# ChicyChen/LOCO-Edit

Hardware: AMD Instinct MI355X
Metric: edit-directions/sec (top-5 PMP-Jacobian SVD @256^2) + vT cos-sim vs ref (higher is better)
Workload: dtype bf16x3 (split-bf16 MFMA operands, fp32 accumulate + fp32 storage); 1 GPU; CelebA-HQ DDPM 256x256 top-5 local basis (l_eye-sized mask, L=2400), t=0.6T, 12 power iterations, one GPU; multi_gpu_form=single, probes_total=5, probes_per_gpu=5, kept=5, n_iter=12, mask_L=2400, weights=synthetic seed 0, streams=2

## Files before the change

### include/loco_hip_diag.h

```cpp
#ifndef LOCO_HIP_DIAG_H
#define LOCO_HIP_DIAG_H
#include "loco_hip.h"
#ifdef __cplusplus
extern "C" {
#endif

int  loco_bench_conv(loco_ctx* ctx, int32_t cin, int32_t cout, int32_t H, int32_t W, int32_t B, int32_t mode,
                     int32_t taps, int32_t tile, int32_t iters, float* ms_avg, void* stream);

typedef struct loco_conv_desc {
    int32_t struct_size;
    int32_t Cin, Cout, Hin, Win, B, taps;
    int32_t stride, upsample, zins, mode, cpg;
    int32_t transposed, accumulate, in_arena, pad;
    int32_t Cin2, cot_cpg;
    float   res_scale;
    int32_t reserved;
    const float *weight, *bias;
    const float *in, *bias2, *res;
    const float *prim, *sc, *sh, *mr, *gamma, *tst, *tc;
    const float *in2, *w2, *bias2nd;
    const float *cot_d, *cot_prim, *cot_sc, *cot_sh, *cot_mr, *cot_tc;
    float* out;
} loco_conv_desc;
int  loco_debug_conv(loco_ctx* ctx, const loco_conv_desc* desc, char* plan, int64_t cap, void* stream);

int64_t loco_debug_tensor(loco_ctx* ctx, const char* name, float* dst, int64_t cap, void* stream);

#ifdef __cplusplus
}
#endif
#endif
```

### loco-edit_amd/csrc/conv_bf16.hip

```cpp
#include "kernels.h"
#include <cstdio>
#include <cstdlib>

namespace loco {

enum : int { PR_BF16X3 = 0, PR_F16 = 1 };
template <int PR, int TAPS, int MODE> void launch_tile_b(const ConvArgs& a, hipStream_t st);
template <int PR, int MODE> void launch_kcat_b(const ConvArgs& a, hipStream_t st);
template <int PR, int MODE> void launch_pair_b(const ConvArgs& a, hipStream_t st);
template <int PR, int MODE> void launch_dual_b(const ConvArgs& a, hipStream_t st);
void launch_conv_gemm(const ConvArgs& a, hipStream_t st);

template <int PR>
static void launch_lowp(const ConvArgs& a, int taps, hipStream_t st) {
#ifdef LOCO_DIAG
    if (a.cot_d && (taps != 1 || a.gemm || a.nsplit > 1 || a.Cin2 > 0 || (a.Cout % conv_bf16_tile_couts(a)) != 0 || a.st_kind == ST_TAN || a.st_kind == ST_COT)) {
        fprintf(stderr, "loco: ConvArgs::cot_d on a launch whose epilogue has no norm-cotangent term (taps %d, gemm %d, nsplit %d, Cout %d, st_kind %d)\n",
                taps, a.gemm, a.nsplit, a.Cout, a.st_kind);
        abort();
    }
#endif
    if constexpr (PR == PR_BF16X3) {
        if (taps == 1 && a.gemm) { launch_conv_gemm(a, st); return; }
    }
    if (taps == 9 && a.Cin2 > 0) {
        if (a.mode == CM_GN_SILU) launch_kcat_b<PR, CM_GN_SILU>(a, st);
        else if (a.mode == CM_GN_GELU) launch_kcat_b<PR, CM_GN_GELU>(a, st);
        else launch_kcat_b<PR, CM_TAN_SILU>(a, st);
        return;
    }
#ifdef LOCO_DIAG
    if constexpr (PR == PR_BF16X3) {
        if (taps == 9 && a.dual) {
            switch (a.mode) {
                case CM_NONE: launch_dual_b<PR, CM_NONE>(a, st); break;
                case CM_GN_SILU: launch_dual_b<PR, CM_GN_SILU>(a, st); break;
                case CM_TAN_SILU: launch_dual_b<PR, CM_TAN_SILU>(a, st); break;
                default: launch_dual_b<PR, CM_COT_SILU>(a, st); break;
            }
            return;
        }
    }
#endif
    if constexpr (PR == PR_BF16X3) {
        if (taps == 9 && a.pair) {
            switch (a.mode) {
                case CM_NONE: launch_pair_b<PR, CM_NONE>(a, st); break;
                case CM_GN_SILU: launch_pair_b<PR, CM_GN_SILU>(a, st); break;
                case CM_TAN_SILU: launch_pair_b<PR, CM_TAN_SILU>(a, st); break;
                default: launch_pair_b<PR, CM_COT_SILU>(a, st); break;
            }
            return;
        }
    }
    if (taps == 9) {
        switch (a.mode) {
            case CM_NONE: launch_tile_b<PR, 9, CM_NONE>(a, st); break;
            case CM_GN_SILU: launch_tile_b<PR, 9, CM_GN_SILU>(a, st); break;
            case CM_GN_GELU: launch_tile_b<PR, 9, CM_GN_GELU>(a, st); break;
            case CM_TAN_SILU: launch_tile_b<PR, 9, CM_TAN_SILU>(a, st); break;
            case CM_COT_SILU: launch_tile_b<PR, 9, CM_COT_SILU>(a, st); break;
            default: launch_tile_b<PR, 9, CM_GN>(a, st); break;
        }
    } else {
        switch (a.mode) {
            case CM_NONE: launch_tile_b<PR, 1, CM_NONE>(a, st); break;
            default: launch_tile_b<PR, 1, CM_GN>(a, st); break;
        }
    }
}
void launch_conv_bf16x3(const ConvArgs& a, int taps, hipStream_t st) { launch_lowp<PR_BF16X3>(a, taps, st); }
void launch_conv_f16(const ConvArgs& a, int taps, hipStream_t st) { launch_lowp<PR_F16>(a, taps, st); }

}
```

### loco-edit_amd/csrc/conv_plan.hip

```cpp
#include "kernels.h"
#include <cstdio>
#include <cstdlib>

namespace loco {

constexpr int BKC = 16;
constexpr int BKF = 8;

static const int kMT[7] = {128, 128, 32, 64, 128, 128, 128}, kNT[7] = {128, 64, 128, 64, 256, 256, 128};

static int env_int(const char* name, int dflt) {
    const char* e = getenv(name);
    return e ? atoi(e) : dflt;
}
static int diag_switch(const char* name) {
#ifdef LOCO_DIAG
    return env_int(name, 0);
#else
    (void)name;
    return 0;
#endif
}

static int pick_tile(int Cout, int HW) {
    if (HW >= 128) return Cout > 32 ? 0 : 2;
    return Cout > 64 ? 1 : 3;
}

static int conv_pick_nsplit(int Cin, int Cout, int Hout, int Wout, int B) {
    const int t = pick_tile(Cout, Hout * Wout);
    long blocks = (long)((Hout * Wout) / kNT[t]) * ((Cout + kMT[t] - 1) / kMT[t]) * B;
    int nchunks = (Cin + BKF - 1) / BKF;
    if (blocks >= 384 || nchunks < 8) return 1;
    int want = (int)((512 + blocks - 1) / blocks);
    int maxs = nchunks / 4;
    if (want > maxs) want = maxs;
    if (want > 32) want = 32;
    return want < 1 ? 1 : want;
}

static int conv_bf16_pick_tile(int Cout, int HW, int B, int tile_override) {
    if (B <= 1 && HW <= 1024 && HW >= 64 && (Cout % 64) == 0) return 3;
    int t = pick_tile(Cout, HW);
    if (t == 0 && HW >= 256) {
        if (tile_override >= 0) return tile_override;
        return 5;
    }
    return t;
}

constexpr int kTile0MaxHW = 65536;

static int bf16_tile_of(const ConvArgs& a, int tile_override = -1) {
    static const bool two_per_cu = diag_switch("LOCO_CONV_2WG") != 0;
    int tile = conv_bf16_pick_tile(a.Cout, a.Hout * a.Wout, a.B, tile_override);
    if (tile == 4) tile = 5;
    if (tile == 5 && a.taps == 1 && !a.gemm && a.B >= 2 && a.Hout * a.Wout <= kTile0MaxHW) return 0;
    if (tile == 5 && two_per_cu && a.taps == 9 && a.stride == 1 && !a.upsample && !a.zins && (a.Cin % BKC) == 0 &&
        a.in_padded && a.pad == 1 && a.Wout >= 32) return 6;
    if (a.stride == 2 && tile == 5) tile = 0;
    return tile;
}
static int tile_for(const ConvArgs& a, int prec, int tile_override) {
    return prec ? bf16_tile_of(a, tile_override) : pick_tile(a.Cout, a.Hout * a.Wout);
}
static int conv_bf16_tile_pixels(const ConvArgs& a) { return a.gemm ? 256 : kNT[a.tile]; }
int conv_bf16_tile_couts(const ConvArgs& a) { return a.gemm ? 64 * a.gemm_tm : kMT[a.tile]; }

static int conv_bf16_pick_nsplit(int Cin, int Cout, int Hout, int Wout, int B, int chip_share, int taps, int lanes) {
    const int HW = Hout * Wout;
    int t = conv_bf16_pick_tile(Cout, HW, B, -1);
    if (t == 4) t = 5;
    if (taps == 1 && t == 5 && B >= 2 && HW <= kTile0MaxHW) t = 0;
    long blocks = (long)(HW / kNT[t]) * ((Cout + kMT[t] - 1) / kMT[t]) * B;
    int nchunks = (Cin + BKC - 1) / BKC;
    int target = chip_share > 1 ? 256 / chip_share : (lanes == 2 ? 240 : 256);
    if (target < 32) target = 32;
    if (blocks >= target / 2 || nchunks < 8) return 1;
    int want = (int)(target / blocks);
    int maxs = nchunks / 4;
    if (want > maxs) want = maxs;
    if (want > 32) want = 32;
    return want < 1 ? 1 : want;
}

static bool conv_lowp_can_kcat(const ConvArgs& a) {
    static const bool on = env_int("LOCO_KCAT", 1) != 0;
    return on && a.Cin2 > 0 && a.nsplit == 1 && bf16_tile_of(a) == 5 && a.stride == 1 && !a.upsample && !a.zins && a.pad == 1 &&
           (a.Cin % BKC) == 0 && (a.Cin2 % BKC) == 0 && a.in_padded &&
           (a.mode == CM_GN_SILU || a.mode == CM_GN_GELU || a.mode == CM_TAN_SILU);
}
static bool conv_lowp_can_fuse_stats(const ConvArgs& a) {
    return a.nsplit <= 1 && !a.gemm && (a.Cout % conv_bf16_tile_couts(a)) == 0;
}

static bool conv_pair_ok(const ConvArgs& a) {
    static const bool on = env_int("LOCO_CONV_PAIR", 1) != 0;
    if (!on || a.Hout * a.Wout < 16384 || a.taps != 9 || a.Cin2 > 0 || a.nsplit != 1 || a.stride != 1 || a.upsample || a.zins ||
        a.pad != 1 || !a.in_padded || (a.Cin % (2 * BKC)) != 0 || (a.Cout % 128) != 0 || (a.Wout % 32) != 0 || (a.Hout % 8) != 0 ||
        a.pers_groups || a.dual)
        return false;
    if (!(a.mode == CM_NONE || a.mode == CM_GN_SILU || a.mode == CM_TAN_SILU || a.mode == CM_COT_SILU)) return false;
    return a.tile == 5;
}

static bool conv_dual_ok(const ConvArgs& a) {
    static const bool on = diag_switch("LOCO_CONV_DUAL") != 0;
    if (!on || a.taps != 9 || a.Cin2 > 0 || a.nsplit != 1 || a.stride != 1 || a.upsample || a.zins || a.pad != 1 || (a.Cin % BKC) != 0 ||
        !a.in_padded || a.Wout < 32 || (a.Wout % 32) != 0 || (a.Hout % 8) != 0 || (a.Cout % 128) != 0 || a.B < 2 || a.cot_d)
        return false;
    if (!(a.mode == CM_NONE || a.mode == CM_GN_SILU || a.mode == CM_TAN_SILU || a.mode == CM_COT_SILU)) return false;
    if (a.tile != 5) return false;
    const long units = (long)((a.Hout * a.Wout) / 256) * (a.Cout / 128) * (a.B / 2);
    return units >= 192;
}

static ConvArgs conv_shift_batch(const ConvArgs& a, int nb) {
    ConvArgs t = a;
    t.B = a.B - nb;
    t.in += (long)nb * a.in_bs; t.out += (long)nb * a.out_bs;
    if (t.prim) t.prim += (long)nb * a.prim_bs;
    if (t.bias2) t.bias2 += (long)nb * a.bias2_bs;
    if (t.res) t.res += (long)nb * a.res_bs;
    if (t.sc) { t.sc += (long)nb * a.scsh_bs; t.sh += (long)nb * a.scsh_bs; }
    if (t.mr) t.mr += (long)nb * a.mr_bs;
    if (t.tst) t.tst += (long)nb * a.tst_bs;
    if (t.tc) t.tc += (long)nb * a.tc_bs;
    if (t.in2) t.in2 += (long)nb * a.in2_bs;
    if (t.cot_d) { t.cot_d += (long)nb * a.cot_d_bs; t.cot_tc += (long)nb * a.cot_tc_bs; }
    if (t.st_part) t.st_part += (long)nb * a.Cout * ((a.Hout * a.Wout) / conv_bf16_tile_pixels(a)) * 2;
    return t;
}

static void conv_pers_plan(ConvArgs& a) {
    a.pers_groups = 0;
    static const int on = diag_switch("LOCO_CONV_PERS");
    if (!on || a.taps != 9 || a.Cin2 > 0 || a.nsplit != 1 || a.stride != 1 || a.upsample || a.zins || a.pad != 1 || !a.in_padded ||
        (a.Cin % (2 * BKC)) != 0 || (a.Cout % 128) != 0 || a.B < 2 || a.cot_d || bf16_tile_of(a) != 5)
        return;
    if (!(a.mode == CM_NONE || a.mode == CM_GN_SILU || a.mode == CM_GN_GELU ||
          (on == 2 && (a.mode == CM_TAN_SILU || a.mode == CM_COT_SILU)))) return;
    const long wg0 = (long)((a.Hout * a.Wout) / 256) * (a.Cout / 128);
    int G = wg0 >= 256 ? 1 : (int)(256 / wg0);
    if (G > a.B) G = a.B;
    const int per = (a.B + G - 1) / G;
    if (per < 2 || a.B * 10 < G * per * 8 || wg0 * G < 192) return;
    a.pers_groups = G;
}

static void conv_gemm_plan(ConvArgs& a) {
    static const bool on = env_int("LOCO_CONV_GEMM", 1) != 0;
    a.gemm = 0;
    const long HW = (long)a.Hout * a.Wout;
    if (!on || a.stride != 1 || a.upsample || a.zins || (a.Cin % BKC) != 0 || a.Cin < 320 || (HW % 256) != 0 || (a.Wout % 16) != 0 ||
        a.Cout < 128 || !a.partial || a.Cin2 > 0 || !(a.mode == CM_NONE || a.mode == CM_GN) || a.cot_d)
        return;
    {
        const int TW = a.Wout < 32 ? a.Wout : 32;
        if ((256 % TW) != 0 || (a.Wout % TW) != 0 || (a.Hout % (256 / TW)) != 0) return;
    }
    static const int all_shapes = env_int("LOCO_GEMM_ALL", 0);
    if (!all_shapes && !(a.Cout >= 640 && (a.Cout >= 4 * a.Cin || a.Cin >= 2560))) return;
    const int pad256 = (a.Cout + 255) / 256 * 256;
    const int tm = (pad256 * 10 <= a.Cout * 11) ? 4 : 2;
    const int mt = 64 * tm;
    const long tiles = (HW / 256) * ((a.Cout + mt - 1) / mt) * a.B;
    const size_t rec_floats = (size_t)a.B * a.Cin * HW;
    int ns = 1;
    if (tiles < 192) {
        const int nchunks = a.Cin / BKC;
        ns = (int)((256 + tiles - 1) / tiles);
        if (ns > 8) ns = 8;
        while (ns > 1 && nchunks / ns < 8) --ns;
        while (ns > 1 && (size_t)ns * a.B * a.Cout * HW + rec_floats > a.partial_floats) --ns;
    }
    if ((ns > 1 ? (size_t)ns * a.B * a.Cout * HW : 0) + rec_floats > a.partial_floats) return;
    a.gemm = 1; a.gemm_tm = tm; a.nsplit = ns;
}

void conv_plan_family(ConvArgs& a, int prec) {
    if (prec == 1 && a.taps == 1) conv_gemm_plan(a);
    if (prec == 1 && a.taps == 9) conv_pers_plan(a);
}

int conv_plan_parts(ConvArgs& a, int prec, int tile_override, ConvArgs parts[2]) {
    a.dual = 0;
    a.tile = tile_for(a, prec, tile_override);
    a.pair = 0;
    parts[0] = a;
    int n = 1;
    if (prec == 1 && a.taps == 9 && conv_dual_ok(a)) {
        parts[0].B = a.B & ~1;
        parts[0].dual = 1;
        if (a.B & 1) {
            parts[1] = conv_shift_batch(a, a.B - 1);
            parts[1].pers_groups = 0;
            n = 2;
        }
    }
    for (int i = 0; i < n; ++i) {
        ConvArgs& p = parts[i];
        p.tile = tile_for(p, prec, tile_override);
        p.pair = prec == 1 && conv_pair_ok(p);
    }
    return n;
}

static bool short_tail(long per_probe, int B) {
    const long total = per_probe * B, r = total % 256;
    return total > 256 && r > 0 && r <= 160;
}

static int tail_split(const ConvArgs& a, size_t partial_floats, int* split) {
    const long per_probe = (long)((a.Hout * a.Wout) / conv_bf16_tile_pixels(a)) * ((a.Cout + 127) / 128);
    const long r = per_probe * a.B % 256;
    if (!short_tail(per_probe, a.B) || per_probe <= 0 || r % per_probe != 0 || r / per_probe >= a.B) return 0;
    int s = (int)(256 / r);
    if (s > 4) s = 4;
    const int nchunks = (a.Cin + 15) / 16;
    while (s > 1 && nchunks / s < 4) --s;
    const size_t one = (size_t)(r / per_probe) * a.Cout * a.Hout * a.Wout;
    while (s > 1 && (size_t)s * one > partial_floats) --s;
    *split = s;
    return s > 1 ? (int)(r / per_probe) : 0;
}

static int stats_route(const ConvEnv& e, const StatAsk* q, bool want, ConvArgs& x, int s0, int B, int* keep_ntile) {
    if (!q || q->kind == ST_NONE) return SR_NONE;
    const int alone = q->norm ? SR_ALONE : SR_NONE;
    if (!want) return alone;
    if (x.nsplit > 1) return !q->norm ? SR_NONE : ((x.Hout * x.Wout) % 4 == 0 ? SR_SPLITK : SR_ALONE);
    const int ntile = (x.Hout * x.Wout) / conv_bf16_tile_pixels(x);
    const size_t need = (size_t)x.B * x.Cout * ntile * 2;
    const int epi = q->norm ? SR_EPI : SR_KEEP;
    const bool kept = q->keep && s0 == 0 && x.B == B && need <= q->keep_floats;
    if (q->kind == ST_FWD && conv_lowp_can_fuse_stats(x) && (kept || (q->norm && need <= e.stpart_floats))) {
        x.st_part = kept ? q->keep : e.stpart; x.st_kind = ST_FWD;
        if (kept) *keep_ntile = ntile;
        return epi;
    }
    const bool cot_cache = q->kind == ST_COT && q->norm && q->sx;
    if ((q->kind == ST_TAN || cot_cache) && e.fuse_lin && !x.cot_d && conv_lowp_can_fuse_stats(x) && !x.pers_groups &&
        !conv_dual_ok(x)) {
        const size_t lane_off = (size_t)e.lane_s0 * (q->keep_floats / e.max_batch);
        const bool keptl = q->kind == ST_TAN && q->keep && s0 == 0 && x.B == B && lane_off + need <= q->keep_floats;
        if (keptl || (q->norm && need <= e.stpart_floats)) {
            x.st_part = keptl ? q->keep + lane_off : e.stpart; x.st_kind = q->kind; x.st_x = q->prim;
            if (q->kind == ST_COT) x.st_sx = q->sx;
            if (keptl) *keep_ntile = ntile;
            return epi;
        }
    }
    return alone;
}

static ConvLaunch plan_launch(const ConvEnv& e, const StatAsk* q, bool want, const ConvArgs& x, int s0, int B, int* keep_ntile) {
    ConvLaunch l;
    l.args = x;
    l.s0 = s0;
    l.args.tile = tile_for(x, e.prec, -1);
    l.stats = stats_route(e, q, want, l.args, s0, B, keep_ntile);
    if (l.stats == SR_EPI || l.stats == SR_KEEP) l.ntile = (x.Hout * x.Wout) / conv_bf16_tile_pixels(l.args);
    l.nparts = conv_plan_parts(l.args, e.prec, -1, l.parts);
    return l;
}

ConvPlan plan_conv(const ConvEnv& e, const ConvArgs& a0, int taps, const StatAsk* q, const ConvArgs* sc) {
    ConvPlan p;
    ConvArgs a = a0;
    a.taps = taps;
    a.dual = 0; a.pers_groups = 0; a.gemm = 0;
    if (sc) {
        ConvArgs t = a;
        t.nsplit = e.prec >= 1 ? conv_bf16_pick_nsplit(a.Cin, a.Cout, a.Hout, a.Wout, a.B, e.chip_share, 9, e.lanes) : 2;
        t.in2 = sc->in; t.in2_bs = sc->in_bs; t.Cin2 = sc->Cin;
        const long per_probe = (long)((a.Hout * a.Wout) / 256) * ((a.Cout + 127) / 128);
        if (e.prec >= 1 && taps == 9 && !short_tail(per_probe, a.B) && !a.bias2 && conv_lowp_can_kcat(t)) {
            a.in2 = sc->in; a.in2_bs = sc->in_bs; a.Cin2 = sc->Cin; a.in2_padded = sc->in_padded;
            a.wb2 = e.prec == 2 ? sc->wh : sc->wb;
            a.bias2 = sc->bias; a.bias2_bs = 0;
            a.res = nullptr;
        } else {
            p.sc_first = true;
            a.res = sc->out; a.res_bs = sc->out_bs;
        }
    }
    if (e.prec == 2) a.wb = a.wh;
    a.no_deep = e.deep1 ? 0 : 1;
    a.nsplit = e.prec >= 1 ? conv_bf16_pick_nsplit(a.Cin, a.Cout, a.Hout, a.Wout, a.B, e.chip_share, taps, e.lanes)
                           : conv_pick_nsplit(a.Cin, a.Cout, a.Hout, a.Wout, a.B);
    if (a.cot_d) {
        ConvArgs t = a;
        t.tile = bf16_tile_of(t);
        const long per_probe = (long)((a.Hout * a.Wout) / conv_bf16_tile_pixels(t)) * ((a.Cout + 127) / 128);
        p.cot = e.prec >= 1 && taps == 1 && a.nsplit == 1 && !short_tail(per_probe, a.B) && conv_lowp_can_fuse_stats(t);
        if (!p.cot) { a.cot_d = nullptr; a.cot_d_bs = 0; a.cot_sx = nullptr; a.cot_tc = nullptr; a.cot_tc_bs = 0; }
    }
    while (a.nsplit > 1 && (size_t)a.nsplit * a.B * a.Cout * a.Hout * a.Wout > e.partial_floats) a.nsplit >>= 1;
    if (a.nsplit < 1) a.nsplit = 1;
    a.partial = e.partial;
    a.partial_floats = e.partial_floats;
    conv_plan_family(a, e.prec);
    a.tile = tile_for(a, e.prec, -1);
    int split = 1;
    const int tail = e.prec >= 1 && a.nsplit == 1 && a.B >= 2 && !a.gemm && !a.pers_groups ? tail_split(a, e.partial_floats, &split) : 0;
    const bool want = q && q->kind != ST_NONE && e.prec >= 1 && e.fuse_stats;
    if (!tail) {
        p.l[0] = plan_launch(e, q, want, a, 0, a.B, &p.keep_ntile);
        return p;
    }
    const bool per_part = want && q->norm && (q->kind == ST_FWD || (e.fuse_lin && (a.Hout * a.Wout) % 4 == 0));
    p.stats_all = !per_part && q && q->kind != ST_NONE && q->norm;
    const StatAsk* ql = per_part ? q : nullptr;
    const int nb = a.B - tail;
    ConvArgs m = a, t = conv_shift_batch(a, nb);
    m.B = nb;
    t.nsplit = split;
    p.nl = 2;
    p.l[0] = plan_launch(e, ql, want, m, 0, a.B, &p.keep_ntile);
    p.l[1] = plan_launch(e, ql, want, t, nb, a.B, &p.keep_ntile);
    return p;
}

const char* conv_variant_name(const ConvArgs& a, int taps, int prec) {
    static const char* tiles[6] = {"2,2,2,2", "4,1,1,2", "1,4,1,1", "2,2,1,1", "2,2,2,4", "2,4,2,2"};
    static char names[3][2][6][6][56];
    static char others[5][3][6][40];
    const int mode = (a.mode < 0 || a.mode > 5) ? 2 : a.mode;
    const char* other = nullptr;
    int k = 0, v = mode;
    if (prec && taps == 9 && a.Cin2 > 0) other = prec == 1 ? "conv_kcat_bf16x3<2,4,2,2,%d>" : "conv_kcat_f16<2,4,2,2,%d>";
    else if (prec == 1 && taps == 1 && a.gemm) { k = 1; other = "conv_gemm_bf16x3<%d>"; v = a.gemm_tm; }
    else if (prec == 1 && taps == 9 && a.pers_groups > 0 && !a.dual) { k = 2; other = "conv_pers_bf16x3<9,2,4,2,2,%d>"; }
    else if (prec == 1 && taps == 9 && a.pair) { k = 3; other = "conv_pair_bf16x3<%d>"; }
    else if (prec == 1 && taps == 9 && a.dual) { k = 4; other = "conv_dual_bf16x3<%d>"; }
    if (other) {
        char* n = others[k][prec][v];
        if (!n[0]) snprintf(n, 40, other, v);
        return n;
    }
    int t = a.tile == 6 ? 0 : a.tile;
    if (t < 0 || t > 5) t = 0;
    int m = mode;
    if (taps != 9 && m != CM_NONE) m = CM_GN;
    if (!prec && m == CM_GN_GELU) m = CM_GN_SILU;
    char* n = names[prec][taps == 9 ? 0 : 1][t][m];
    static const char* kn[3] = {"conv_mfma_f32", "conv_mfma_bf16x3", "conv_mfma_f16"};
    if (!n[0]) snprintf(n, 56, "%s<%d,%s,%d>", kn[prec], taps, tiles[t], m);
    return n;
}

}
```

### loco-edit_amd/csrc/conv_plan_text.h

```cpp
#pragma once
#include "kernels.h"
#include <cstdio>
#include <string>

namespace loco {

inline void conv_plan_text(const ConvPlan& p, int taps, int prec, std::string& out) {
    char line[320];
    for (int li = 0; li < p.nl; ++li) {
        const ConvLaunch& l = p.l[li];
        for (int pi = 0; pi < l.nparts; ++pi) {
            const ConvArgs& y = l.parts[pi];
            snprintf(line, sizeof(line),
                     "launch=%d part=%d kernel=%s tile=%d nsplit=%d B=%d s0=%d gemm=%d gemm_tm=%d pair=%d Cin2=%d sc_first=%d cot=%d\n",
                     li, pi, conv_variant_name(y, taps, prec), y.tile, l.args.nsplit, y.B, l.s0 + (pi ? l.args.B - y.B : 0), y.gemm,
                     y.gemm ? y.gemm_tm : 0, y.pair, y.Cin2, p.sc_first ? 1 : 0, p.cot ? 1 : 0);
            out += line;
        }
    }
}

}
```

### loco-edit_amd/csrc/engine.hip

```cpp
#include <hip/hip_runtime.h>

#include <algorithm>
#include <array>
#include <cmath>
#include <cstdio>
#include <cstdlib>
#include <cstring>
#include <map>
#include <memory>
#include <thread>
#include <atomic>
#include <string>
#include <vector>

#include "../../include/loco_hip.h"
#ifdef LOCO_DIAG
#include "../../include/loco_hip_diag.h"
#endif
#include "kernels.h"
#include "program.h"
#ifdef LOCO_DIAG
#include "conv_plan_text.h"
#endif

// ... 35 lines not shown
};
struct Weights {
    std::vector<OpWeights> op;
    float *freq = nullptr, *td0w = nullptr, *td0b = nullptr, *td1w = nullptr, *td1b = nullptr;
    float* tcw = nullptr;
    float *tp_w = nullptr, *tp_b = nullptr;
    long tproj_total = 0;
    double flops = 0.0;
};

struct Tens : TensPlan {
    float* keep = nullptr; size_t keep_floats = 0; int keep_ntile = 0;
};
struct NormP : NormPlan, NormW {
    bool ready = false;
};
struct Op : OpPlan, OpWeights {
    NormP n1, n2, nx;
    float *xK = nullptr, *xV = nullptr;
};

struct HostParam { std::vector<float> data; std::vector<int64_t> shape; bool loaded = false; };

}


struct loco_ctx {
    loco_unet_cfg cfg;
    std::string err;
    std::map<std::string, HostParam> params;
    bool finalized = false;

    std::shared_ptr<const Program> prog;
    std::shared_ptr<Weights> wts;
    std::vector<Tens> tens;
    std::vector<Op> ops;


    float *arenaP = nullptr, *arenaT = nullptr;
    float *statsP = nullptr, *statsT = nullptr;
    double* red = nullptr;
    bool fuse_cot = true;
    float *stpart = nullptr, *stpart2 = nullptr;
    size_t stpart_floats = 0;
    bool fuse_stats = true;
    bool fuse_xattn = true;
    bool deep1 = true;
    bool flash_attn = true;
    float* attn_delta = nullptr;
    float* partial = nullptr;
    size_t partial_floats = 0;
    const float* bench_out = nullptr; int64_t bench_out_count = 0;
#ifdef LOCO_DIAG
    std::string* plan_log = nullptr;
#endif
    float *tact = nullptr, *tproj = nullptr;
    float* eps_buf = nullptr;
    float* gx0 = nullptr;
    float* ge = nullptr;
    float* tmpA = nullptr;
    double *G = nullptr, *Q = nullptr, *W = nullptr, *gscratch = nullptr;
    float* alphas = nullptr;
    float* ctx_colbias = nullptr;
    bool has_ctx = false;
    float* cond_add = nullptr;
    float* ctx_norm = nullptr;
    bool has_cond = false;
    float* cond_in = nullptr;
    bool has_tcond = false;
    float2* sxcache = nullptr;
    int prec = 0;
    std::vector<float*> owned;
    size_t bytes = 0;

    bool primal_ok = false;
    float p_cv = 0.f, p_ce = 0.f;
    uint8_t* mask = nullptr;
    bool has_mask = false;
    uint8_t* mask2 = nullptr;
    bool has_mask2 = false;
    int mask2_from = 0;
    int* mask_idx = nullptr;
    int* mask_L_dev = nullptr;
    long mask_L = 0;
    hipStream_t mask_stream = nullptr;
    int primal_B = 0;
    hipEvent_t ev0 = nullptr, ev1 = nullptr;
    int n_streams = 1;
    hipStream_t st2 = nullptr;
    hipStream_t st2_user = nullptr;
    hipEvent_t ev_fork = nullptr, ev_join = nullptr;
    double* red2 = nullptr;
    struct FwdGraph { hipGraph_t graph = nullptr; hipGraphExec_t exec = nullptr; int calls = 0; };
    std::map<int, FwdGraph> fwd_graphs;
    bool graph_on = false;
    bool gemm_lowp = true;
    unsigned char* gemm_ws[2] = {nullptr, nullptr}; size_t gemm_ws_bytes[2] = {0, 0}; int lane = 0;
    loco_ctx* weights_of = nullptr;
    int forks = 0;
    bool zombie = false;
    bool fuse_lin = true;
    int lanes_active = 1;
    int lane_s0 = 0;
    int chip_share = 1;
    hipStream_t cap_st = nullptr;
    float* xin_buf = nullptr;
    float* t_dev = nullptr;
    bool prof_on = false;
    struct ProfRec { const char* name; double flops; hipEvent_t e0, e1; int cin, cout, h, b, ns, mode, taps; };
    bool prof_shapes = false;
    std::vector<ProfRec> prof;
    std::vector<hipEvent_t> ev_pool;
    size_t ev_used = 0;
    hipEvent_t next_event() {
        if (ev_used == ev_pool.size()) {
            hipEvent_t e; (void)hipEventCreate(&e); ev_pool.push_back(e);
        }
        return ev_pool[ev_used++];
    }
};

namespace {

template <typename T>
int dalloc(loco_ctx* c, T** p, size_t count) {
    void* q = nullptr;
    HIPCHK(c, hipMalloc(&q, count * sizeof(T)));
    *p = reinterpret_cast<T*>(q);
    c->owned.push_back(reinterpret_cast<float*>(q));
    c->bytes += count * sizeof(T);
    return 0;
}

inline float eps_of(const loco_ctx* c, const NormP& n) { return n.eps > 0.f ? n.eps : c->cfg.gn_eps; }


int upload(loco_ctx* c, float** dst, const std::vector<float>& h) {
    if (dalloc(c, dst, h.size() ? h.size() : 1)) return -1;
    HIPCHK(c, hipMemcpy(*dst, h.data(), h.size() * sizeof(float), hipMemcpyHostToDevice));
    return 0;
}

static inline uint16_t f2bf(float f) {
    uint32_t u; std::memcpy(&u, &f, 4);
    u += 0x7FFFu + ((u >> 16) & 1u);
    return (uint16_t)(u >> 16);
}
static inline float bf2f(uint16_t h) {
    uint32_t u = (uint32_t)h << 16; float f; std::memcpy(&f, &u, 4); return f;
}
template <typename F>
static void parallel_for(int n, size_t work, F fn) {
    unsigned nt = std::thread::hardware_concurrency();
    if (nt > 16) nt = 16;
    if ((int)nt > n) nt = (unsigned)n;
    if (nt <= 1 || work < ((size_t)1 << 18)) { for (int i = 0; i < n; ++i) fn(i); return; }
    std::atomic<int> next{0};
    std::vector<std::thread> th;
    for (unsigned t = 0; t < nt; ++t)
        th.emplace_back([&]() { int i; while ((i = next.fetch_add(1)) < n) fn(i); });
    for (auto& t : th) t.join();
}

template <typename F>
static std::vector<float> build_records(int nin, int nout, int taps, F get) {
    int nch = (nin + 15) / 16, noutP = (nout + 31) & ~31;
// ... 895 lines not shown
                const long PSb = p.bs();
                auto X = [&](int i) { return p.T(op.xt[i]); };
                if (!op.n1.ready) gn_forward_stats(p, op.n1, p.T(op.in), PSb, HW);
                op.n1.ready = false;
                NS s = nstats(c, stats, op.n1);
                {
                    ConvArgs a; conv_defaults(a);
                    a.in = p.T(op.in); a.in_bs = PSb; a.Cin = C; a.Hin = H; a.Win = W;
                    setw(a, op.pj_in, false); a.bias = op.pj_in.bias; a.pad = 0;
                    a.mode = CM_GN; a.sc = s.sc; a.sh = s.sh; a.scsh_bs = SB;
                    a.out = X(X_H0); a.out_bs = PSb; a.Cout = C; a.Hout = H; a.Wout = W; a.B = B;
                    run_conv(c, a, 1, st);
                }
                const SA sa{c, &op, B, T, NH, C / NH, st};
                const XA xa = xa_of(c, op, B, st);
                launch_ln_fwd(X(X_H0), PSb, B, C, T, op.lng[0], op.lnb[0], 1e-5f, X(X_A1), PSb, X(X_LN1), PSb, st);
                lin1x1(c, op.qkvc, false, X(X_A1), PSb, C, X(X_QKV), PSb, 3 * C, H, W, B, nullptr, 0, false, st);
                sa_forward(sa, arena);
                lin1x1(c, op.to_out1, false, X(X_O), PSb, C, X(X_H1), PSb, C, H, W, B, X(X_H0), PSb, true, st);
                launch_ln_fwd(X(X_H1), PSb, B, C, T, op.lng[1], op.lnb[1], 1e-5f, X(X_A2), PSb, X(X_LN2), PSb, st);
                lin1x1(c, op.xqc, false, X(X_A2), PSb, C, X(X_XQ), PSb, C, H, W, B, nullptr, 0, false, st);
                if (!xa_fused(xa, 0, X(X_XQ), PSb, op.xK, op.xV, X(X_XS), PSb, X(X_XO), PSb)) {
                    xa_scores(xa, X(X_XQ), PSb, op.xK, X(X_XS), PSb, xa.scale, true);
                    launch_softmax_rows(X(X_XS), (long)NH * T, xa.Lp, st, B, PSb);
                    xa_values(xa, op.xV, X(X_XS), PSb, X(X_XO), PSb);
                }
                lin1x1(c, op.to_out2, false, X(X_XO), PSb, C, X(X_H2), PSb, C, H, W, B, X(X_H1), PSb, true, st);
                launch_ln_fwd(X(X_H2), PSb, B, C, T, op.lng[2], op.lnb[2], 1e-5f, X(X_A3), PSb, X(X_LN3), PSb, st);
                lin1x1(c, op.ff1, false, X(X_A3), PSb, C, X(X_F), PSb, 8 * C, H, W, B, nullptr, 0, true, st);
                launch_geglu(0, X(X_F), PSb, nullptr, B, 4L * C * T, X(X_GG), PSb, st);
                lin1x1(c, op.ff2, false, X(X_GG), PSb, 4 * C, X(X_H3), PSb, C, H, W, B, X(X_H2), PSb, true, st);
                const StatReq rq = next_fwd(op.out);
                lin1x1(c, op.pj_out, false, X(X_H3), PSb, C, p.T(op.out), PSb, C, H, W, B, p.T(op.in), PSb, true, st, &rq);
                break;
            }
            case OP_DOWN: case OP_UP: {
                const Tens& ti = c->tens[op.in];
                ConvArgs a; conv_defaults(a);
                a.in = p.T(op.in); a.in_bs = p.bs(); a.Cin = ti.C; a.Hin = ti.H; a.Win = ti.W;
                setw(a, op.conv, false); a.bias = op.conv.bias;
                if (op.kind == OP_DOWN) { a.stride = 2; a.pad = op.sym_down ? 1 : 0; } else { a.upsample = 1; }
                a.out = p.T(op.out); a.out_bs = p.bs(); a.Cout = to.C; a.Hout = to.H; a.Wout = to.W; a.B = B;
                const StatReq rq = next_fwd(op.out);
                run_conv(c, a, 9, st, &rq);
                break;
            }
            case OP_OUT: {
                const Tens& ti = c->tens[op.in];
                if (!op.n1.ready) gn_forward_stats(p, op.n1, p.T(op.in), p.bs(), ti.H * ti.W);
                op.n1.ready = false;
                NS s = nstats(c, stats, op.n1);
                ConvArgs a; conv_defaults(a);
                a.in = p.T(op.in); a.in_bs = p.bs(); a.Cin = ti.C; a.Hin = ti.H; a.Win = ti.W;
                setw(a, op.conv, false); a.bias = op.conv.bias;
                a.mode = CM_GN_SILU; a.sc = s.sc; a.sh = s.sh; a.scsh_bs = SB;
                a.out = p.T(op.out); a.out_bs = p.bs(); a.Cout = to.C; a.Hout = to.H; a.Wout = to.W; a.B = B;
                run_conv(c, a, 9, st);
                break;
            }
        }
    }
    return 0;
}

void tangent_stats(loco_ctx* c, const NormP& n, const float* d, long dbs, const float* x, int HW, int B,
                   hipStream_t st) {
    NS sp = nstats(c, c->statsP, n);
    NS stt = nstats(c, c->statsT, n);
    launch_gn_tstats(d, dbs, x, 0, B, n.C, HW, c->cfg.gn_groups, sp.sc, sp.sh, sp.mr, 0, 0, 0, stt.tst,
                     stt.tc, c->prog->stats_per_sample, c->red, st);
}
void set_tan(loco_ctx* c, ConvArgs& a, const NormP& n, const float* prim) {
    NS sp = nstats(c, c->statsP, n);
    NS stt = nstats(c, c->statsT, n);
    a.mode = CM_TAN_SILU; a.prim = prim; a.prim_bs = 0;
    a.sc = sp.sc; a.sh = sp.sh; a.scsh_bs = 0; a.mr = sp.mr; a.mr_bs = 0; a.gamma_ = n.gamma;
    a.tst = stt.tst; a.tst_bs = c->prog->stats_per_sample; a.cpg = n.C / c->cfg.gn_groups;
    a.tc = stt.tc; a.tc_bs = c->prog->stats_per_sample;
    a.sx = (n.sx_off >= 0 && c->sxcache) ? c->sxcache + n.sx_off : nullptr;
}

constexpr size_t RED_BYTES = (size_t)4 << 20;

int tangent_pass(loco_ctx* c, const float* V, int B, hipStream_t st) {
    const loco_unet_cfg& cfg = c->cfg;
    const long PS = c->prog->per_sample;
    auto TP = [&](int id) { return c->arenaP + c->tens[id].off; };
    auto TT = [&](int id) { return c->arenaT + c->tens[id].off; };
    clear_ready(c);
    auto next_tan = [&](int tid) {
        StatReq r = req_lin(c, ST_TAN, consumer_norm(c, tid), TP(tid));
        Tens& t = c->tens[tid];
        if (t.cat_of >= 0 && t.keep && c->fuse_lin) {
            r.kind = ST_TAN; r.stats = c->statsT; r.prim = TP(tid);
            r.keep = t.keep; r.keep_floats = t.keep_floats; r.keep_ntile = &t.keep_ntile;
        }
        return r;
    };
    for (auto& op : c->ops) {
        const Tens& to = c->tens[op.out];
        const int HW = to.H * to.W;
        switch (op.kind) {
            case OP_CONV_IN: {
                ConvArgs a; conv_defaults(a);
                a.in = V; a.in_bs = c->prog->n_in; a.Cin = cfg.in_channels; a.Hin = cfg.resolution; a.Win = cfg.resolution;
                setw(a, op.conv, false);
                a.out = TT(op.out); a.out_bs = PS; a.Cout = to.C; a.Hout = to.H; a.Wout = to.W; a.B = B;
                if (op.ksize == 1) a.pad = 0;
                const StatReq rq = next_tan(op.out);
                run_conv(c, a, op.ksize == 1 ? 1 : 9, st, &rq);
                break;
            }
            case OP_CONV: {
                const Tens& ti = c->tens[op.in];
                ConvArgs a; conv_defaults(a);
                a.in = TT(op.in); a.in_bs = PS; a.Cin = ti.C; a.Hin = ti.H; a.Win = ti.W;
                setw(a, op.conv, false);
                a.out = TT(op.out); a.out_bs = PS; a.Cout = to.C; a.Hout = to.H; a.Wout = to.W; a.B = B;
                if (op.ksize == 1) a.pad = 0;
                const StatReq rq = next_tan(op.out);
                run_conv(c, a, op.ksize == 1 ? 1 : 9, st, &rq);
                break;
            }
            case OP_RES: {
                const Tens& ti = c->tens[op.in];
                const int HWi = ti.H * ti.W;
                if (!op.n1.ready && !cat_fused_tstats(c, op.n1, op.in, B, st)) tangent_stats(c, op.n1, TT(op.in), PS, TP(op.in), HWi, B, st);
                op.n1.ready = false;
                ConvArgs a; conv_defaults(a);
                a.Cin = ti.C;
                setw(a, op.c1, false);
                if (op.updown == 1) {
                    NS sp = nstats(c, c->statsP, op.n1);
                    NS stt = nstats(c, c->statsT, op.n1);
                    launch_gn_apply(5, TT(op.in), PS, TP(op.in), 0, nullptr, 0, TT(op.a1), PS, 0, B, ti.C, HWi,
                                    cfg.gn_groups, sp.sc, sp.sh, sp.mr, 0, 0, stt.tst, c->prog->stats_per_sample, st, cfg.act);
                    launch_pool2x2_sum(TT(op.a1), PS, TT(op.ap), PS, 0, B, ti.C, to.H, to.W, st, 0.25f);
                    launch_pool2x2_sum(TT(op.in), PS, TT(op.xu), PS, 0, B, ti.C, to.H, to.W, st, 0.25f);
                    a.in = TT(op.ap); a.in_bs = PS; a.Hin = to.H; a.Win = to.W;
                } else {
                    a.in = TT(op.in); a.in_bs = PS; a.Hin = ti.H; a.Win = ti.W;
                    set_tan(c, a, op.n1, TP(op.in));
                    if (op.updown == 2) {
                        a.upsample = 1;
                        launch_upsample2x(TT(op.in), PS, TT(op.xu), PS, 0, 1.0f, B, ti.C, ti.H, ti.W, st);
                    }
                }
                a.out = TT(op.h1); a.out_bs = PS; a.Cout = to.C; a.Hout = to.H; a.Wout = to.W; a.B = B;
                {
                    const StatReq rq2 = req_lin(c, ST_TAN, &op.n2, TP(op.h1));
                    run_conv(c, a, 9, st, &rq2);
                    op.n2.ready = false;
                }
                const float* xin = op.updown ? TT(op.xu) : TT(op.in);
                ConvArgs n; conv_defaults(n);
                if (op.has_nin) {
                    n.in = xin; n.in_bs = PS; n.Cin = ti.C; n.Hin = to.H; n.Win = to.W;
                    setw(n, op.nin, false); n.pad = 0;
                    n.out = TT(op.out); n.out_bs = PS; n.Cout = to.C; n.Hout = to.H; n.Wout = to.W; n.B = B;
                }
                ConvArgs b; conv_defaults(b);
                b.in = TT(op.h1); b.in_bs = PS; b.Cin = to.C; b.Hin = to.H; b.Win = to.W;
                setw(b, op.c2, false); b.res = xin; b.res_bs = PS;
                b.res_scale = op.has_nin ? 1.f : c->prog->res_scale;
                set_tan(c, b, op.n2, TP(op.h1));
                b.out = TT(op.out); b.out_bs = PS; b.Cout = to.C; b.Hout = to.H; b.Wout = to.W; b.B = B;
                const StatReq rq = next_tan(op.out);
// ... 49 lines not shown
                attn_gemm(c, h, st);
                if (!kcat) { h.A = v; h.sab = 0; h.Bm = TT(op.S); h.sbb = PS; h.beta = 1.f; attn_gemm(c, h, st); }
                }
                ConvArgs pr; conv_defaults(pr);
                pr.in = TT(op.o); pr.in_bs = PS; pr.Cin = C; pr.Hin = to.H; pr.Win = to.W;
                setw(pr, op.proj, false); pr.pad = 0; pr.res = TT(op.in); pr.res_bs = PS;
                pr.out = TT(op.has_x ? op.xmid : op.out); pr.out_bs = PS; pr.Cout = C; pr.Hout = to.H; pr.Wout = to.W; pr.B = B;
                {
                    const StatReq rq = next_tan(op.has_x ? op.xmid : op.out);
                    run_conv(c, pr, 1, st, &rq);
                }
                if (op.has_x) {
                    const XA x = xa_of(c, op, B, st);
                    if (!op.nx.ready) tangent_stats(c, op.nx, TT(op.xmid), PS, TP(op.xmid), HW, B, st);
                    op.nx.ready = false;
                    NS spx = nstats(c, c->statsP, op.nx);
                    NS stx = nstats(c, c->statsT, op.nx);
                    launch_gn_apply(1, TT(op.xmid), PS, TP(op.xmid), 0, nullptr, 0, TT(op.xhn), PS, 0, B, C, HW,
                                    cfg.gn_groups, spx.sc, spx.sh, spx.mr, 0, 0, stx.tst, c->prog->stats_per_sample, st);
                    xa_conv1x1(c, op.xqc, false, TT(op.xhn), PS, TT(op.xq), PS, C, to.H, to.W, B, nullptr, 0, false, st);
                    if (!xa_fused(x, 1, TT(op.xq), PS, op.xK, op.xV, TP(op.xS), 0, TT(op.xo), PS)) {
                        xa_scores(x, TT(op.xq), PS, op.xK, TT(op.xS), PS, 1.f, false);
                        launch_softmax_jac(TT(op.xS), TP(op.xS), (long)NH * T, x.Lp, (long)NH * T, x.scale, st, B, PS);
                        xa_values(x, op.xV, TT(op.xS), PS, TT(op.xo), PS);
                    }
                    const StatReq rqx = next_tan(op.out);
                    xa_conv1x1(c, op.xproj, false, TT(op.xo), PS, TT(op.out), PS, C, to.H, to.W, B, TT(op.xmid), PS, false, st, &rqx);
                }
                break;
            }
            case OP_XFMR: {
                const int C = to.C, T = HW, NH = op.heads, H = to.H, W = to.W;
                auto XP = [&](int i) { return TP(op.xt[i]); };
                auto XT_ = [&](int i) { return TT(op.xt[i]); };
                if (!op.n1.ready) tangent_stats(c, op.n1, TT(op.in), PS, TP(op.in), HW, B, st);
                op.n1.ready = false;
                NS sp = nstats(c, c->statsP, op.n1);
                NS stt = nstats(c, c->statsT, op.n1);
                launch_gn_apply(1, TT(op.in), PS, TP(op.in), 0, nullptr, 0, XT_(X_G0), PS, 0, B, C, HW,
                                cfg.gn_groups, sp.sc, sp.sh, sp.mr, 0, 0, stt.tst, c->prog->stats_per_sample, st);
                lin1x1(c, op.pj_in, false, XT_(X_G0), PS, C, XT_(X_H0), PS, C, H, W, B, nullptr, 0, false, st);
                const SA sa{c, &op, B, T, NH, C / NH, st};
                const XA xa = xa_of(c, op, B, st);
                launch_ln_tan(XT_(X_H0), PS, XP(X_H0), XP(X_LN1), B, C, T, op.lng[0], XT_(X_A1), PS, st);
                lin1x1(c, op.qkvc, false, XT_(X_A1), PS, C, XT_(X_QKV), PS, 3 * C, H, W, B, nullptr, 0, false, st);
                sa_tangent(sa);
                lin1x1(c, op.to_out1, false, XT_(X_O), PS, C, XT_(X_H1), PS, C, H, W, B, XT_(X_H0), PS, false, st);
                launch_ln_tan(XT_(X_H1), PS, XP(X_H1), XP(X_LN2), B, C, T, op.lng[1], XT_(X_A2), PS, st);
                lin1x1(c, op.xqc, false, XT_(X_A2), PS, C, XT_(X_XQ), PS, C, H, W, B, nullptr, 0, false, st);
                if (!xa_fused(xa, 1, XT_(X_XQ), PS, op.xK, op.xV, XP(X_XS), 0, XT_(X_XO), PS)) {
                    xa_scores(xa, XT_(X_XQ), PS, op.xK, XT_(X_XS), PS, 1.f, false);
                    launch_softmax_jac(XT_(X_XS), XP(X_XS), (long)NH * T, xa.Lp, (long)NH * T, xa.scale, st, B, PS);
                    xa_values(xa, op.xV, XT_(X_XS), PS, XT_(X_XO), PS);
                }
                lin1x1(c, op.to_out2, false, XT_(X_XO), PS, C, XT_(X_H2), PS, C, H, W, B, XT_(X_H1), PS, false, st);
                launch_ln_tan(XT_(X_H2), PS, XP(X_H2), XP(X_LN3), B, C, T, op.lng[2], XT_(X_A3), PS, st);
                lin1x1(c, op.ff1, false, XT_(X_A3), PS, C, XT_(X_F), PS, 8 * C, H, W, B, nullptr, 0, false, st);
                launch_geglu(1, XT_(X_F), PS, XP(X_F), B, 4L * C * T, XT_(X_GG), PS, st);
                lin1x1(c, op.ff2, false, XT_(X_GG), PS, 4 * C, XT_(X_H3), PS, C, H, W, B, XT_(X_H2), PS, false, st);
                const StatReq rq = next_tan(op.out);
                lin1x1(c, op.pj_out, false, XT_(X_H3), PS, C, TT(op.out), PS, C, H, W, B, TT(op.in), PS, false, st, &rq);
                break;
            }
            case OP_DOWN: case OP_UP: {
                const Tens& ti = c->tens[op.in];
                ConvArgs a; conv_defaults(a);
                a.in = TT(op.in); a.in_bs = PS; a.Cin = ti.C; a.Hin = ti.H; a.Win = ti.W;
                setw(a, op.conv, false);
                if (op.kind == OP_DOWN) { a.stride = 2; a.pad = op.sym_down ? 1 : 0; } else { a.upsample = 1; }
                a.out = TT(op.out); a.out_bs = PS; a.Cout = to.C; a.Hout = to.H; a.Wout = to.W; a.B = B;
                const StatReq rq = next_tan(op.out);
                run_conv(c, a, 9, st, &rq);
                break;
            }
            case OP_OUT: {
                const Tens& ti = c->tens[op.in];
                if (!op.n1.ready) tangent_stats(c, op.n1, TT(op.in), PS, TP(op.in), ti.H * ti.W, B, st);
                op.n1.ready = false;
                ConvArgs a; conv_defaults(a);
                a.in = TT(op.in); a.in_bs = PS; a.Cin = ti.C; a.Hin = ti.H; a.Win = ti.W;
                setw(a, op.conv, false);
                set_tan(c, a, op.n1, TP(op.in));
                a.out = TT(op.out); a.out_bs = PS; a.Cout = to.C; a.Hout = to.H; a.Wout = to.W; a.B = B;
                run_conv(c, a, 9, st);
                break;
            }
        }
    }
    return 0;
}

void cot_stats(loco_ctx* c, const NormP& n, const float* d, long dbs, const float* x, int HW, int B, int kind,
               hipStream_t st) {
    NS sp = nstats(c, c->statsP, n);
    NS stt = nstats(c, c->statsT, n);
    launch_gn_tstats(d, dbs, x, 0, B, n.C, HW, c->cfg.gn_groups, sp.sc, sp.sh, sp.mr, 0, 0, kind, stt.tst,
                     stt.tc, c->prog->stats_per_sample, c->red, st, c->cfg.act);
}

int cotangent_pass(loco_ctx* c, const float* ge, const float* gx0, float* Aout, int B, hipStream_t st) {
    const loco_unet_cfg& cfg = c->cfg;
    const long PS = c->prog->per_sample;
    const int G = cfg.gn_groups;
    auto TP = [&](int id) { return c->arenaP + c->tens[id].off; };
    auto TG = [&](int id) { return c->arenaT + c->tens[id].off; };
    auto GO = [&](const Op& o) -> const float* { return o.out == c->prog->eps_t ? ge : TG(o.out); };
    auto GOS = [&](const Op& o) -> long { return o.out == c->prog->eps_t ? (long)c->prog->n_out : PS; };
    clear_ready(c);
    for (int oi = (int)c->ops.size() - 1; oi >= 0; --oi) {
        Op& op = c->ops[oi];
        const Tens& to = c->tens[op.out];
        const int HW = to.H * to.W;
        switch (op.kind) {
            case OP_OUT: {
                const Tens& ti = c->tens[op.in];
                ConvArgs a; conv_defaults(a);
                a.in = GO(op); a.in_bs = GOS(op); a.Cin = to.C; a.Hin = to.H; a.Win = to.W;
                setw(a, op.conv, true);
                a.out = TG(op.a1); a.out_bs = PS; a.Cout = ti.C; a.Hout = ti.H; a.Wout = ti.W; a.B = B;
                {
                    const StatReq rq = req_lin(c, ST_COT, &op.n1, TP(op.in));
                    run_conv(c, a, 9, st, &rq);
                    op.n1.ready = false;
                }
                NS sp = nstats(c, c->statsP, op.n1);
                NS stt = nstats(c, c->statsT, op.n1);
                launch_gn_apply(2, TG(op.a1), PS, TP(op.in), 0, nullptr, 0, TG(op.in), PS, 0, B, ti.C, ti.H * ti.W, G,
                                sp.sc, sp.sh, sp.mr, 0, 0, stt.tst, c->prog->stats_per_sample, st, cfg.act);
                break;
            }
            case OP_UP: {
                const Tens& ti = c->tens[op.in];
                ConvArgs a; conv_defaults(a);
                a.in = TG(op.out); a.in_bs = PS; a.Cin = to.C; a.Hin = to.H; a.Win = to.W;
                setw(a, op.conv, true);
                a.out = TG(op.up); a.out_bs = PS; a.Cout = ti.C; a.Hout = to.H; a.Wout = to.W; a.B = B;
                run_conv(c, a, 9, st);
                launch_pool2x2_sum(TG(op.up), PS, TG(op.in), PS, 0, B, ti.C, ti.H, ti.W, st);
                break;
            }
            case OP_DOWN: {
                const Tens& ti = c->tens[op.in];
                ConvArgs a; conv_defaults(a);
                a.in = TG(op.out); a.in_bs = PS; a.Cin = to.C; a.Hin = to.H; a.Win = to.W;
                setw(a, op.conv, true); a.zins = 1; a.pad = op.sym_down ? 1 : 2; a.accumulate = op.in_is_skip ? 1 : 0;
                a.out = TG(op.in); a.out_bs = PS; a.Cout = ti.C; a.Hout = ti.H; a.Wout = ti.W; a.B = B;
                run_conv(c, a, 9, st);
                break;
            }
            case OP_RES: {
                const Tens& ti = c->tens[op.in];
                const int HWi = ti.H * ti.W;
                ConvArgs a; conv_defaults(a);
                a.in = TG(op.out); a.in_bs = PS; a.Cin = to.C; a.Hin = to.H; a.Win = to.W;
                setw(a, op.c2, true);
                a.out = TG(op.h1); a.out_bs = PS; a.Cout = to.C; a.Hout = to.H; a.Wout = to.W; a.B = B;
                {
                    const StatReq rq2 = req_lin(c, ST_COT, &op.n2, TP(op.h1));
                    run_conv(c, a, 9, st, &rq2);
                    op.n2.ready = false;
                }
                ConvArgs b; conv_defaults(b);
                b.in = TG(op.h1); b.in_bs = PS; b.Cin = to.C; b.Hin = to.H; b.Win = to.W;
                setw(b, op.c1, true);
                set_tan(c, b, op.n2, TP(op.h1));
                b.mode = CM_COT_SILU;
                b.out_bs = PS; b.Cout = ti.C; b.Hout = to.H; b.Wout = to.W; b.B = B;
                if (op.updown == 0) {
                    b.out = TG(op.a1);
                    const StatReq rq1 = req_lin(c, ST_COT, &op.n1, TP(op.in));
                    run_conv(c, b, 9, st, &rq1);
                } else if (op.updown == 1) {
                    b.out = TG(op.ap);
                    run_conv(c, b, 9, st);
                    launch_upsample2x(TG(op.ap), PS, TG(op.a1), PS, 0, 0.25f, B, ti.C, to.H, to.W, st);
                } else {
                    b.out = TG(op.xu);
                    run_conv(c, b, 9, st);
                    launch_pool2x2_sum(TG(op.xu), PS, TG(op.a1), PS, 0, B, ti.C, ti.H, ti.W, st);
                }
                if (!op.n1.ready) cot_stats(c, op.n1, TG(op.a1), PS, TP(op.in), HWi, B, 1, st);
                op.n1.ready = false;
                NS sp = nstats(c, c->statsP, op.n1);
                NS stt = nstats(c, c->statsT, op.n1);
                int acc = op.in_is_skip ? 1 : 0;
                const float* gsk = TG(op.out);
                bool cot_in_epilogue = false;
                if (op.has_nin) {
                    ConvArgs n; conv_defaults(n);
                    n.in = TG(op.out); n.in_bs = PS; n.Cin = to.C; n.Hin = to.H; n.Win = to.W;
                    setw(n, op.nin, true); n.pad = 0;
                    n.Cout = ti.C; n.Hout = to.H; n.Wout = to.W; n.B = B; n.out_bs = PS;
                    n.out = TG(op.in); n.accumulate = acc;
                    if (op.updown == 0 && c->prec >= 1 && c->fuse_cot && op.n1.sx_off >= 0 && c->sxcache) {
                        n.cot_d = TG(op.a1); n.cot_d_bs = PS; n.cot_sx = c->sxcache + op.n1.sx_off;
                        n.cot_tc = stt.tc; n.cot_tc_bs = c->prog->stats_per_sample;
                    }
                    cot_in_epilogue = run_conv(c, n, 1, st);
                    gsk = nullptr;
                }
                if (op.updown == 0) {
                    if (cot_in_epilogue) {  }
                    else if (op.has_nin)
                        launch_gn_apply(2, TG(op.a1), PS, TP(op.in), 0, nullptr, 0, TG(op.in), PS, 1, B, ti.C, HWi, G,
                                        sp.sc, sp.sh, sp.mr, 0, 0, stt.tst, c->prog->stats_per_sample, st, cfg.act);
                    else
                        launch_gn_apply(2, TG(op.a1), PS, TP(op.in), 0, gsk, PS, TG(op.in), PS, acc, B, ti.C, HWi, G,
                                        sp.sc, sp.sh, sp.mr, 0, 0, stt.tst, c->prog->stats_per_sample, st, cfg.act, c->prog->res_scale);
                } else {
                    launch_gn_apply(2, TG(op.a1), PS, TP(op.in), 0, nullptr, 0, TG(op.in), PS, acc, B, ti.C, HWi, G,
                                    sp.sc, sp.sh, sp.mr, 0, 0, stt.tst, c->prog->stats_per_sample, st, cfg.act);
// ... 171 lines not shown
    c->lanes_active = 1;
    if (rc) return rc;
    HIPCHK(c, hipEventRecord(c->ev_join, s2));
    HIPCHK(c, hipStreamWaitEvent(st, c->ev_join, 0));
    return 0;
}
int alloc_state(loco_ctx* c) {
    const Program& P = *c->prog;
    const size_t MB = (size_t)c->cfg.max_batch;
    c->tens.resize(P.tens.size());
    c->ops.resize(P.ops.size());
    for (size_t i = 0; i < P.tens.size(); ++i) {
        Tens& t = c->tens[i];
        static_cast<TensPlan&>(t) = P.tens[i];
        if (t.cat_of < 0) continue;
        t.keep_floats = MB * (size_t)t.C * ((size_t)t.H * t.W / 64 + 1) * 2;
        if (dalloc(c, &t.keep, t.keep_floats)) return -1;
    }
    for (size_t i = 0; i < P.ops.size(); ++i) {
        const OpPlan& plan = P.ops[i];
        Op& v = c->ops[i];
        static_cast<OpPlan&>(v) = plan;
        static_cast<NormPlan&>(v.n1) = plan.n1; static_cast<NormPlan&>(v.n2) = plan.n2; static_cast<NormPlan&>(v.nx) = plan.nx;
        if (!plan.has_ctx_kv()) continue;
        const size_t kv = (size_t)P.tens[plan.in].C * P.ctx_Lp;
        if (dalloc(c, &v.xK, kv) || dalloc(c, &v.xV, kv)) return -1;
    }
    return 0;
}

int create_ctx(loco_ctx* c, const loco_unet_cfg* cfg, std::shared_ptr<const Program> prog) {
    c->cfg = *cfg;
    c->prog = std::move(prog);
    const size_t MB = (size_t)cfg->max_batch;
    {
        float *p0 = nullptr, *p1 = nullptr;
        if (dalloc(c, &p0, MB * c->prog->per_sample + 128) || dalloc(c, &p1, MB * c->prog->per_sample + 128)) return -1;
        c->arenaP = p0 + 64; c->arenaT = p1 + 64;
    }
    if (dalloc(c, &c->statsP, MB * c->prog->stats_per_sample) || dalloc(c, &c->statsT, MB * c->prog->stats_per_sample)) return -1;
    if (dalloc(c, &c->red, RED_BYTES) || dalloc(c, &c->red2, RED_BYTES)) return -1;
    if (alloc_state(c)) return -1;
    {
        c->stpart_floats = MB * (size_t)(c->prog->max_tensor / 64 + 1) * 2;
        if (dalloc(c, &c->stpart, c->stpart_floats) || dalloc(c, &c->stpart2, c->stpart_floats)) return -1;
        const char* e = getenv("LOCO_FUSE_STATS");
        c->fuse_stats = !(e && atoi(e) == 0);
        e = getenv("LOCO_FUSE_LIN");
        c->fuse_lin = !(e && atoi(e) == 0);
        e = getenv("LOCO_FUSE_COT");
        c->fuse_cot = !(e && atoi(e) == 0) && cfg->act == ACT_SILU;
        e = getenv("LOCO_DEEP1");
        c->deep1 = !(e && atoi(e) == 0);
        e = getenv("LOCO_FUSE_XATTN");
        c->fuse_xattn = !(e && atoi(e) == 0);
        const char* fa = getenv("LOCO_FLASH_ATTN");
        c->flash_attn = !(fa && atoi(fa) == 0);
        if (dalloc(c, &c->attn_delta, MB * (size_t)c->prog->attn_dmax)) return -1;
    }
    c->partial_floats = (size_t)64 << 20;
    if (dalloc(c, &c->partial, c->partial_floats)) return -1;
    if (dalloc(c, &c->xin_buf, MB * c->prog->n_in) || dalloc(c, &c->t_dev, 4)) return -1;
    if (dalloc(c, &c->eps_buf, MB * c->prog->n_out) || dalloc(c, &c->gx0, MB * c->prog->n_in) || dalloc(c, &c->ge, MB * c->prog->n_out))
        return -1;
    if (dalloc(c, &c->tmpA, (size_t)64 * c->prog->n_in)) return -1;
    if (dalloc(c, &c->G, 64 * 64) || dalloc(c, &c->Q, 64 * 64) || dalloc(c, &c->W, SOLVER_W_GATE + 1)) return -1;
    {
        size_t nblk = ((size_t)c->prog->n_in + 255) / 256;
        if (dalloc(c, &c->gscratch, nblk * 64 * 64 + 4096)) return -1;
    }
    if (dalloc(c, &c->alphas, 256) || dalloc(c, &c->cond_add, (size_t)cfg->ch * 4)) return -1;
    if (dalloc(c, &c->cond_in, (size_t)cfg->ch)) return -1;
    {
        float2* sx0 = nullptr;
        if (dalloc(c, &sx0, (size_t)c->prog->sx_total + 64)) return -1;
        c->sxcache = sx0 + 32;
    }
    {
        const char* e = getenv("LOCO_PRECISION");
        c->prec = (e && std::string(e) == "f32") ? 0 : (e && std::string(e) == "f16") ? 2 : 1;
    }
    if (dalloc(c, &c->mask2, (size_t)c->prog->n_out)) return -1;
    if (dalloc(c, &c->mask, (size_t)c->prog->n_out) || dalloc(c, &c->mask_idx, (size_t)c->prog->n_out) ||
        dalloc(c, &c->mask_L_dev, 4)) return -1;
    HIPCHK(c, hipEventCreate(&c->ev0));
    HIPCHK(c, hipEventCreate(&c->ev1));
    {
        const char* e = getenv("LOCO_STREAMS");
        c->n_streams = (e && atoi(e) == 2) ? 2 : 1;
        HIPCHK(c, hipStreamCreateWithFlags(&c->st2, hipStreamNonBlocking));
        HIPCHK(c, hipStreamCreateWithFlags(&c->cap_st, hipStreamNonBlocking));
        const char* gl = getenv("LOCO_GEMM_LOWP");
        if (gl) c->gemm_lowp = atoi(gl) != 0;
        const char* gr = getenv("LOCO_GRAPH");
        c->graph_on = gr && atoi(gr) == 1;
        HIPCHK(c, hipEventCreateWithFlags(&c->ev_fork, hipEventDisableTiming));
        HIPCHK(c, hipEventCreateWithFlags(&c->ev_join, hipEventDisableTiming));
    }
    return 0;
}

}

extern "C" {

const char* loco_version(void) { return "loco_hip 0.2 (gfx950; conv arithmetic: f32 MFMA | bf16x3 split-bf16 MFMA | f16 MFMA)"; }

int loco_device_count(void) {
    int n = 0;
    if (hipGetDeviceCount(&n) != hipSuccess) return 0;
    return n;
}

int loco_create(const loco_unet_cfg* cfg, loco_ctx** out) {
    if (!cfg || !out) return -2;
    loco_ctx* c = new loco_ctx();
    *out = c;
    if (cfg->struct_size != (int32_t)sizeof(loco_unet_cfg)) {
        c->err = "loco_unet_cfg.struct_size = " + std::to_string(cfg->struct_size) + ", this library expects " +
                 std::to_string(sizeof(loco_unet_cfg)) + " (binding and library built from different headers)";
        return -2;
    }
    auto prog = std::make_shared<Program>();
    if (const int rc = build_program(*cfg, prog.get(), &c->err)) return rc;
    for (const ParamDecl& d : prog->params) c->params[d.name].shape = d.shape;
    c->wts = std::make_shared<Weights>();
    c->wts->op.resize(prog->ops.size());
    return create_ctx(c, cfg, std::move(prog));
}

int loco_fork(loco_ctx* parent, int32_t max_batch, loco_ctx** out) {
    if (!parent || !out) return -2;
    *out = nullptr;
    if (finalize_params(parent)) return -3;
    loco_ctx* root = parent->weights_of ? parent->weights_of : parent;
    loco_unet_cfg cfg = parent->cfg;
    if (max_batch > 0) cfg.max_batch = max_batch;
    loco_ctx* c = new loco_ctx();
    *out = c;
    if (const int rc = create_ctx(c, &cfg, root->prog)) return rc;
    c->wts = root->wts;
    if (bind_weights(c)) return -1;
    c->prec = parent->prec;
    c->weights_of = root;
    ++root->forks;
    return 0;
}

static void destroy_now(loco_ctx* c);
void loco_destroy(loco_ctx* c) {
    if (!c) return;
    if (c->forks > 0) { c->zombie = true; return; }
    loco_ctx* root = c->weights_of;
    destroy_now(c);
    if (root && --root->forks == 0 && root->zombie) destroy_now(root);
}
static void destroy_now(loco_ctx* c) {
    for (float* p : c->owned) (void)hipFree(p);
    for (unsigned char* p : c->gemm_ws) if (p) (void)hipFree(p);
    if (c->ev0) (void)hipEventDestroy(c->ev0);
    if (c->ev1) (void)hipEventDestroy(c->ev1);
    if (c->ev_fork) (void)hipEventDestroy(c->ev_fork);
    if (c->ev_join) (void)hipEventDestroy(c->ev_join);
    if (c->st2) (void)hipStreamDestroy(c->st2);
    drop_graphs(c);
    if (c->cap_st) (void)hipStreamDestroy(c->cap_st);
    for (hipEvent_t e : c->ev_pool) (void)hipEventDestroy(e);
// ... 57 lines not shown
            c->primal_B = B;
            launch_copy(c->arenaP + c->tens[c->prog->eps_t].off, c->prog->per_sample, eps, c->prog->n_out, 0, B, c->prog->n_out, st);
            HIPCHK(c, hipGetLastError());
            return 0;
        }
    }
    if (forward_pass(c, x, t, B, c->arenaP, c->statsP, st)) return -1;
    c->primal_B = B;
    launch_copy(c->arenaP + c->tens[c->prog->eps_t].off, c->prog->per_sample, eps, c->prog->n_out, 0, B, c->prog->n_out, st);
    HIPCHK(c, hipGetLastError());
    return 0;
}

static void sched_coeffs(float at, float at_next, float eta, float* s1, float* s2, float* s3, float* ce, float* cn) {
    *s1 = std::sqrt(1.0f - at); *s2 = std::sqrt(at); *s3 = std::sqrt(at_next);
    *cn = 0.f;
    if (eta == 0.f) {
        *ce = std::sqrt(1.0f - at_next);
    } else {
        float sigma = std::sqrt((1.0f - at / at_next) * (1.0f - at_next) / (1.0f - at));
        *ce = std::sqrt(1.0f - at_next - eta * (sigma * sigma));
        *cn = eta * sigma;
    }
}

int loco_sched_step(loco_ctx* c, const float* x, const float* et, float at, float at_next, float eta,
                    const float* noise, int64_t count, float* x_next, float* x0_out, void* stream) {
    if (!c) return -2;
    if (eta != 0.f && !noise) { c->err = "eta != 0 needs a noise tensor"; return -2; }
    float s1, s2, s3, ce, cn;
    sched_coeffs(at, at_next, eta, &s1, &s2, &s3, &ce, &cn);
    launch_ddim_step(x, et, eta == 0.f ? nullptr : noise, x_next, x0_out, (long)count, s2, s1, s3, ce, cn,
                     (hipStream_t)stream);
    HIPCHK(c, hipGetLastError());
    return 0;
}

int loco_ddim_step(loco_ctx* c, const float* x, float t, float at, float at_next, float eta, const float* noise,
                   int32_t B, float* x_next, void* stream) {
    if (!c) return -2;
    if (eta != 0.f && !noise) { c->err = "eta != 0 needs a noise tensor"; return -2; }
    if (c->prog->n_out != c->prog->n_in) { c->err = "loco_ddim_step: this network is not a denoiser (output and input sizes differ)"; return -2; }
    int rc = loco_unet_forward(c, x, t, B, c->eps_buf, stream);
    if (rc) return rc;
    return loco_sched_step(c, x, c->eps_buf, at, at_next, eta, noise, (int64_t)B * c->prog->n_in, x_next, nullptr, stream);
}

int loco_pmp_primal(loco_ctx* c, const float* x, float t, float at, const uint8_t* mask, int32_t use_et,
                    void* stream) {
    if (!c) return -2;
    if (finalize_params(c)) return -3;
    if (c->prog->n_out != c->prog->n_in && !use_et) {
        c->err = "loco_pmp_primal: a network whose output size differs from its input has no x0 combination; use_et = 1 "
                 "(raw network Jacobian)";
        return -2;
    }
    hipStream_t st = (hipStream_t)stream;
    if (forward_pass(c, x, t, 1, c->arenaP, c->statsP, st)) return -1;
    c->primal_B = 1;
    if (c->prec >= 1) {
        for (auto& op : c->ops) {
            if (op.kind != OP_RES && op.kind != OP_OUT) continue;
            const Tens& ti = c->tens[op.in];
            const int HW = ti.H * ti.W, G = c->cfg.gn_groups;
            NS s1 = nstats(c, c->statsP, op.n1);
            launch_gn_cache(c->arenaP + ti.off, op.n1.C, HW, op.n1.C / G, s1.sc, s1.sh, s1.mr,
                            c->sxcache + op.n1.sx_off, st, c->cfg.act);
            if (op.kind == OP_RES) {
                const Tens& th = c->tens[op.h1];
                NS s2 = nstats(c, c->statsP, op.n2);
                launch_gn_cache(c->arenaP + th.off, op.n2.C, th.H * th.W, op.n2.C / G, s2.sc, s2.sh, s2.mr,
                                c->sxcache + op.n2.sx_off, st, c->cfg.act);
            }
        }
    }
    if (use_et) { c->p_cv = 0.f; c->p_ce = 1.f; }
    else { c->p_cv = 1.0f / std::sqrt(at); c->p_ce = -std::sqrt(1.0f - at) / std::sqrt(at); }
    c->has_mask = (mask != nullptr);
    c->has_mask2 = false;
    c->mask_L = c->prog->n_out;
    if (mask) {
        HIPCHK(c, hipMemcpyAsync(c->mask, mask, (size_t)c->prog->n_out, hipMemcpyDeviceToDevice, st));
        launch_mask_compact(c->mask, c->prog->n_out, c->mask_idx, c->mask_L_dev, st);
        c->mask_L = -1;
        c->mask_stream = st;
    }
    HIPCHK(c, hipGetLastError());
    c->primal_ok = true;
    return 0;
}

int loco_pmp_set_second_mask(loco_ctx* c, const uint8_t* mask2, int32_t from_row, void* stream) {
    if (!c) return -2;
    if (!c->primal_ok) { c->err = "loco_pmp_primal has not been called"; return -2; }
    if (!mask2) { c->has_mask2 = false; return 0; }
    if (!c->has_mask) { c->err = "a second mask needs a first one (loco_pmp_primal with mask)"; return -2; }
    if (from_row < 0) { c->err = "from_row must be >= 0"; return -2; }
    HIPCHK(c, hipMemcpyAsync(c->mask2, mask2, (size_t)c->prog->n_out, hipMemcpyDeviceToDevice, (hipStream_t)stream));
    c->has_mask2 = true;
    c->mask2_from = from_row;
    return 0;
}

int loco_pmp_jvp(loco_ctx* c, const float* V, int32_t k, float* U, void* stream) {
    if (!c) return -2;
    if (!c->primal_ok) { c->err = "loco_pmp_primal has not been called"; return -2; }
    hipStream_t st = (hipStream_t)stream;
    const int MB = c->cfg.max_batch;
    for (int b0 = 0; b0 < k; b0 += MB) {
        int B = (k - b0 < MB) ? k - b0 : MB;
        int rc = run_lanes(c, B, st, [&](int s0, int nb, hipStream_t ls) -> int {
            const float* Vc = V + (long)(b0 + s0) * c->prog->n_in;
            if (tangent_pass(c, Vc, nb, ls)) return -1;
            launch_copy(c->arenaT + c->tens[c->prog->eps_t].off, c->prog->per_sample, c->eps_buf, c->prog->n_out, 0, nb, c->prog->n_out, ls);
            launch_masked_axpby(c->prog->n_out == c->prog->n_in ? Vc : nullptr, c->eps_buf, c->has_mask ? c->mask : nullptr, c->p_cv,
                                c->p_ce, U + (long)(b0 + s0) * c->prog->n_out, nb, c->prog->n_out, ls,
                                c->has_mask2 ? c->mask2 : nullptr, (long)c->mask2_from - (b0 + s0));
            return 0;
        });
        if (rc) return rc;
    }
    HIPCHK(c, hipGetLastError());
    return 0;
}

int loco_pmp_vjp(loco_ctx* c, const float* U, int32_t k, float* A, void* stream) {
    if (!c) return -2;
    if (!c->primal_ok) { c->err = "loco_pmp_primal has not been called"; return -2; }
    hipStream_t st = (hipStream_t)stream;
    const int MB = c->cfg.max_batch;
    for (int b0 = 0; b0 < k; b0 += MB) {
        int B = (k - b0 < MB) ? k - b0 : MB;
        int rc = run_lanes(c, B, st, [&](int s0, int nb, hipStream_t ls) -> int {
            const bool same = c->prog->n_out == c->prog->n_in;
            launch_cot_seed(U + (long)(b0 + s0) * c->prog->n_out, c->has_mask ? c->mask : nullptr, c->p_cv, c->p_ce, c->ge,
                            same ? c->gx0 : nullptr, nb, c->prog->n_out, ls, c->has_mask2 ? c->mask2 : nullptr,
                            (long)c->mask2_from - (b0 + s0));
            return cotangent_pass(c, c->ge, same ? c->gx0 : nullptr, A + (long)(b0 + s0) * c->prog->n_in, nb, ls);
        });
        if (rc) return rc;
    }
    HIPCHK(c, hipGetLastError());
    return 0;
}

int loco_orthonormalize(loco_ctx* c, float* A, int32_t k, int64_t n, float* s, void* stream) {
    if (!c) return -2;
    if (k < 1 || k > 64 || n > c->prog->n_in) { c->err = "orthonormalize: need k <= 64 and n <= C*H*W"; return -2; }
    hipStream_t st = (hipStream_t)stream;
    launch_gram(A, k, n, c->G, c->gscratch, st);
    launch_jacobi_eig(c->G, k, c->W, c->Q, st);
    launch_rotate_rows(A, c->tmpA, k, n, c->Q, c->W, 0, st);
    const double* gate = c->W + SOLVER_W_GATE;
    launch_gram(c->tmpA, k, n, c->G, c->gscratch, st, gate);
    launch_cholesky(c->G, k, st, 0.25, c->W, gate);
    launch_trsm_rows(c->tmpA, A, k, n, c->G, st, gate);
    launch_sign_fix(A, k, n, s, c->W, reinterpret_cast<float*>(c->red), st);
    HIPCHK(c, hipGetLastError());
    return 0;
}

int loco_qr_rows(loco_ctx* c, float* A, int32_t k, int64_t n, void* stream) {
    if (!c) return -2;
    if (k < 1 || k > 64 || n > c->prog->n_in) { c->err = "qr_rows: need k <= 64 and n <= C*H*W"; return -2; }
    hipStream_t st = (hipStream_t)stream;
    for (int rep = 0; rep < 2; ++rep) {
        launch_gram(A, k, n, c->G, c->gscratch, st);
        launch_cholesky(c->G, k, st);
        launch_trsm_rows(A, c->tmpA, k, n, c->G, st);
        HIPCHK(c, hipMemcpyAsync(A, c->tmpA, (size_t)k * n * sizeof(float), hipMemcpyDeviceToDevice, st));
    }
    HIPCHK(c, hipGetLastError());
    return 0;
}

int loco_convergence(loco_ctx* c, const float* Vprev, const float* V, int64_t count, float atol, float* out2,
                     void* stream) {
    if (!c) return -2;
    launch_convergence(Vprev, V, count, atol, 1e-5f, out2, c->gscratch, (hipStream_t)stream);
    HIPCHK(c, hipGetLastError());
    return 0;
}

int loco_convergence_rows(loco_ctx* c, const float* Vprev, const float* V, int32_t k, int64_t n, float atol,
                          float* out2, void* stream) {
    if (!c) return -2;
    if (k < 1 || k > 64 || n < 1) { c->err = "convergence_rows: need 1 <= k <= 64"; return -2; }
    if (n > c->prog->n_in) { c->err = "convergence_rows: rows longer than the context's input"; return -2; }
    {
        const size_t nseg = (size_t)((n + 255) / 256) < 64 ? (size_t)((n + 255) / 256) : 64;
        const size_t cap = (((size_t)c->prog->n_in + 255) / 256) * 64 * 64 + 4096;
        if ((size_t)k * nseg * 4 > cap) { c->err = "convergence_rows: k rows of this length exceed the reduction workspace"; return -2; }
    }
    launch_convergence_rows(Vprev, V, k, n, atol, 1e-5f, out2, c->gscratch, (hipStream_t)stream);
    HIPCHK(c, hipGetLastError());
    return 0;
}

int loco_null_project(loco_ctx* c, const float* Vm, int32_t k, const float* Vn, int32_t k0, int64_t n, float* out,
                      void* stream) {
    if (!c) return -2;
    if (k < 1 || k > 64 || k0 > 64 || n > c->prog->n_in) { c->err = "null_project: bad sizes"; return -2; }
    hipStream_t st = (hipStream_t)stream;
    if (Vn && k0 > 0) {
        launch_cross_gram(Vn, k0, Vm, k, n, c->G, c->gscratch, st);
        launch_project_rows(Vm, k, Vn, k0, n, c->G, out, st);
    } else if (out != Vm) {
        HIPCHK(c, hipMemcpyAsync(out, Vm, (size_t)k * n * sizeof(float), hipMemcpyDeviceToDevice, st));
    }
    launch_normalize_rows(out, k, n, c->gscratch, st);
    HIPCHK(c, hipGetLastError());
    return 0;
}

int loco_edit_axpy(loco_ctx* c, const float* x, const float* v, const float* alphas, int32_t B, int64_t n, float* out,
                   void* stream) {
    if (!c) return -2;
    if (B > 256) { c->err = "edit_axpy: B > 256"; return -2; }
    hipStream_t st = (hipStream_t)stream;
    HIPCHK(c, hipMemcpyAsync(c->alphas, alphas, B * sizeof(float), hipMemcpyHostToDevice, st));
    launch_edit_axpy(x, v, c->alphas, B, n, out, st);
// ... 151 lines not shown
    HIPCHK(c, hipGetLastError());
    return 0;
}

int loco_diffedit_mask(loco_ctx* c, const float* eps_a, const float* eps_b, float scale, int32_t B, int32_t C, int64_t HW,
                       int32_t rule, float* m_out, uint8_t* mask_out, void* stream) {
    if (!c) return -2;
    if (!eps_a || !eps_b || !mask_out || B < 1 || C < 1 || HW < 1) { c->err = "diffedit_mask: bad arguments"; return -2; }
    if (rule != 0 && rule != 1) { c->err = "diffedit_mask: rule is 0 (reference) or 1 (intended)"; return -2; }
    float* ws = reinterpret_cast<float*>(c->gscratch);
    const size_t cap = 2 * ((((size_t)c->prog->n_in + 255) / 256) * 64 * 64 + 4096);
    float* m = m_out;
    if (!m) {
        if (1024 + (size_t)HW > cap) { c->err = "diffedit_mask: map larger than the reduction workspace; pass m_out"; return -2; }
        m = ws + 1024;
    }
    hipStream_t st = (hipStream_t)stream;
    launch_diffedit_mask(eps_a, eps_b, scale, B, C, (long)HW, rule, m, mask_out, ws, ws + 768, st);
    HIPCHK(c, hipGetLastError());
    float status[3] = {0.f, 0.f, 0.f};
    HIPCHK(c, hipMemcpyAsync(status, ws + 768, sizeof(status), hipMemcpyDeviceToHost, st));
    HIPCHK(c, hipStreamSynchronize(st));
    if (status[0] == 1.f) {
        c->err = "diffedit_mask: constant map (max == min = " + std::to_string(status[1]) + "): the two noise predictions do not differ";
        return -4;
    }
    if (status[0] != 0.f) { c->err = "diffedit_mask: non-finite map"; return -5; }
    return 0;
}

int loco_cfg_masked_step(loco_ctx* c, const float* x, const float* eps_for, const float* eps_edit, const float* eps_null,
                         float g, float at, float at_next, const uint8_t* mask, int32_t B, int64_t n, float* x_next,
                         void* stream) {
    if (!c) return -2;
    if (!x || !eps_for || !eps_edit || !eps_null || !mask || !x_next || B < 1 || n < 1) {
        c->err = "cfg_masked_step: bad arguments";
        return -2;
    }
    float s1, s2, s3, ce, cn;
    sched_coeffs(at, at_next, 0.f, &s1, &s2, &s3, &ce, &cn);
    launch_cfg_masked_step(x, eps_for, eps_edit, eps_null, mask, x_next, B, (long)n, g, s2, s1, s3, ce, (hipStream_t)stream);
    HIPCHK(c, hipGetLastError());
    return 0;
}

int loco_lcm_step(loco_ctx* c, const float* x, const float* eps, float at, float at_prev, float c_skip, float c_out,
                  const float* noise, int64_t count, float* x_prev, float* denoised, void* stream) {
    if (!c) return -2;
    if (!x || !eps || count < 1 || (!x_prev && !denoised)) { c->err = "lcm_step: bad arguments"; return -2; }
    if (!(at > 0.f && at <= 1.f) || !(at_prev >= 0.f && at_prev <= 1.f)) { c->err = "lcm_step: alpha-bar outside (0, 1]"; return -2; }
    launch_lcm_step(x, eps, noise, x_prev, denoised, (long)count, std::sqrt(at), std::sqrt(1.0f - at), std::sqrt(at_prev),
                    std::sqrt(1.0f - at_prev), c_skip, c_out, (hipStream_t)stream);
    HIPCHK(c, hipGetLastError());
    return 0;
}

#ifdef LOCO_DIAG
}
__global__ void diag_fill_records(unsigned char* rec, long nrec, int wpitch, unsigned seed, float scale) {
    const long r = (long)blockIdx.x * 256 + threadIdx.x;
    if (r >= nrec) return;
    const int idx = (int)(r % wpitch);
    unsigned short hi[16], lo[16];
    for (int k = 0; k < 16; ++k) {
        unsigned h = (unsigned)(r * 16 + k) * 2654435761u + seed * 40503u;
        h ^= h >> 15; h *= 2246822519u; h ^= h >> 13; h *= 3266489917u; h ^= h >> 16;
        const float v = scale * ((float)(h & 0xffffff) * (1.0f / 8388608.0f) - 1.0f);
        const __bf16 hb = (__bf16)v;
        const __bf16 lb = (__bf16)(v - (float)hb);
        hi[k] = __builtin_bit_cast(unsigned short, hb);
        lo[k] = __builtin_bit_cast(unsigned short, lb);
    }
    const int sw = (idx >> 2) & 3;
    unsigned short* base = reinterpret_cast<unsigned short*>(rec + r * 64);
    for (int k = 0; k < 8; ++k) {
        base[((0 ^ sw) << 3) + k] = hi[k];
        base[((1 ^ sw) << 3) + k] = hi[8 + k];
        base[((2 ^ sw) << 3) + k] = lo[k];
        base[((3 ^ sw) << 3) + k] = lo[8 + k];
    }
}
extern "C" {
int loco_bench_conv(loco_ctx* c, int32_t cin, int32_t cout, int32_t H, int32_t W, int32_t B, int32_t mode,
                    int32_t taps, int32_t tile, int32_t iters, float* ms_avg, void* stream) {
    if (!c) return -2;
    if (finalize_params(c)) return -3;
    hipStream_t st = (hipStream_t)stream;
    const long HW = (long)H * W;
    const long in_e = (long)cin * HW, out_e = (long)cout * HW;
    if ((in_e + out_e) * B > (long)c->cfg.max_batch * c->prog->per_sample || 2 * in_e > (long)c->prog->per_sample ||
        in_e > c->prog->sx_total) { c->err = "bench_conv: shape exceeds the arenas"; return -2; }
    float* in = c->arenaT;
    float* out = c->arenaT + in_e * B;
    const int bz = getenv("LOCO_BENCH_ZERO") ? atoi(getenv("LOCO_BENCH_ZERO")) : 0;
    const float zs = (bz & 1) ? 0.0f : 1.0f, zw = (bz & 2) ? 0.0f : 1.0f;
    launch_fill_random(in, in_e * B, 1u, zs, st);
    launch_fill_random(c->arenaP, in_e, 2u, zs, st);
    launch_fill_random(reinterpret_cast<float*>(c->sxcache), 2 * in_e, 3u, zs, st);
    launch_fill_random(c->statsP, c->prog->stats_per_sample, 4u, 1.0f, st);
    launch_fill_random(c->statsT, c->prog->stats_per_sample * B, 5u, 0.01f, st);
    size_t wfl = (size_t)((cin + 15) / 16) * 16 * taps * ((cout + 31) & ~31);
    if (wfl * 2 > c->partial_floats) { c->err = "bench_conv: weights exceed workspace"; return -2; }
    float* wf = c->partial + c->partial_floats - wfl * 2;
    launch_fill_random(wf, (long)wfl * 2, 6u, 0.05f * zw, st);
    if (c->prec == 1) {
        const long nrec = (long)((cin + 15) / 16) * taps * ((cout + 31) & ~31);
        hipLaunchKernelGGL(diag_fill_records, dim3((unsigned)((nrec + 255) / 256)), dim3(256), 0, st,
                           reinterpret_cast<unsigned char*>(wf), nrec, (cout + 31) & ~31, 7u, 0.05f * zw);
    }
    ConvArgs a; conv_defaults(a);
    a.in = in; a.in_bs = in_e; a.Cin = cin; a.Hin = H; a.Win = W;
    a.prim = c->arenaP; a.prim_bs = 0; a.sx = c->sxcache;
    a.w = wf; a.wb = wf; a.wh = wf;
    a.out = out; a.out_bs = out_e; a.Cout = cout; a.Hout = H; a.Wout = W; a.B = B;
    a.mode = mode; a.pad = taps == 9 ? 1 : 0; a.in_padded = 1; a.taps = taps;
    a.sc = c->statsP; a.sh = c->statsP + cin; a.scsh_bs = 0; a.mr = c->statsP + 2 * cin; a.mr_bs = 0;
    a.gamma_ = c->statsP; a.tst = c->statsT; a.tst_bs = c->prog->stats_per_sample; a.cpg = cin / c->cfg.gn_groups;
    a.tc = c->statsT + 64; a.tc_bs = c->prog->stats_per_sample;
    if (a.cpg < 1) a.cpg = 1;
    a.nsplit = 1; a.partial = c->partial;
    a.partial_floats = c->partial_floats - wfl * 2;
    if (getenv("LOCO_BENCH_COT") && atoi(getenv("LOCO_BENCH_COT")) && taps == 1) {
        if ((in_e + 2 * out_e) * B > (long)c->cfg.max_batch * c->prog->per_sample || out_e > c->prog->sx_total ||
            2L * cout > c->prog->stats_per_sample) { c->err = "bench_conv: cot operands exceed the arenas"; return -2; }
        launch_fill_random(out + out_e * B, out_e * B, 8u, zs, st);
        if (out_e > in_e) launch_fill_random(reinterpret_cast<float*>(c->sxcache), 2 * out_e, 3u, zs, st);
        a.cot_d = out + out_e * B; a.cot_d_bs = out_e; a.cot_sx = c->sxcache; a.cot_tc = c->statsT; a.cot_tc_bs = c->prog->stats_per_sample;
    }
    if (getenv("LOCO_BENCH_ACC") && atoi(getenv("LOCO_BENCH_ACC"))) a.accumulate = 1;
    conv_plan_family(a, c->prec);
    if (const char* e = getenv("LOCO_DUAL_WHATIF")) a.no_deep = atoi(e);
    ConvArgs parts[2];
    const int nparts = conv_plan_parts(a, c->prec, tile, parts);
    auto run = [&]() {
        for (int pi = 0; pi < nparts; ++pi) {
            if (c->prec == 1) launch_conv_bf16x3(parts[pi], taps, st);
            else if (c->prec == 2) launch_conv_f16(parts[pi], taps, st);
            else launch_conv(parts[pi], taps, st);
        }
        launch_conv_splitk_reduce(a, st);
    };
    run();
    HIPCHK(c, hipEventRecord(c->ev0, st));
    for (int i = 0; i < iters; ++i) run();
    HIPCHK(c, hipEventRecord(c->ev1, st));
    HIPCHK(c, hipEventSynchronize(c->ev1));
    c->bench_out = out; c->bench_out_count = (int64_t)out_e * B;
    float ms = 0.f;
    HIPCHK(c, hipEventElapsedTime(&ms, c->ev0, c->ev1));
    *ms_avg = ms / iters;
    HIPCHK(c, hipGetLastError());
    return 0;
}

}
__global__ void diag_scale_tc(const float* tc, const float* mr, int C, int cpg, long n, int by_rstd, float* out) {
    const long i = (long)blockIdx.x * 256 + threadIdx.x;
    if (i >= n) return;
    const float f = by_rstd ? mr[2 * (int)((i % C) / cpg) + 1] : 1.0f;
    out[2 * i] = f * tc[2 * i];
    out[2 * i + 1] = f * tc[2 * i + 1];
}
extern "C" {
int loco_debug_conv(loco_ctx* c, const loco_conv_desc* d, char* plan, int64_t cap, void* stream) {
    if (!c) return -2;
    if (!d || d->struct_size != (int32_t)sizeof(loco_conv_desc)) { c->err = "debug_conv: descriptor size mismatch"; return -2; }
    if (finalize_params(c)) return -3;
    hipStream_t st = (hipStream_t)stream;
    const int taps = d->taps, k = taps == 9 ? 3 : 1, B = d->B;
    if ((taps != 9 && taps != 1) || d->Cin < 1 || d->Cout < 1 || d->Hin < 1 || d->Win < 1 || B < 1 || (d->stride != 1 && d->stride != 2) ||
        d->mode < CM_NONE || d->mode > CM_GN_GELU || (d->upsample && d->zins) || (d->stride == 2 && (d->upsample || d->zins)) ||
        !d->weight || !d->in || !d->out) { c->err = "debug_conv: bad descriptor"; return -2; }
    if (d->stride == 2 && ((d->Hin | d->Win) & 1)) { c->err = "debug_conv: stride 2 needs an even map"; return -2; }
    const bool lin = d->mode == CM_TAN_SILU || d->mode == CM_COT_SILU;
    if (d->mode != CM_NONE && (!d->sc || !d->sh)) { c->err = "debug_conv: the prologue modes need sc / sh"; return -2; }
    if (lin && (!d->prim || !d->mr || !d->gamma || !d->tst || !d->tc || d->cpg < 1 || d->Cin % d->cpg)) {
        c->err = "debug_conv: modes 3 / 4 need prim, mr, gamma, tst, tc and cpg"; return -2;
    }
    if (d->Cin2 > 0 && (!d->in2 || !d->w2)) { c->err = "debug_conv: the second operator needs in2 and w2"; return -2; }
    if (d->Cin2 > 0 && (d->res || d->accumulate || taps != 9)) {
        c->err = "debug_conv: the second operator goes with a 3x3 conv without res / accumulate"; return -2;
    }
    if (d->cot_d && (!d->cot_prim || !d->cot_sc || !d->cot_sh || !d->cot_mr || !d->cot_tc || d->cot_cpg < 1 || d->Cout % d->cot_cpg)) {
        c->err = "debug_conv: the norm-cotangent term needs cot_prim, cot_sc, cot_sh, cot_mr, cot_tc and cot_cpg"; return -2;
    }
    const int Hout = d->stride == 2 ? d->Hin / 2 : (d->upsample || d->zins) ? 2 * d->Hin : d->Hin;
    const int Wout = d->stride == 2 ? d->Win / 2 : (d->upsample || d->zins) ? 2 * d->Win : d->Win;
    {
        auto pow2 = [](int v) { return v >= 8 && (v & (v - 1)) == 0; };
        if (!((pow2(Hout) && pow2(Wout)) || (Wout % 32 == 0 && Hout % 8 == 0 && ((long)Hout * Wout) % 256 == 0))) {
            c->err = "debug_conv: output map outside the tile geometry of the conv kernels"; return -2;
        }
    }
    const long in_e = (long)d->Cin * d->Hin * d->Win, out_e = (long)d->Cout * Hout * Wout, in2_e = (long)d->Cin2 * Hout * Wout;
    if ((in_e | out_e | in2_e) & 3) { c->err = "debug_conv: planes must be whole 16-byte units"; return -2; }
    auto up64 = [](long v) { return (v + 63) & ~63L; };
    const long offT_in2 = d->in_arena ? up64(in_e * B) : 0, offT_cot = offT_in2 + up64(in2_e * B);
    const long needT = offT_cot + (d->cot_d ? out_e * B : 0);
    const long sx_cot = lin ? up64(in_e) : 0, need_sx = sx_cot + (d->cot_d ? out_e : 0);
    if (needT > (long)c->cfg.max_batch * c->prog->per_sample || (lin && in_e > (long)c->cfg.max_batch * c->prog->per_sample) ||
        need_sx > c->prog->sx_total) { c->err = "debug_conv: shape exceeds the arenas"; return -2; }
    const int G = lin ? d->Cin / d->cpg : 0;
    const long tbs = up64(2L * G) + up64(2L * d->Cin);
    const long small_n = (lin ? (long)B * tbs : 0) + (d->cot_d ? (long)B * up64(2L * d->Cout) : 0) + 64;
    const size_t owned0 = c->owned.size();
    const size_t bytes0 = c->bytes;
    auto release = [&]() {
        (void)hipStreamSynchronize(st);
        while (c->owned.size() > owned0) { (void)hipFree(c->owned.back()); c->owned.pop_back(); }
        c->bytes = bytes0;
    };
    auto host_param = [&](const float* p, std::vector<int64_t> shape) {
        HostParam h; h.shape = shape; h.loaded = true;
        size_t n = 1; for (int64_t s : shape) n *= (size_t)s;
        if (p) h.data.assign(p, p + n); else h.data.assign(n, 0.f);
        return h;
    };
    const int m_out = d->transposed ? d->Cin : d->Cout, m_in = d->transposed ? d->Cout : d->Cin;
    HostParam w = host_param(d->weight, {m_out, m_in, k, k}), wb0 = host_param(nullptr, {m_out});
    HostParam w2 = host_param(d->Cin2 > 0 ? d->w2 : nullptr, {d->Cout, d->Cin2 > 0 ? d->Cin2 : 1, 1, 1}), wb2 = host_param(nullptr, {d->Cout});
    ConvP cp, cp2;
    float *bias_d = nullptr, *bias2nd_d = nullptr, *small = nullptr;
    int rc = make_conv(c, {&w}, {&wb0}, &cp);
    if (!rc && d->Cin2 > 0) rc = make_conv(c, {&w2}, {&wb2}, &cp2);
    if (!rc && d->bias) rc = upload(c, &bias_d, std::vector<float>(d->bias, d->bias + d->Cout));
    if (!rc && d->Cin2 > 0 && d->bias2nd) rc = upload(c, &bias2nd_d, std::vector<float>(d->bias2nd, d->bias2nd + d->Cout));
    if (!rc) rc = dalloc(c, &small, (size_t)small_n);
    if (rc) { release(); return -1; }
    auto copy = [&](float* dst, const float* src, long n) {
        return hipMemcpyAsync(dst, src, (size_t)n * sizeof(float), hipMemcpyDeviceToDevice, st);
    };
    hipError_t he = hipSuccess;
    ConvArgs a; conv_defaults(a);
    if (d->in_arena) { he = copy(c->arenaT, d->in, in_e * B); a.in = c->arenaT; } else a.in = d->in;
    a.in_bs = in_e; a.Cin = d->Cin; a.Hin = d->Hin; a.Win = d->Win;
    setw(a, cp, d->transposed != 0);
    a.bias = bias_d;
    a.out = d->out; a.out_bs = out_e; a.Cout = d->Cout; a.Hout = Hout; a.Wout = Wout; a.B = B;
    a.bias2 = d->bias2; a.bias2_bs = d->Cout;
    a.res = d->res; a.res_bs = out_e; a.res_scale = d->res_scale;
    a.mode = d->mode; a.stride = d->stride; a.upsample = d->upsample; a.zins = d->zins; a.accumulate = d->accumulate;
    a.pad = d->pad >= 0 ? d->pad : taps == 1 ? 0 : d->zins ? 2 : d->stride == 2 ? 0 : 1;
    a.sc = d->sc; a.sh = d->sh; a.scsh_bs = 0; a.cpg = d->cpg;
    if (lin) {
        if (he == hipSuccess) he = copy(c->arenaP, d->prim, in_e);
        a.prim = c->arenaP; a.prim_bs = 0;
        a.mr = d->mr; a.mr_bs = 0; a.gamma_ = d->gamma;
        for (int b = 0; b < B && he == hipSuccess; ++b) he = copy(small + b * tbs, d->tst + (long)b * 2 * G, 2L * G);
        a.tst = small; a.tst_bs = tbs;
        for (int b = 0; b < B; ++b)
            hipLaunchKernelGGL(diag_scale_tc, dim3((unsigned)((d->Cin + 255) / 256)), dim3(256), 0, st, d->tc + (long)b * 2 * d->Cin, d->mr,
                               d->Cin, d->cpg, (long)d->Cin, d->mode == CM_COT_SILU ? 1 : 0, small + b * tbs + up64(2L * G));
        a.tc = small + up64(2L * G); a.tc_bs = tbs;
        launch_gn_cache(c->arenaP, d->Cin, d->Hin * d->Win, d->cpg, d->sc, d->sh, d->mr, c->sxcache, st, ACT_SILU);
        a.sx = c->sxcache;
    }
    ConvArgs n2; conv_defaults(n2);
    if (d->Cin2 > 0) {
        float* in2 = c->arenaT + offT_in2;
        if (he == hipSuccess) he = copy(in2, d->in2, in2_e * B);
        n2.in = in2; n2.in_bs = in2_e; n2.Cin = d->Cin2; n2.Hin = Hout; n2.Win = Wout;
        setw(n2, cp2, false); n2.bias = bias2nd_d; n2.pad = 0;
        n2.out = d->out; n2.out_bs = out_e; n2.Cout = d->Cout; n2.Hout = Hout; n2.Wout = Wout; n2.B = B;
        a.res = d->out; a.res_bs = out_e;
    }
    if (d->cot_d) {
        float* cd = c->arenaT + offT_cot;
        float* ctc = small + (lin ? (long)B * tbs : 0);
        const long cbs = up64(2L * d->Cout);
        if (he == hipSuccess) he = copy(cd, d->cot_d, out_e * B);
        for (int b = 0; b < B; ++b)
            hipLaunchKernelGGL(diag_scale_tc, dim3((unsigned)((d->Cout + 255) / 256)), dim3(256), 0, st, d->cot_tc + (long)b * 2 * d->Cout,
                               d->cot_mr, d->Cout, d->cot_cpg, (long)d->Cout, 1, ctc + b * cbs);
        launch_gn_cache(d->cot_prim, d->Cout, Hout * Wout, d->cot_cpg, d->cot_sc, d->cot_sh, d->cot_mr, c->sxcache + sx_cot, st, ACT_SILU);
        a.cot_d = cd; a.cot_d_bs = out_e; a.cot_sx = c->sxcache + sx_cot; a.cot_tc = ctc; a.cot_tc_bs = cbs;
    }
    if (he != hipSuccess) { c->err = std::string("debug_conv: ") + hipGetErrorString(he); release(); return -1; }
    std::string text;
    const int act0 = c->cfg.act;
    if (d->mode == CM_GN_GELU) c->cfg.act = ACT_GELU;
    c->plan_log = &text;
    const bool rode = run_conv(c, a, taps, st, nullptr, d->Cin2 > 0 ? &n2 : nullptr);
    c->plan_log = nullptr;
    c->cfg.act = act0;
    he = hipGetLastError();
    release();
    if (he == hipSuccess) he = hipGetLastError();
    if (he != hipSuccess) { c->err = std::string("debug_conv: ") + hipGetErrorString(he); return -1; }
    if (plan && cap > 0) {
        if ((int64_t)text.size() + 1 > cap) { c->err = "debug_conv: plan buffer too small"; return -4; }
        std::memcpy(plan, text.c_str(), text.size() + 1);
    }
    if (d->cot_d && !rode) { c->err = "debug_conv: norm-cotangent term declined"; return 1; }
    return 0;
}

#endif

int loco_set_streams(loco_ctx* c, int32_t n) {
    if (!c || (n != 1 && n != 2)) return -2;
    c->n_streams = n;
    return 0;
}

int loco_set_chip_share(loco_ctx* c, int32_t n) {
    if (!c || n < 1 || n > 8) return -2;
    c->chip_share = n;
    return 0;
}

int loco_set_side_stream(loco_ctx* c, void* stream) {
    if (!c) return -2;
    c->st2_user = (hipStream_t)stream;
    return 0;
}

int loco_profile_enable(loco_ctx* c, int32_t on) {
    if (!c) return -2;
    c->prof_on = on != 0;
    c->prof_shapes = on == 2;
    if (on) { c->prof.clear(); c->ev_used = 0; }
    return 0;
}

int loco_profile_report(loco_ctx* c, char* buf, int64_t cap) {
    if (!c || !buf || cap < 1) return -2;
    HIPCHK(c, hipDeviceSynchronize());
    std::map<std::string, std::array<double, 3>> agg;
    for (auto& r : c->prof) {
        float ms = 0.f;
        if (hipEventElapsedTime(&ms, r.e0, r.e1) != hipSuccess) continue;
        std::string key = r.name;
        if (c->prof_shapes) {
            char sb[96];
            snprintf(sb, sizeof(sb), "|t%d_m%d_ci%d_co%d_h%d_b%d_s%d", r.taps, r.mode, r.cin, r.cout, r.h, r.b, r.ns);
            key += sb;
        }
        auto& a = agg[key];
        a[0] += 1.0; a[1] += ms; a[2] += r.flops;
    }
    std::string out;
    char line[256];
    for (auto& kv : agg) {
        snprintf(line, sizeof(line), "%s %.0f %.6f %.6e\n", kv.first.c_str(), kv.second[0], kv.second[1], kv.second[2]);
        out += line;
    }
    if ((int64_t)out.size() + 1 > cap) { c->err = "profile buffer too small"; return -4; }
    std::memcpy(buf, out.c_str(), out.size() + 1);
    return 0;
}

#ifdef LOCO_DIAG
int64_t loco_debug_tensor(loco_ctx* c, const char* name, float* dst, int64_t cap, void* stream) {
    if (!c) return -2;
    std::string nm(name);
    if (nm == "bench_out") {
        if (!c->bench_out) { c->err = "no loco_bench_conv yet"; return -3; }
        int64_t cnt = cap < c->bench_out_count ? cap : c->bench_out_count;
// ... 32 lines not shown
```

### loco-edit_amd/csrc/kernels.h

```cpp
#pragma once
#include <hip/hip_runtime.h>
#include <stdint.h>

namespace loco {

struct DeviceOnce { bool seen[64] = {}; };
inline bool first_on_device(DeviceOnce& f) {
    int d = 0;
    (void)hipGetDevice(&d);
    d &= 63;
    if (f.seen[d]) return false;
    f.seen[d] = true;
    return true;
}


enum ConvMode : int {
    CM_NONE = 0,
    CM_GN_SILU = 1,
    CM_GN = 2,
    CM_TAN_SILU = 3,
    CM_COT_SILU = 4,
    CM_GN_GELU = 5,
};
enum ActKind : int { ACT_SILU = 0, ACT_GELU = 1 };
__device__ __forceinline__ float act_fwd(float y, int act) {
    if (act == ACT_GELU) return 0.5f * y * (1.0f + erff(y * 0.70710678118654752f));
    return y * (1.0f / (1.0f + __expf(-y)));
}
__device__ __forceinline__ float act_der(float y, int act) {
    if (act == ACT_GELU) return 0.5f * (1.0f + erff(y * 0.70710678118654752f)) + y * 0.39894228040143268f * __expf(-0.5f * y * y);
    const float sg = 1.0f / (1.0f + __expf(-y));
    return sg * (1.0f + y * (1.0f - sg));
}

enum StatKind : int { ST_NONE = 0, ST_FWD = 1, ST_TAN = 2, ST_COT = 3 };

struct ConvArgs {
    const float* in; long in_bs; int Cin, Hin, Win;
    const float* prim; long prim_bs;
    const float* w;
    const void* wb;
    const void* wh;
    const float2* sx;
    float* out; long out_bs; int Cout, Hout, Wout;
    const float* bias;
    const float* bias2; long bias2_bs;
    const float* res; long res_bs;
    const float* sc; const float* sh; long scsh_bs;
    const float* mr; long mr_bs;
    const float* gamma_;
    const float* tst; long tst_bs;
    const float* tc; long tc_bs;
    int cpg;
    int mode;
    int stride;
    int pad;
    int upsample;
    int zins;
    int in_padded;
    int accumulate;
    int nsplit;
    int taps;
    int no_deep;
    float* partial;
    int B;
    float* st_part; int st_kind;
    const float* st_x; const float2* st_sx;
    const float* in2; long in2_bs; int Cin2; int in2_padded;
    const void* wb2;
    const float* cot_d; long cot_d_bs; const float2* cot_sx; const float* cot_tc; long cot_tc_bs;
    int act;
    float res_scale;
    int dual;
    int gemm, gemm_tm;
    size_t partial_floats;
    int pers_groups;
    int tile, pair;
};

void launch_conv(const ConvArgs& a, int taps, hipStream_t st);
void launch_conv_bf16x3(const ConvArgs& a, int taps, hipStream_t st);
void launch_conv_f16(const ConvArgs& a, int taps, hipStream_t st);
void launch_conv_splitk_reduce(const ConvArgs& a, hipStream_t st);

struct ConvEnv {
    int prec = 1;
    int chip_share = 1;
    int lanes = 1, lane_s0 = 0;
    float* partial = nullptr; size_t partial_floats = 0;
    float* stpart = nullptr; size_t stpart_floats = 0;
    bool fuse_stats = true, fuse_lin = true, deep1 = true;
    int max_batch = 1;
};

struct StatAsk {
    int kind = ST_NONE;
    bool norm = false;
    const float2* sx = nullptr;
    const float* prim = nullptr;
    float* keep = nullptr; size_t keep_floats = 0;
};

enum StatRoute : int {
    SR_NONE = 0,
    SR_EPI = 1,
    SR_SPLITK = 2,
    SR_ALONE = 3,
    SR_KEEP = 4,
};

struct ConvLaunch {
    ConvArgs args;
    ConvArgs parts[2]; int nparts = 1;
    int s0 = 0;
    int stats = SR_NONE;
    int ntile = 0;
};

struct ConvPlan {
    bool sc_first = false;
    int nl = 1;
    ConvLaunch l[2];
    bool stats_all = false;
    int keep_ntile = 0;
    bool cot = false;
};

ConvPlan plan_conv(const ConvEnv& env, const ConvArgs& a, int taps, const StatAsk* ask, const ConvArgs* shortcut);
void conv_plan_family(ConvArgs& a, int prec);
int conv_plan_parts(ConvArgs& a, int prec, int tile_override, ConvArgs parts[2]);

int conv_bf16_tile_couts(const ConvArgs& a);
const char* conv_variant_name(const ConvArgs& a, int taps, int prec);

void launch_fill_random(float* p, long count, unsigned seed, float scale, hipStream_t st);
void launch_gn_cache(const float* x, int C, int HW, int cpg, const float* sc, const float* sh, const float* mr,
                     float2* sx, hipStream_t st, int act = 0);

struct GemmArgs {
    const float* A; long sam, sak, sab;
    const float* Bm; long sbk, sbn, sbb;
    float* C; long scm, scn, scb;
    const float* bias;
    const float* colbias;
    const float* R; long srb;
    int M, N, K, batch;
    float alpha, beta;
    int batch2; long sah, sbh, sch;
    const float* A2; long sab2; const float* Bm2; long sbb2;
};
void launch_gemm(const GemmArgs& g, hipStream_t st);
enum GemmAct : int { GEMM_ACT_NONE = 0, GEMM_ACT_QUICK_GELU = 1, GEMM_ACT_GELU = 2 };
void launch_gemm_fixed(const GemmArgs& g, int act, hipStream_t st);
void launch_gemm_bf16x3(const GemmArgs& g, hipStream_t st);
bool gemm_prefers_bf16x3(const GemmArgs& g);
bool gemm_rec_eligible(const GemmArgs& g);
size_t gemm_rec_ws_bytes(const GemmArgs& g);
void launch_gemm_rec(const GemmArgs& g, unsigned char* ws, hipStream_t st);

struct AttnFlashArgs {
    int T, NH, B, CH; float scale;
    const float *q, *k, *v; long hs;
    const float* P;
    const float* o;
    const float *dq, *dk, *dv; long bs_d;
    float* out; long bs_out;
    const float* go; long bs_go;
    float *gq, *gk, *gv; long bs_g;
    float* delta;
    int Lt; const float *kt, *vt;
    unsigned char* ws; size_t ws_bytes;
};
size_t attn_flash_ws_bytes(const AttnFlashArgs& a);
bool attn_flash_supported(int T, int CH);
bool attn_flash_text_supported(int T, int CH, int Lt);
void launch_attn_flash_tangent(const AttnFlashArgs& a, hipStream_t st);
void launch_attn_flash_cotangent(const AttnFlashArgs& a, hipStream_t st);

void launch_ln_fwd(const float* x, long xbs, int B, int C, int T, const float* gamma, const float* beta, float eps, float* y,
                   long ybs, float* stats, long sbs, hipStream_t st);
void launch_ln_tan(const float* dx, long dbs, const float* xprim, const float* sprim, int B, int C, int T, const float* gamma,
                   float* dy, long ybs, hipStream_t st);
void launch_ln_cot(const float* gy, long gbs, const float* xprim, const float* sprim, int B, int C, int T, const float* gamma,
                   const float* base, long base_bs, float* gx, long xbs, hipStream_t st);
struct XAttnArgs {
    int T, NH, B, CH, L, Lp, fwd;
    float alpha;
    const float* X; long x_bs;
    const float* K1; const float* K2;
    float* P; long p_bs;
    float* O; long o_bs;
};
bool xattn_fused_supported(int T, int CH, int L, int Lp);
void launch_xattn_fused(const XAttnArgs& a, hipStream_t st);
void launch_geglu(int kind, const float* in, long in_bs, const float* fprim, int B, long n4, float* out, long out_bs,
                  hipStream_t st);

void launch_gn_stats(const float* x, long bs, int B, int C, int HW, int G, float eps,
                     const float* gamma, const float* beta,
                     float* mr, float* sc, float* sh, long stats_bs, double* scratch, hipStream_t st,
                     const float* ss_scale = nullptr, const float* ss_shift = nullptr);
void launch_gn_fused_finalize_cat(const float* partA, int C1, int ntA, const float* partB, int ntB, int B, int C, int HW, int G,
                                  float eps, const float* gamma, const float* beta, float* mr, float* sc, float* sh,
                                  long stats_bs, hipStream_t st);
void launch_gn_fused_finalize(const float* part, int ntile, int B, int C, int HW, int G, float eps, const float* gamma,
                              const float* beta, float* mr, float* sc, float* sh, long stats_bs, const float* ss_scale,
                              const float* ss_shift, hipStream_t st);
void launch_gn_lin_fused_finalize(int kind, const float* partA, int C1, int ntA, const float* partB, int ntB, int B, int C, int HW,
                                  int G, const float* mr, float* tst, float* tc, long tst_bs, hipStream_t st);
void launch_conv_splitk_reduce_stats(const ConvArgs& a, int kind, int G, float eps, const float* gamma, const float* beta,
                                     float* mr, float* sc, float* sh, long stats_bs, const float* ss_scale,
                                     const float* ss_shift, const float* prim, const float* sc_prim, const float* sh_prim,
                                     const float* mr_prim, float* tst, float* tc, long tst_bs, double* scratch,
                                     hipStream_t st);
void launch_gn_tstats(const float* d, long d_bs, const float* x, long x_bs, int B, int C, int HW, int G,
                      const float* sc, const float* sh, const float* mr, long pbs_c, long pbs_g,
                      int kind, float* tst, float* tc, long tst_bs, double* scratch, hipStream_t st, int act = 0);
void launch_gn_apply(int kind, const float* d, long d_bs, const float* x, long x_bs,
                     const float* base, long base_bs, float* out, long out_bs, int accumulate,
                     int B, int C, int HW, int G, const float* sc, const float* sh, const float* mr,
                     long pbs_c, long pbs_g, const float* tst, long tst_bs, hipStream_t st, int act = 0,
                     float base_scale = 1.0f);

void launch_ctx_groupnorm(const float* tok, int L, int D, int G, float eps, const float* gamma, const float* beta,
                          float* out, hipStream_t st);

void launch_softmax_rows(float* S, long rows, int T, hipStream_t st, int B = 1, long bs = 0);
void launch_softmax_jac(float* dS, const float* P, long rows, int T, long p_rows, float scale, hipStream_t st,
                        int B = 1, long bs = 0);

void launch_temb(float t, int ch, int temb_ch, const float* freq, const float* w0, const float* b0,
                 const float* w1, const float* b1, float* scratch, hipStream_t st, int cos_first = 0,
                 const float* add = nullptr,
                 const float* t_ptr = nullptr,
                 int act = 0,
                 const float* add_in = nullptr);
void launch_set_scalar(float* p, float v, hipStream_t st);
void launch_clock_stamp(unsigned long long* out2, hipStream_t st);
void launch_temb_proj(const float* tact, int temb_ch, const float* w, const float* b, int cout,
                      float* out, hipStream_t st);
void launch_pool2x2_sum(const float* in, long in_bs, float* out, long out_bs, int accumulate,
                        int B, int C, int Hout, int Wout, hipStream_t st, float scale = 1.0f);
void launch_upsample2x(const float* in, long in_bs, float* out, long out_bs, int accumulate, float scale, int B,
                       int C, int Hin, int Win, hipStream_t st);
void launch_copy(const float* in, long in_bs, float* out, long out_bs, int accumulate,
                 int B, long per_sample, hipStream_t st);

void launch_ddim_step(const float* x, const float* eps, const float* noise, float* out, float* x0_out, long count,
                      float c_x0_x, float c_x0_e, float c_next_x0, float c_next_e, float c_noise,
                      hipStream_t st);
void launch_latent_sample(const float* mom, const float* noise, float scale, float* z, int B, long zhw, hipStream_t st);
void launch_masked_axpby(const float* V, const float* dE, const uint8_t* mask, float cv, float ce,
                         float* U, int k, long n, hipStream_t st, const uint8_t* mask2 = nullptr, long split = 0);
void launch_cot_seed(const float* U, const uint8_t* mask, float cv, float ce, float* gE, float* gX0,
                     int k, long n, hipStream_t st, const uint8_t* mask2 = nullptr, long split = 0);
void launch_add(const float* a, const float* b, float* out, long count, hipStream_t st);
void launch_lincomb(const float* const* src, const float* coef, int n, float* out, long count, hipStream_t st);
void launch_diffedit_mask(const float* eps_a, const float* eps_b, float scale, int B, int C, long HW, int rule, float* m,
                          uint8_t* mask, float* part, float* status, hipStream_t st);
void launch_cfg_masked_step(const float* x, const float* ef, const float* ee, const float* en, const uint8_t* mask, float* out,
                            int B, long n, float g, float c_x0_x, float c_x0_e, float c_next_x0, float c_next_e,
                            hipStream_t st);
void launch_lcm_step(const float* x, const float* eps, const float* noise, float* prev, float* den, long count, float sat,
                     float s1mat, float satp, float s1matp, float c_skip, float c_out, hipStream_t st);

void launch_gram(const float* A, int k, long n, double* G, double* scratch, hipStream_t st, const double* gate = nullptr);
void launch_cross_gram(const float* A, int k1, const float* B, int k2, long n, double* C, double* scratch,
                       hipStream_t st, const double* gate = nullptr);
constexpr int SOLVER_W_GATE = 64;
constexpr double SOLVER_W_FLOOR = 0x1p-47;
constexpr double SOLVER_REORTHO_RATIO = 1e-7;
void launch_jacobi_eig(double* G, int k, double* w, double* Q, hipStream_t st);
void launch_rotate_rows(const float* Ain, float* Aout, int k, long n, const double* Q, const double* w,
                        int mode, hipStream_t st);
void launch_sign_fix(float* A, int k, long n, float* s_out, const double* w, float* scratch, hipStream_t st);
void launch_cholesky(double* G, int k, hipStream_t st, double drop_below = 0.0, double* w = nullptr,
                     const double* gate = nullptr);
void launch_trsm_rows(const float* Ain, float* Aout, int k, long n, const double* L, hipStream_t st,
                      const double* gate = nullptr);
void launch_convergence(const float* a, const float* b, long count, float atol, float rtol, float* out2,
                        double* scratch, hipStream_t st);
void launch_convergence_rows(const float* a, const float* b, int k, long n, float atol, float rtol, float* out2,
                             double* scratch, hipStream_t st);
void launch_project_rows(const float* Vm, int k, const float* Vn, int k0, long n, const double* C,
                         float* out, hipStream_t st);
void launch_normalize_rows(float* A, int k, long n, double* scratch, hipStream_t st);
void launch_edit_axpy(const float* x, const float* v, const float* alphas_dev, int B, long n, float* out,
                      hipStream_t st);
void launch_mask_gather(const float* U, const int* idx, long L, long n, int k, float* out, hipStream_t st);
void launch_mask_compact(const uint8_t* mask, long n, int* idx, int* count, hipStream_t st);

}
```

### loco-edit_amd/csrc/misc.hip

```cpp
#include "kernels.h"

namespace loco {

typedef float f32x4_t __attribute__((ext_vector_type(4)));

__device__ __forceinline__ double wave_sum(double v) {
#pragma unroll
    for (int o = 32; o > 0; o >>= 1) v += __shfl_down(v, o, 64);
    return v;
}
__device__ __forceinline__ float wave_sumf(float v) {
#pragma unroll
    for (int o = 32; o > 0; o >>= 1) v += __shfl_down(v, o, 64);
    return v;
}
__device__ __forceinline__ float wave_maxf(float v) {
#pragma unroll
    for (int o = 32; o > 0; o >>= 1) v = fmaxf(v, __shfl_down(v, o, 64));
    return v;
}
__device__ __forceinline__ double block_sum(double v, double* sm) {
    v = wave_sum(v);
    __syncthreads();
    if ((threadIdx.x & 63) == 0) sm[threadIdx.x >> 6] = v;
// ... 433 lines not shown
        if (threadIdx.x == 0) {
            if (KIND == ST_FWD) {
                double* o = scratch + (((long)b * G + g) * nsl + s) * 3;
                const double n = (double)(end - beg), mu = n > 0 ? t1 / n : 0.0;
                o[0] = n; o[1] = mu; o[2] = t2;
            } else {
                double* o = scratch + (((long)b * G + g) * nsl + s) * 2;
                o[0] = t1; o[1] = t2;
            }
        }
        return;
    }
    const double inv_n = 1.0 / (double)len;
    if (KIND == ST_FWD) {
        const double mean = t1 * inv_n;
        double var = t2 * inv_n;
        if (var < 0.0) var = 0.0;
        const float meanf = (float)mean, rstd = (float)(1.0 / sqrt(var + (double)eps));
        if (threadIdx.x == 0) {
            mr[(long)b * sbs + g * 2] = meanf;
            mr[(long)b * sbs + g * 2 + 1] = rstd;
        }
        if (threadIdx.x < cpg) {
            const int c = g * cpg + threadIdx.x;
            const float gm = gamma[c];
            float aa = gm * rstd, oo = beta[c] - meanf * rstd * gm;
            if (ss_scale) {
                const float f = 1.0f + ss_scale[c];
                aa *= f;
                oo = oo * f + ss_shift[c];
            }
            sc[(long)b * sbs + c] = aa;
            sh[(long)b * sbs + c] = oo;
        }
    } else {
        const float m1 = (float)(t1 * inv_n), m2 = (float)(t2 * inv_n);
        if (threadIdx.x == 0) {
            tst[(long)b * tbs + 2 * g] = m1;
            tst[(long)b * tbs + 2 * g + 1] = m2;
        }
        if (tc && threadIdx.x < cpg) {
            const float f = KIND == ST_TAN ? 1.0f : rstd_p;
            float* t = tc + (long)b * tbs + 2 * ((long)g * cpg + threadIdx.x);
            t[0] = f * m1;
            t[1] = f * m2;
        }
    }
}

void launch_conv_splitk_reduce_stats(const ConvArgs& a, int kind, int G, float eps, const float* gamma, const float* beta,
                                     float* mr, float* sc, float* sh, long stats_bs, const float* ss_scale,
                                     const float* ss_shift, const float* prim, const float* sc_prim, const float* sh_prim,
                                     const float* mr_prim, float* tst, float* tc, long tst_bs, double* scratch,
                                     hipStream_t st) {
    const int HW = a.Hout * a.Wout, cpg = a.Cout / G;
    const long len = (long)cpg * HW;
    const int ns = gn_nsplit(len, a.B * G);
    dim3 grid(ns, G, a.B);
    long pieces = (len / ns + 3) / 4;
    int nthr = (int)((pieces + 63) / 64) * 64;
    if (nthr < 64) nthr = 64;
    if (nthr > 1024) nthr = 1024;
    if (nthr < cpg) nthr = ((cpg + 63) / 64) * 64;
#define RS(K) hipLaunchKernelGGL(splitk_reduce_stats_kernel<K>, grid, dim3(nthr), 0, st, a, G, eps, gamma, beta, mr, sc, sh, \
                                 stats_bs, ss_scale, ss_shift, prim, sc_prim, sh_prim, mr_prim, tst, tc, tst_bs, scratch)
    if (kind == ST_FWD) RS(ST_FWD); else if (kind == ST_TAN) RS(ST_TAN); else RS(ST_COT);
#undef RS
    if (ns == 1) return;
    if (kind == ST_FWD) {
        hipLaunchKernelGGL(gn_finalize_kernel, dim3((G + 63) / 64, a.B), dim3(64), 0, st, scratch, ns, G, a.Cout, eps, gamma,
                           beta, mr, sc, sh, stats_bs, ss_scale, ss_shift);
    } else {
        const long BG = (long)a.B * G;
        hipLaunchKernelGGL(gn_tstats_finalize, dim3((unsigned)((BG + 255) / 256)), dim3(256), 0, st, scratch, ns, BG, G,
                           1.0 / (double)len, tst, tc, tst_bs, cpg, mr_prim, 0L, kind == ST_TAN ? 0 : 1);
    }
}

template <int KIND>
__global__ __launch_bounds__(256) void gn_apply_kernel(const float* d, long d_bs, const float* x, long x_bs,
                                                       const float* base, long base_bs, float* out, long out_bs,
                                                       int accumulate, int C, int HW, int cpg, const float* sc,
                                                       const float* sh, const float* mr, long pbs_c, long pbs_g,
                                                       const float* tst, long tbs, int act, float base_scale) {
    const int b = blockIdx.y;
    const long per = (long)C * HW;
    for (long i = ((long)blockIdx.x * 256 + threadIdx.x) * 4; i < per; i += (long)gridDim.x * 1024) {
        int c = (int)(i / HW);
        int g = c / cpg;
        float scc = sc[(long)b * pbs_c + c], shc = sh[(long)b * pbs_c + c];
        float4 xv = *reinterpret_cast<const float4*>(x + (long)b * x_bs + i);
        float xx[4] = {xv.x, xv.y, xv.z, xv.w};
        float r[4];
        if (KIND == 0) {
#pragma unroll
            for (int j = 0; j < 4; ++j) r[j] = fmaf(scc, xx[j], shc);
        } else if (KIND == 4) {
#pragma unroll
            for (int j = 0; j < 4; ++j) r[j] = act_fwd(fmaf(scc, xx[j], shc), act);
        } else {
            float mean = mr[(long)b * pbs_g + 2 * g], rstd = mr[(long)b * pbs_g + 2 * g + 1];
            float m1 = tst[(long)b * tbs + g * 2], m2 = tst[(long)b * tbs + g * 2 + 1];
            float4 dv = *reinterpret_cast<const float4*>(d + (long)b * d_bs + i);
            float dd[4] = {dv.x, dv.y, dv.z, dv.w};
            float bb[4] = {0.f, 0.f, 0.f, 0.f};
            if (KIND >= 2 && base) {
                float4 bv = *reinterpret_cast<const float4*>(base + (long)b * base_bs + i);
                bb[0] = base_scale * bv.x; bb[1] = base_scale * bv.y; bb[2] = base_scale * bv.z; bb[3] = base_scale * bv.w;
            }
            float gm = scc / rstd;
#pragma unroll
            for (int j = 0; j < 4; ++j) {
                float xh = (xx[j] - mean) * rstd;
                if (KIND == 1) r[j] = scc * (dd[j] - m1 - xh * m2);
                else if (KIND == 5) r[j] = act_der(fmaf(scc, xx[j], shc), act) * scc * (dd[j] - m1 - xh * m2);
                else if (KIND == 2) r[j] = bb[j] + rstd * (gm * act_der(fmaf(scc, xx[j], shc), act) * dd[j] - m1 - xh * m2);
                else r[j] = bb[j] + rstd * (gm * dd[j] - m1 - xh * m2);
            }
        }
        float4* o = reinterpret_cast<float4*>(out + (long)b * out_bs + i);
        if (accumulate) {
            float4 ov = *o;
            r[0] += ov.x; r[1] += ov.y; r[2] += ov.z; r[3] += ov.w;
        }
        *o = make_float4(r[0], r[1], r[2], r[3]);
    }
}

void launch_gn_apply(int kind, const float* d, long d_bs, const float* x, long x_bs, const float* base,
                     long base_bs, float* out, long out_bs, int accumulate, int B, int C, int HW, int G,
                     const float* sc, const float* sh, const float* mr, long pbs_c, long pbs_g, const float* tst,
                     long tst_bs, hipStream_t st, int act, float base_scale) {
    long per = (long)C * HW;
    int blocks = (int)((per / 4 + 255) / 256);
    if (blocks > 1024) blocks = 1024;
    dim3 grid(blocks, B);
    int cpg = C / G;
#define GA(K) hipLaunchKernelGGL(gn_apply_kernel<K>, grid, dim3(256), 0, st, d, d_bs, x, x_bs, base, base_bs, out, \
                                 out_bs, accumulate, C, HW, cpg, sc, sh, mr, pbs_c, pbs_g, tst, tst_bs, act, base_scale)
    switch (kind) {
        case 0: GA(0); break;
        case 1: GA(1); break;
        case 2: GA(2); break;
        case 4: GA(4); break;
        case 5: GA(5); break;
        default: GA(3); break;
    }
#undef GA
}

__global__ __launch_bounds__(256) void gn_cache_kernel(const float* x, int C, int HW, int cpg, const float* sc,
                                                       const float* sh, const float* mr, float2* sx, int act) {
    const long per = (long)C * HW;
    for (long i = ((long)blockIdx.x * 256 + threadIdx.x) * 4; i < per; i += (long)gridDim.x * 1024) {
        int c = (int)(i / HW);
        int g = c / cpg;
        float scc = sc[c], shc = sh[c], mean = mr[2 * g], rstd = mr[2 * g + 1];
        float4 xv = *reinterpret_cast<const float4*>(x + i);
        float xx[4] = {xv.x, xv.y, xv.z, xv.w};
        float4 o0, o1;
        float r[8];
#pragma unroll
        for (int j = 0; j < 4; ++j) {
            r[2 * j] = scc * act_der(fmaf(scc, xx[j], shc), act);
            r[2 * j + 1] = (xx[j] - mean) * rstd;
        }
        o0 = make_float4(r[0], r[1], r[2], r[3]);
        o1 = make_float4(r[4], r[5], r[6], r[7]);
        float4* o = reinterpret_cast<float4*>(sx + i);
        o[0] = o0;
        o[1] = o1;
    }
}
void launch_gn_cache(const float* x, int C, int HW, int cpg, const float* sc, const float* sh, const float* mr,
                     float2* sx, hipStream_t st, int act) {
    long per = (long)C * HW;
    int blocks = (int)((per / 4 + 255) / 256);
    if (blocks > 2048) blocks = 2048;
    hipLaunchKernelGGL(gn_cache_kernel, dim3(blocks), dim3(256), 0, st, x, C, HW, cpg, sc, sh, mr, sx, act);
}

__global__ __launch_bounds__(256) void ctx_groupnorm_kernel(const float* tok, int L, int D, int cpg, float eps,
                                                            const float* gamma, const float* beta, float* out) {
    __shared__ double sm[4];
    const int g = blockIdx.x, n = L * cpg;
    double s1 = 0.0;
    for (int i = threadIdx.x; i < n; i += 256) s1 += (double)tok[(long)(i / cpg) * D + g * cpg + (i % cpg)];
    const double mean = block_sum(s1, sm) / (double)n;
    __syncthreads();
    double s2 = 0.0;
    for (int i = threadIdx.x; i < n; i += 256) {
        const double d = (double)tok[(long)(i / cpg) * D + g * cpg + (i % cpg)] - mean;
        s2 += d * d;
    }
    const double var = block_sum(s2, sm) / (double)n;
    const float mf = (float)mean, rstd = (float)(1.0 / sqrt(var + (double)eps));
    for (int i = threadIdx.x; i < n; i += 256) {
        const int c = g * cpg + (i % cpg);
        const long o = (long)(i / cpg) * D + c;
        out[o] = (tok[o] - mf) * rstd * gamma[c] + beta[c];
    }
}
void launch_ctx_groupnorm(const float* tok, int L, int D, int G, float eps, const float* gamma, const float* beta,
                          float* out, hipStream_t st) {
    hipLaunchKernelGGL(ctx_groupnorm_kernel, dim3(G), dim3(256), 0, st, tok, L, D, D / G, eps, gamma, beta, out);
}

__global__ __launch_bounds__(256) void softmax_rows_kernel(float* S, long rows, int T, long bs) {
    long row = (long)blockIdx.x * 4 + (threadIdx.x >> 6);
    if (row >= rows) return;
    const int lane = threadIdx.x & 63;
    float* p = S + (long)blockIdx.y * bs + row * T;
    float v[16];
    const int per = T / 64;
    float mx = -INFINITY;
    if (per > 16) {
        for (int i = 0; i < per; ++i) mx = fmaxf(mx, p[lane + i * 64]);
        mx = wave_maxf(mx);
        mx = __shfl(mx, 0, 64);
        float sum = 0.f;
        for (int i = 0; i < per; ++i) sum += expf(p[lane + i * 64] - mx);
        sum = wave_sumf(sum);
// ... 316 lines not shown
```

### loco-edit_amd/hip.py

```python
from __future__ import annotations

import ctypes as C
import os
from typing import Dict, Optional

import numpy as np
import torch

from .config import UNetConfig

_LIB_PATH = os.environ.get("LOCO_HIP_LIB") or os.path.join(os.path.dirname(os.path.abspath(__file__)), "libloco_hip.so")
_lib = None

DIAG_SYMBOLS = ["loco_bench_conv", "loco_debug_conv", "loco_debug_tensor"]

SYMBOLS = [
    "loco_version", "loco_device_count", "loco_create", "loco_fork", "loco_destroy", "loco_last_error",
    "loco_load_param", "loco_params_missing", "loco_unet_forward", "loco_ddim_step", "loco_sched_step",
    "loco_pmp_primal", "loco_pmp_set_second_mask", "loco_pmp_jvp", "loco_pmp_vjp", "loco_orthonormalize", "loco_qr_rows",
    "loco_convergence", "loco_convergence_rows", "loco_null_project", "loco_edit_axpy", "loco_mask_gather", "loco_mask_count",
    "loco_unet_flops", "loco_workspace_bytes", "loco_clock_stamp", "loco_set_side_stream", "loco_timer_start", "loco_timer_stop",
    "loco_profile_enable", "loco_profile_report", "loco_set_precision", "loco_get_precision", "loco_set_streams", "loco_set_chip_share",
    "loco_set_cond", "loco_set_context", "loco_lincomb", "loco_masked_axpby", "loco_latent_sample",
    "loco_text_create", "loco_text_load_param", "loco_text_params_missing", "loco_text_encode", "loco_text_last_error",
    "loco_text_destroy", "loco_t5_create", "loco_text_encode_masked",
    "loco_diffedit_mask", "loco_cfg_masked_step", "loco_set_time_cond", "loco_lcm_step",
    "loco_sam_create", "loco_sam_load_param", "loco_sam_params_missing", "loco_sam_encode", "loco_sam_profile",
    "loco_sam_profile_read", "loco_sam_last_error", "loco_sam_destroy",
]

DIFFEDIT_RULES = {"reference": 0, "intended": 1}


class LocoCfg(C.Structure):
    _fields_ = [
        ("struct_size", C.c_int32), ("resolution", C.c_int32), ("in_channels", C.c_int32), ("out_ch", C.c_int32), ("ch", C.c_int32),
        ("num_levels", C.c_int32), ("ch_mult", C.c_int32 * 8), ("num_res_blocks", C.c_int32),
        ("num_attn_res", C.c_int32), ("attn_resolutions", C.c_int32 * 8), ("gn_groups", C.c_int32),
        ("gn_eps", C.c_float), ("max_batch", C.c_int32),
        ("arch", C.c_int32), ("num_head_channels", C.c_int32), ("learn_sigma", C.c_int32),
        ("context_dim", C.c_int32), ("context_len", C.c_int32),
        ("scale_shift_norm", C.c_int32), ("resblock_updown", C.c_int32), ("num_heads", C.c_int32),
        ("transformer_depth", C.c_int32),
        ("act", C.c_int32), ("res_scale", C.c_float), ("added_kv", C.c_int32),
        ("time_cond_proj_dim", C.c_int32),
    ]


class LocoConvDesc(C.Structure):
    _PTRS = ("weight", "bias", "in", "bias2", "res", "prim", "sc", "sh", "mr", "gamma", "tst", "tc", "in2", "w2", "bias2nd",
             "cot_d", "cot_prim", "cot_sc", "cot_sh", "cot_mr", "cot_tc", "out")
    _HOST = ("weight", "bias", "w2", "bias2nd")
    _fields_ = ([("struct_size", C.c_int32)] +
                [(k, C.c_int32) for k in ("Cin", "Cout", "Hin", "Win", "B", "taps", "stride", "upsample", "zins", "mode", "cpg",
                                          "transposed", "accumulate", "in_arena", "pad", "Cin2", "cot_cpg")] +
                [("res_scale", C.c_float), ("reserved", C.c_int32)] + [(k, C.c_void_p) for k in _PTRS])


class LocoTextCfg(C.Structure):
    _fields_ = [("vocab", C.c_int32), ("width", C.c_int32), ("layers", C.c_int32), ("heads", C.c_int32), ("ffn", C.c_int32),
                ("positions", C.c_int32), ("act", C.c_int32), ("ln_eps", C.c_float)]


class LocoT5Cfg(C.Structure):
    _fields_ = [("vocab", C.c_int32), ("d_model", C.c_int32), ("d_kv", C.c_int32), ("heads", C.c_int32), ("d_ff", C.c_int32),
                ("layers", C.c_int32), ("positions", C.c_int32), ("buckets", C.c_int32), ("max_distance", C.c_int32),
                ("act", C.c_int32), ("ln_eps", C.c_float)]


SAM_MAX_GLOBAL = 16


class LocoSamCfg(C.Structure):
    _fields_ = [("image_size", C.c_int32), ("patch_size", C.c_int32), ("width", C.c_int32), ("depth", C.c_int32),
                ("heads", C.c_int32), ("mlp_dim", C.c_int32), ("window_size", C.c_int32), ("num_global", C.c_int32),
                ("global_attn", C.c_int32 * SAM_MAX_GLOBAL), ("out_channels", C.c_int32), ("ln_eps", C.c_float)]


def library_path() -> str:
    return _LIB_PATH


def load_library():
    global _lib
    if _lib is not None:
        return _lib
    if not os.path.exists(_LIB_PATH):
        raise RuntimeError(
            f"{_LIB_PATH} not found: build it with `python -c 'import __graft_entry__ as g; g.build()'` "
            "(hipcc --offload-arch=gfx950). There is no CPU fallback.")
    lib = C.CDLL(_LIB_PATH)
    vp, i32, i64, f32 = C.c_void_p, C.c_int32, C.c_int64, C.c_float
    lib.loco_version.restype = C.c_char_p
    lib.loco_device_count.restype = C.c_int
    lib.loco_create.argtypes = [C.POINTER(LocoCfg), C.POINTER(vp)]
    if hasattr(lib, "loco_fork"):
        lib.loco_fork.argtypes = [vp, C.c_int32, C.POINTER(vp)]
    lib.loco_destroy.argtypes = [vp]
    lib.loco_destroy.restype = None
    lib.loco_last_error.argtypes = [vp]
    lib.loco_last_error.restype = C.c_char_p
    lib.loco_load_param.argtypes = [vp, C.c_char_p, vp, C.POINTER(i64), i32, i32]
    lib.loco_params_missing.argtypes = [vp]
    lib.loco_unet_forward.argtypes = [vp, vp, f32, i32, vp, vp]
    lib.loco_ddim_step.argtypes = [vp, vp, f32, f32, f32, f32, vp, i32, vp, vp]
    lib.loco_sched_step.argtypes = [vp, vp, vp, f32, f32, f32, vp, i64, vp, vp, vp]
    lib.loco_pmp_primal.argtypes = [vp, vp, f32, f32, vp, i32, vp]
    lib.loco_pmp_set_second_mask.argtypes = [vp, vp, i32, vp]
    lib.loco_pmp_jvp.argtypes = [vp, vp, i32, vp, vp]
    lib.loco_pmp_vjp.argtypes = [vp, vp, i32, vp, vp]
    lib.loco_orthonormalize.argtypes = [vp, vp, i32, i64, vp, vp]
    lib.loco_qr_rows.argtypes = [vp, vp, i32, i64, vp]
    lib.loco_convergence.argtypes = [vp, vp, vp, i64, f32, vp, vp]
    lib.loco_convergence_rows.argtypes = [vp, vp, vp, i32, i64, f32, vp, vp]
    lib.loco_null_project.argtypes = [vp, vp, i32, vp, i32, i64, vp, vp]
    lib.loco_edit_axpy.argtypes = [vp, vp, vp, C.POINTER(f32), i32, i64, vp, vp]
    lib.loco_mask_gather.argtypes = [vp, vp, i32, vp, vp]
    lib.loco_mask_count.argtypes = [vp]
    lib.loco_mask_count.restype = i64
    lib.loco_clock_stamp.argtypes = [vp, vp, vp]
    lib.loco_set_side_stream.argtypes = [vp, vp]
    lib.loco_unet_flops.argtypes = [vp]
    lib.loco_unet_flops.restype = C.c_double
    lib.loco_workspace_bytes.argtypes = [vp]
    lib.loco_workspace_bytes.restype = i64
    lib.loco_timer_start.argtypes = [vp, vp]
    lib.loco_timer_stop.argtypes = [vp, vp, C.POINTER(f32)]
    lib.loco_set_precision.argtypes = [vp, i32]
    lib.loco_get_precision.argtypes = [vp]
    lib.loco_set_streams.argtypes = [vp, i32]
    lib.loco_set_chip_share.argtypes = [vp, i32]
    lib.loco_set_cond.argtypes = [vp, vp, vp]
    lib.loco_set_context.argtypes = [vp, vp, vp]
    lib.loco_masked_axpby.argtypes = [vp, vp, vp, f32, f32, i32, vp, vp]
    lib.loco_latent_sample.argtypes = [vp, vp, vp, f32, i32, vp, vp]
    lib.loco_lincomb.argtypes = [vp, C.POINTER(vp), C.POINTER(f32), i32, vp, i64, vp]
    lib.loco_diffedit_mask.argtypes = [vp, vp, vp, f32, i32, i32, i64, i32, vp, vp, vp]
    lib.loco_cfg_masked_step.argtypes = [vp, vp, vp, vp, vp, f32, f32, f32, vp, i32, i64, vp, vp]
    lib.loco_set_time_cond.argtypes = [vp, vp, vp]
    lib.loco_lcm_step.argtypes = [vp, vp, vp, f32, f32, f32, f32, vp, i64, vp, vp, vp]
    lib.loco_profile_enable.argtypes = [vp, i32]
    lib.loco_profile_report.argtypes = [vp, C.c_char_p, i64]
    if hasattr(lib, "loco_text_create"):
        lib.loco_text_create.argtypes = [C.POINTER(LocoTextCfg), i32, i32, C.POINTER(vp)]
        lib.loco_text_load_param.argtypes = [vp, C.c_char_p, vp, C.POINTER(i64), i32]
        lib.loco_text_params_missing.argtypes = [vp]
        lib.loco_text_encode.argtypes = [vp, vp, i32, vp, vp]
        lib.loco_text_last_error.argtypes = [vp]
        lib.loco_text_last_error.restype = C.c_char_p
        lib.loco_text_destroy.argtypes = [vp]
        lib.loco_text_destroy.restype = None
    if hasattr(lib, "loco_t5_create"):
        lib.loco_t5_create.argtypes = [C.POINTER(LocoT5Cfg), i32, i32, C.POINTER(vp)]
        lib.loco_text_encode_masked.argtypes = [vp, vp, C.POINTER(i32), i32, vp, vp]
    if hasattr(lib, "loco_sam_create"):
        lib.loco_sam_create.argtypes = [C.POINTER(LocoSamCfg), i32, C.POINTER(vp)]
        lib.loco_sam_load_param.argtypes = [vp, C.c_char_p, vp, C.POINTER(i64), i32]
        lib.loco_sam_params_missing.argtypes = [vp]
        lib.loco_sam_encode.argtypes = [vp, vp, vp, vp]
        lib.loco_sam_profile.argtypes = [vp, i32]
        lib.loco_sam_profile_read.argtypes = [vp, C.POINTER(f32)]
        lib.loco_sam_last_error.argtypes = [vp]
        lib.loco_sam_last_error.restype = C.c_char_p
        lib.loco_sam_destroy.argtypes = [vp]
        lib.loco_sam_destroy.restype = None
    if hasattr(lib, "loco_bench_conv"):
        lib.loco_bench_conv.argtypes = [vp, i32, i32, i32, i32, i32, i32, i32, i32, i32, C.POINTER(f32), vp]
        lib.loco_debug_tensor.argtypes = [vp, C.c_char_p, vp, i64, vp]
        lib.loco_debug_tensor.restype = i64
    if hasattr(lib, "loco_debug_conv"):
        lib.loco_debug_conv.argtypes = [vp, C.POINTER(LocoConvDesc), C.c_char_p, i64, vp]
    _lib = lib
    return lib


def _ptr(t: Optional[torch.Tensor]):
    return None if t is None else C.c_void_p(t.data_ptr())


def _stream():
    return C.c_void_p(torch.cuda.current_stream().cuda_stream)


def _chk_dev(t: torch.Tensor, dtype=torch.float32):
    if not t.is_cuda:
        raise ValueError("loco_hip operates on device tensors only")
    if t.dtype != dtype:
        raise ValueError(f"expected {dtype}, got {t.dtype}")
    if not t.is_contiguous():
        raise ValueError("tensor must be contiguous")


def c_cfg(cfg: UNetConfig, max_batch: int) -> LocoCfg:
    c = LocoCfg()
    c.struct_size = C.sizeof(LocoCfg)
    c.resolution, c.in_channels, c.out_ch, c.ch = cfg.resolution, cfg.in_channels, cfg.out_ch, cfg.ch
    c.num_levels = len(cfg.ch_mult)
    for i, m in enumerate(cfg.ch_mult):
        c.ch_mult[i] = m
    c.num_res_blocks = cfg.num_res_blocks
    c.num_attn_res = len(cfg.attn_resolutions)
    for i, r in enumerate(cfg.attn_resolutions):
        c.attn_resolutions[i] = r
    c.gn_groups, c.gn_eps, c.max_batch = cfg.gn_groups, cfg.gn_eps, int(max_batch)
    c.arch = {"ddpm": 0, "adm": 1, "dec": 2, "enc": 3}[cfg.arch]
    c.num_head_channels, c.learn_sigma = cfg.num_head_channels, int(cfg.learn_sigma)
    c.context_dim, c.context_len = cfg.context_dim, cfg.context_len
    c.scale_shift_norm, c.resblock_updown = int(cfg.scale_shift_norm), int(cfg.resblock_updown)
    c.num_heads, c.transformer_depth = cfg.num_heads, cfg.transformer_depth
    c.act, c.res_scale, c.added_kv = {"silu": 0, "gelu": 1}[cfg.act], float(cfg.res_scale), int(cfg.added_kv)
    c.time_cond_proj_dim = int(cfg.time_cond_proj_dim)
    return c


class LocoEngine:

    def __init__(self, cfg: UNetConfig, max_batch: int = 8, device: Optional[torch.device] = None):
        self.lib = load_library()
        if not torch.cuda.is_available() or self.lib.loco_device_count() < 1:
            raise RuntimeError("loco_hip: no HIP device visible; the hot path has no CPU fallback")
        self.device = torch.device(device if device is not None else "cuda:0")
        torch.cuda.set_device(self.device)
        self.cfg = cfg
        self.max_batch = int(max_batch)
        c = c_cfg(cfg, self.max_batch)
        self._ctx = C.c_void_p()
        rc = self.lib.loco_create(C.byref(c), C.byref(self._ctx))
        if rc != 0:
            msg = self.lib.loco_last_error(self._ctx).decode() if self._ctx else "?"
            raise RuntimeError(f"loco_create failed ({rc}): {msg}")
        self.n = cfg.n
        self.n_out = cfg.n_out

    def fork(self, max_batch: Optional[int] = None) -> "LocoEngine":
        child = object.__new__(LocoEngine)
        child.lib, child.cfg, child.device = self.lib, self.cfg, self.device
        child.max_batch = int(max_batch or self.max_batch)
        child.n, child.n_out = self.n, self.n_out
        for k, v in self.__dict__.items():
            if k not in child.__dict__ and k != "_ctx":
                child.__dict__[k] = v
        child._ctx = C.c_void_p()
        torch.cuda.set_device(self.device)
        rc = self.lib.loco_fork(self._ctx, child.max_batch, C.byref(child._ctx))
        if rc != 0:
            msg = self.lib.loco_last_error(child._ctx).decode() if child._ctx else self.lib.loco_last_error(self._ctx).decode()
            raise RuntimeError(f"loco_fork failed ({rc}): {msg}")
        return child

    def __del__(self):
# ... 276 lines not shown
        if eps.shape != x.shape:
            raise ValueError(f"x and eps must share a shape, got {tuple(x.shape)} and {tuple(eps.shape)}")
        if noise is not None:
            _chk_dev(noise)
            if noise.shape != x.shape:
                raise ValueError(f"noise must be {tuple(x.shape)}, got {tuple(noise.shape)}")
        if not (want_prev or want_denoised):
            raise ValueError("lcm_step: ask for prev, denoised or both")
        prev = None
        if want_prev:
            prev = torch.empty_like(x) if out is None else out
            if out is not None:
                _chk_dev(out)
                if out.shape != x.shape:
                    raise ValueError(f"out must be {tuple(x.shape)}, got {tuple(out.shape)}")
        den = torch.empty_like(x) if want_denoised else None
        self._check(self.lib.loco_lcm_step(self._ctx, _ptr(x), _ptr(eps), float(at), float(at_prev), float(c_skip), float(c_out),
                                           _ptr(noise), x.numel(), _ptr(prev), _ptr(den), _stream()), "loco_lcm_step")
        return prev, den

    def version(self) -> str:
        return self.lib.loco_version().decode()

    def clock_stamp(self) -> torch.Tensor:
        out = torch.zeros(2, device=self.device, dtype=torch.int64)
        self._check(self.lib.loco_clock_stamp(self._ctx, _ptr(out), _stream()), "loco_clock_stamp")
        return out

    @staticmethod
    def sclk_mhz(stamp0: torch.Tensor, stamp1: torch.Tensor) -> float:
        d = (stamp1 - stamp0).tolist()
        return 100.0 * d[0] / max(d[1], 1)

    def unet_flops(self) -> float:
        return float(self.lib.loco_unet_flops(self._ctx))

    def workspace_bytes(self) -> int:
        return int(self.lib.loco_workspace_bytes(self._ctx))

    def timer_start(self):
        self._check(self.lib.loco_timer_start(self._ctx, _stream()), "loco_timer_start")

    def timer_stop(self) -> float:
        ms = C.c_float()
        self._check(self.lib.loco_timer_stop(self._ctx, _stream(), C.byref(ms)), "loco_timer_stop")
        return float(ms.value)

    PRECISIONS = {"f32": 0, "bf16x3": 1, "f16": 2}

    def set_precision(self, mode: str):
        self._check(self.lib.loco_set_precision(self._ctx, self.PRECISIONS[mode]), "loco_set_precision")

    def set_streams(self, n: int):
        self._check(self.lib.loco_set_streams(self._ctx, int(n)), "loco_set_streams")

    def set_chip_share(self, n: int):
        self._check(self.lib.loco_set_chip_share(self._ctx, int(n)), "loco_set_chip_share")

    def set_side_stream(self, stream: "Optional[torch.cuda.Stream]"):
        self._side_stream = stream
        ptr = C.c_void_p(stream.cuda_stream) if stream is not None else None
        self._check(self.lib.loco_set_side_stream(self._ctx, ptr), "loco_set_side_stream")

    def set_streams_measured(self, n: int):
        if n == 2:
            from .tloco import BranchStreams
            side = BranchStreams._pick(1, self.device)
            if not side:
                self.set_streams(1)
                return 1
            self.set_side_stream(side[0])
        self.set_streams(n)
        return n

    def get_precision(self) -> str:
        m = self.lib.loco_get_precision(self._ctx)
        return {v: k for k, v in self.PRECISIONS.items()}[m]

    def _need_diag(self, sym):
        if not hasattr(self.lib, sym):
            raise RuntimeError(f"{sym} is a diagnostic of include/loco_hip_diag.h: build `make -C loco-edit_amd/csrc diag` "
                               "and set LOCO_HIP_LIB=<repo>/loco-edit_amd/libloco_hip_diag.so")

    def bench_conv(self, cin, cout, H, W, B, mode, taps=9, tile=-1, iters=20) -> float:
        self._need_diag("loco_bench_conv")
        ms = C.c_float()
        self._check(self.lib.loco_bench_conv(self._ctx, cin, cout, H, W, B, mode, taps, tile, iters, C.byref(ms),
                                             _stream()), "loco_bench_conv")
        return float(ms.value)

    def debug_conv(self, out: torch.Tensor, **desc):
        self._need_diag("loco_debug_conv")
        d = LocoConvDesc()
        d.struct_size = C.sizeof(LocoConvDesc)
        d.stride, d.in_arena, d.pad, d.res_scale = 1, 1, -1, 1.0
        keep = []
        _chk_dev(out)
        d.out = out.data_ptr()
        for k, v in desc.items():
            if k not in LocoConvDesc._PTRS:
                if not hasattr(d, k) or k in ("struct_size", "reserved"):
                    raise TypeError(f"debug_conv: no descriptor field {k!r}")
                setattr(d, k, v)
            elif v is not None:
                if k in LocoConvDesc._HOST:
                    v = v.detach().to("cpu", torch.float32).contiguous()
                else:
                    _chk_dev(v)
                keep.append(v)
                setattr(d, k, v.data_ptr())
        buf = C.create_string_buffer(1 << 12)
        rc = self.lib.loco_debug_conv(self._ctx, C.byref(d), buf, len(buf), _stream())
        if rc not in (0, 1):
            self._check(rc, "loco_debug_conv")
        plan = []
        for line in buf.value.decode().splitlines():
            rec = dict(f.split("=", 1) for f in line.split(" "))
            plan.append({k: (v if k == "kernel" else int(v)) for k, v in rec.items()})
        return plan, rc == 0

    def profile_enable(self, on):
        self._check(self.lib.loco_profile_enable(self._ctx, int(on)), "loco_profile_enable")

    def profile_report(self):
        buf = C.create_string_buffer(1 << 18)
        self._check(self.lib.loco_profile_report(self._ctx, buf, len(buf)), "loco_profile_report")
        out = {}
        for line in buf.value.decode().splitlines():
            name, n, ms, fl = line.rsplit(" ", 3)
            out[name] = dict(launches=int(float(n)), ms=float(ms), flops=float(fl))
        return out

    def debug_tensor(self, name: str, numel: int) -> torch.Tensor:
        self._need_diag("loco_debug_tensor")
        dst = torch.empty(numel, device=self.device, dtype=torch.float32)
        got = self.lib.loco_debug_tensor(self._ctx, name.encode(), _ptr(dst), numel, _stream())
        if got < 0:
            raise RuntimeError(f"loco_debug_tensor({name}) failed: {self.lib.loco_last_error(self._ctx).decode()}")
        return dst[:got]


class _EncoderEngine:
    _prefix = ""
    _label = ""

    def _open(self, device: Optional[torch.device]):
        self.lib = load_library()
        if not torch.cuda.is_available() or self.lib.loco_device_count() < 1:
            raise RuntimeError(f"loco_hip: no HIP device visible; the {self._label} has no CPU fallback")
        self.device = torch.device(device if device is not None else "cuda:0")
        if self.device.index is None:
            self.device = torch.device("cuda", torch.cuda.current_device())
        self._t = C.c_void_p()

    def _fn(self, name):
        return getattr(self.lib, f"{self._prefix}_{name}")

    def _create(self, what, c_cfg, *args):
        rc = getattr(self.lib, what)(C.byref(c_cfg), self.device.index, *args, C.byref(self._t))
        if rc != 0:
            raise RuntimeError(f"{what} failed ({rc}): {self._fn('last_error')(None).decode()}")

    def __del__(self):
        try:
            if getattr(self, "_t", None):
                self._fn("destroy")(self._t)
                self._t = None
        except Exception:
            pass

    def _check(self, rc, what):
        if rc != 0:
            raise RuntimeError(f"{what} failed ({rc}): {self._fn('last_error')(self._t).decode()}")

    def load_params(self, sd: Dict[str, "np.ndarray | torch.Tensor"]):
        if any(isinstance(v, torch.Tensor) and v.is_cuda for v in sd.values()):
            torch.cuda.synchronize()
        for name, v in sd.items():
            t = torch.as_tensor(np.asarray(v) if not isinstance(v, torch.Tensor) else v).detach().to(torch.float32).contiguous()
            if not t.is_cuda:
                t = t.cpu()
            shape = (C.c_int64 * max(t.dim(), 1))(*t.shape)
            self._check(self._fn("load_param")(self._t, name.encode(), C.c_void_p(t.data_ptr()), shape, t.dim()),
                        f"{self._prefix}_load_param({name})")
# ... 101 lines not shown
```

Measured before the change: 19.90 edit-directions/s.

## Add specialised end-conv kernels and mask row-window skipping for stem/head convs

Adds two specialised 3x3 conv kernels for the network's ends. One targets few-output-channel convs (Cout*9<=32): it puts the taps into the MFMA M dimension and reduces the shifted partials through shared memory. The other targets few-input-channel convs (Cin*9<=32) and uses an im2col-style K of at most 32. It also computes a device-side row window from the edit mask, so tiles outside the masked rows can exit early and the GN-apply backward can skip loading rows outside it. This is meant to cut wasted MFMA padding and wasted work on unmasked rows. The cost is extra kernel paths and the correctness risk of the mask-derived windowing.

```diff
diff --git a/include/loco_hip_diag.h b/include/loco_hip_diag.h
--- a/include/loco_hip_diag.h
+++ b/include/loco_hip_diag.h
@@ -6,7 +6,7 @@
 #endif
 
 int  loco_bench_conv(loco_ctx* ctx, int32_t cin, int32_t cout, int32_t H, int32_t W, int32_t B, int32_t mode,
-                     int32_t taps, int32_t tile, int32_t iters, float* ms_avg, void* stream);
+                     int32_t taps, int32_t tile, int32_t iters, float* ms_avg, void* stream, int32_t win_y0, int32_t win_y1);
 
 typedef struct loco_conv_desc {
     int32_t struct_size;
@@ -15,13 +15,15 @@
     int32_t transposed, accumulate, in_arena, pad;
     int32_t Cin2, cot_cpg;
     float   res_scale;
-    int32_t reserved;
+    int32_t st_kind;
     const float *weight, *bias;
     const float *in, *bias2, *res;
     const float *prim, *sc, *sh, *mr, *gamma, *tst, *tc;
     const float *in2, *w2, *bias2nd;
     const float *cot_d, *cot_prim, *cot_sc, *cot_sh, *cot_mr, *cot_tc;
     float* out;
+    const int32_t* rowwin;
+    float* st_part;
 } loco_conv_desc;
 int  loco_debug_conv(loco_ctx* ctx, const loco_conv_desc* desc, char* plan, int64_t cap, void* stream);
 
diff --git a/loco-edit_amd/csrc/conv_bf16.hip b/loco-edit_amd/csrc/conv_bf16.hip
--- a/loco-edit_amd/csrc/conv_bf16.hip
+++ b/loco-edit_amd/csrc/conv_bf16.hip
@@ -43,6 +43,10 @@
     }
 #endif
     if constexpr (PR == PR_BF16X3) {
+        if (taps == 9 && a.ends == 1) { launch_conv_fewcout(a, st); return; }
+        if (taps == 9 && a.ends == 2) { launch_conv_fewcin(a, st); return; }
+    }
+    if constexpr (PR == PR_BF16X3) {
         if (taps == 9 && a.pair) {
             switch (a.mode) {
                 case CM_NONE: launch_pair_b<PR, CM_NONE>(a, st); break;
diff --git a/loco-edit_amd/csrc/conv_ends.hip b/loco-edit_amd/csrc/conv_ends.hip
--- /dev/null
+++ b/loco-edit_amd/csrc/conv_ends.hip
@@ -0,0 +1,263 @@
+#include "conv_bf16_kernel.h"
+
+namespace loco {
+
+constexpr int FC_TH = 8, FC_TW = 32;
+constexpr int FC_HW = FC_TW + 2, FC_HH = FC_TH + 2;
+constexpr int FC_HALO = FC_HW * FC_HH;
+constexpr int FC_NT = (FC_HALO + 31) / 32;
+constexpr int FC_PITCH = FC_NT * 32;
+constexpr int FC_ROWS = 27;
+constexpr int FC_NW = 4;
+constexpr int FC_PER = (FC_NT + FC_NW - 1) / FC_NW;
+
+template <int MODE>
+__global__ __launch_bounds__(FC_NW * 64) void conv_fewcout_bf16x3(ConvArgs a) {
+    static_assert(MODE == CM_NONE || MODE == CM_GN_SILU || MODE == CM_TAN_SILU, "prologues of the few-cout kernel");
+    __shared__ float P[FC_ROWS * FC_PITCH];
+    const int tid = threadIdx.x, lane = tid & 63, wave = tid >> 6, l31 = lane & 31, kh = lane >> 5;
+    const int tiles_x = a.Wout / FC_TW, ntile = tiles_x * (a.Hout / FC_TH);
+    int tile_id, b;
+    {
+        const int L = blockIdx.x;
+        if ((ntile & 7) == 0) { const int q = L >> 3, t8 = q / a.B; b = q - t8 * a.B; tile_id = t8 * 8 + (L & 7); }
+        else { tile_id = L / a.B; b = L - tile_id * a.B; }
+    }
+    const int ty0 = tile_id / tiles_x;
+    const int oy0 = ty0 * FC_TH, ox0 = (tile_id - ty0 * tiles_x) * FC_TW;
+    int y0 = 0, y1 = a.Hout - 1;
+    if (a.rowwin) { y0 = a.rowwin[0]; y1 = a.rowwin[1]; }
+    if (oy0 + FC_TH - 1 < y0 || oy0 > y1) return;
+
+    const long plane = (long)a.Hin * a.Win;
+    const float* const inb = a.in + (long)b * a.in_bs;
+    unsigned poff[FC_PER];
+    bool pval[FC_PER];
+#pragma unroll
+    for (int i = 0; i < FC_PER; ++i) {
+        const int p = (wave + FC_NW * i) * 32 + l31;
+        const int py = p / FC_HW, px = p - py * FC_HW;
+        const int iy = oy0 - 1 + py, ix = ox0 - 1 + px;
+        pval[i] = p < FC_HALO && iy >= 0 && iy < a.Hin && ix >= 0 && ix < a.Win;
+        poff[i] = pval[i] ? (unsigned)(iy * a.Win + ix) : 0u;
+    }
+    const int coutP = (a.Cout + 31) & ~31;
+    const bool rval = l31 < a.Cout * 9;
+    const int rco = l31 / 9, rtap = l31 - rco * 9;
+    const float* const wrow = a.w + (rval ? rtap * coutP + rco : 0);
+    const long wstride = 9L * coutP;
+    const float* const scb = MODE == CM_GN_SILU ? a.sc + (long)b * a.scsh_bs : nullptr;
+    const float* const shb = MODE == CM_GN_SILU ? a.sh + (long)b * a.scsh_bs : nullptr;
+    const f32x2* const tcb = MODE == CM_TAN_SILU ? reinterpret_cast<const f32x2*>(a.tc + (long)b * a.tc_bs) : nullptr;
+
+    f32x16 acc[FC_PER];
+#pragma unroll
+    for (int i = 0; i < FC_PER; ++i)
+#pragma unroll
+        for (int r = 0; r < 16; ++r) acc[i][r] = 0.f;
+
+    for (int c0 = 0; c0 < a.Cin; c0 += BKC) {
+        const int cb = c0 + 8 * kh;
+        float d[FC_PER][8];
+        float2 pv[MODE == CM_TAN_SILU ? FC_PER : 1][8];
+#pragma unroll
+        for (int i = 0; i < FC_PER; ++i) {
+            if (wave + FC_NW * i >= FC_NT) continue;
+#pragma unroll
+            for (int j = 0; j < 8; ++j) {
+                const long o = (long)(cb + j) * plane + poff[i];
+                d[i][j] = inb[o];
+                if constexpr (MODE == CM_TAN_SILU) pv[i][j] = a.sx[o];
+            }
+        }
+        float wv[8], cA[8], cB[8];
+#pragma unroll
+        for (int j = 0; j < 8; ++j) {
+            const float w = wrow[(long)(cb + j) * wstride];
+            wv[j] = rval ? w : 0.f;
+            if constexpr (MODE == CM_GN_SILU) { cA[j] = scb[cb + j]; cB[j] = shb[cb + j]; }
+            if constexpr (MODE == CM_TAN_SILU) { const f32x2 t = tcb[cb + j]; cA[j] = t[0]; cB[j] = t[1]; }
+        }
+        uint4 ah4, al4;
+        split8<PR_BF16X3>(wv, ah4, al4);
+        const bf16x8 ah = __builtin_bit_cast(bf16x8, ah4), al = __builtin_bit_cast(bf16x8, al4);
+#pragma unroll
+        for (int i = 0; i < FC_PER; ++i) {
+            if (wave + FC_NW * i >= FC_NT) continue;
+            float v[8];
+#pragma unroll
+            for (int j = 0; j < 8; ++j) {
+                float r = d[i][j];
+                if constexpr (MODE == CM_GN_SILU) {
+                    const float y = fmaf(cA[j], r, cB[j]);
+                    r = y * sigmoidf2_(y);
+                } else if constexpr (MODE == CM_TAN_SILU) {
+                    r = pv[i][j].x * fmaf(-pv[i][j].y, cB[j], r - cA[j]);
+                }
+                v[j] = pval[i] ? r : 0.f;
+            }
+            uint4 bh4, bl4;
+            split8<PR_BF16X3>(v, bh4, bl4);
+            const bf16x8 bh = __builtin_bit_cast(bf16x8, bh4), bl = __builtin_bit_cast(bf16x8, bl4);
+            acc[i] = __builtin_amdgcn_mfma_f32_32x32x16_bf16(al, bh, acc[i], 0, 0, 0);
+            acc[i] = __builtin_amdgcn_mfma_f32_32x32x16_bf16(ah, bl, acc[i], 0, 0, 0);
+            acc[i] = __builtin_amdgcn_mfma_f32_32x32x16_bf16(ah, bh, acc[i], 0, 0, 0);
+        }
+    }
+#pragma unroll
+    for (int i = 0; i < FC_PER; ++i) {
+        if (wave + FC_NW * i >= FC_NT) continue;
+#pragma unroll
+        for (int r = 0; r < 16; ++r) {
+            const int row = (r & 3) + 8 * (r >> 2) + 4 * kh;
+            if (row < FC_ROWS) P[row * FC_PITCH + (wave + FC_NW * i) * 32 + l31] = acc[i][r];
+        }
+    }
+    __syncthreads();
+    const int ty = tid >> 5, tx = tid & 31;
+    const int oy = oy0 + ty, ox = ox0 + tx;
+    if (oy < y0 || oy > y1) return;
+    const long out_plane = (long)a.Hout * a.Wout;
+    float* const ob = a.out + (long)b * a.out_bs;
+    const float* const rb = a.res ? a.res + (long)b * a.res_bs : nullptr;
+    const float* const b2 = a.bias2 ? a.bias2 + (long)b * a.bias2_bs : nullptr;
+    for (int co = 0; co < a.Cout; ++co) {
+        const float* const pc = P + co * 9 * FC_PITCH + ty * FC_HW + tx;
+        float s = 0.f;
+#pragma unroll
+        for (int ky = 0; ky < 3; ++ky)
+#pragma unroll
+            for (int kx = 0; kx < 3; ++kx) s += pc[(ky * 3 + kx) * FC_PITCH + ky * FC_HW + kx];
+        const long off = co * out_plane + (long)oy * a.Wout + ox;
+        if (a.bias) s += a.bias[co];
+        if (b2) s += b2[co];
+        if (rb) s += a.res_scale * rb[off];
+        if (a.accumulate) s += ob[off];
+        ob[off] = s;
+    }
+}
+
+void launch_conv_fewcout(const ConvArgs& a, hipStream_t st) {
+    const dim3 grid((unsigned)((a.Hout / FC_TH) * (a.Wout / FC_TW) * a.B)), block(FC_NW * 64);
+    switch (a.mode) {
+        case CM_NONE: hipLaunchKernelGGL(conv_fewcout_bf16x3<CM_NONE>, grid, block, 0, st, a); break;
+        case CM_GN_SILU: hipLaunchKernelGGL(conv_fewcout_bf16x3<CM_GN_SILU>, grid, block, 0, st, a); break;
+        default: hipLaunchKernelGGL(conv_fewcout_bf16x3<CM_TAN_SILU>, grid, block, 0, st, a); break;
+    }
+}
+
+constexpr int CI_WM = 2, CI_WN = 4, CI_TM = 2, CI_TN = 2;
+
+__global__ __launch_bounds__(CI_WM * CI_WN * 64) void conv_fewcin_bf16x3(ConvArgs a) {
+    extern __shared__ __attribute__((aligned(16))) unsigned char smem_b[];
+    constexpr int MT = CI_WM * CI_TM * 32, NT = CI_WN * CI_TN * 32;
+    const int tid = threadIdx.x, lane = tid & 63, wave = tid >> 6, l31 = lane & 31, kh = lane >> 5;
+    const int wm = wave / CI_WN, wn = wave % CI_WN;
+    const int tiles_x = a.Wout / 32, ntile = (a.Hout * a.Wout) / NT, ncot = (a.Cout + MT - 1) / MT;
+    int tile_id, cot_id, b;
+    {
+        const int L = blockIdx.x;
+        if ((ntile & 7) == 0) {
+            const int q = L >> 3, q2 = q / ncot, t8 = q2 / a.B;
+            cot_id = q - q2 * ncot; b = q2 - t8 * a.B; tile_id = t8 * 8 + (L & 7);
+        } else {
+            const int T = L / a.B;
+            b = L - T * a.B; cot_id = T / ntile; tile_id = T - cot_id * ntile;
+        }
+    }
+    const int ty0 = tile_id / tiles_x;
+    const int oy0 = ty0 * 8, ox0 = (tile_id - ty0 * tiles_x) * 32, co0 = cot_id * MT;
+    if (a.rowwin) {
+        const int y0 = a.rowwin[0], y1 = a.rowwin[1];
+        if (y0 > y1 || oy0 + 7 < y0 - 1 || oy0 > y1 + 1) {
+            if (a.st_part && a.st_kind != ST_NONE && tid < MT && co0 + tid < a.Cout) {
+                float* const sp = a.st_part + (((long)b * a.Cout + co0 + tid) * ntile + tile_id) * 2;
+                sp[0] = 0.f; sp[1] = 0.f;
+            }
+            return;
+        }
+    }
+    const long plane = (long)a.Hin * a.Win;
+    const float* const inb = a.in + (long)b * a.in_bs;
+    const int coutP = (a.Cout + 31) & ~31, K = a.Cin * 9;
+    f32x16 acc[CI_TM][CI_TN];
+#pragma unroll
+    for (int i = 0; i < CI_TM; ++i)
+#pragma unroll
+        for (int j = 0; j < CI_TN; ++j)
+#pragma unroll
+            for (int r = 0; r < 16; ++r) acc[i][j][r] = 0.f;
+#pragma unroll
+    for (int ks = 0; ks < 2; ++ks) {
+        const int kb = ks * 16 + 8 * kh;
+        bf16x8 ah[CI_TM], al[CI_TM], bh[CI_TN], bl[CI_TN];
+#pragma unroll
+        for (int i = 0; i < CI_TM; ++i) {
+            const int co = co0 + (wm * CI_TM + i) * 32 + l31;
+            float wv[8];
+#pragma unroll
+            for (int j = 0; j < 8; ++j) {
+                const bool ok = kb + j < K && co < a.Cout;
+                const float w = a.w[ok ? (long)(kb + j) * coutP + co : 0];
+                wv[j] = ok ? w : 0.f;
+            }
+            uint4 h4, l4;
+            split8<PR_BF16X3>(wv, h4, l4);
+            ah[i] = __builtin_bit_cast(bf16x8, h4); al[i] = __builtin_bit_cast(bf16x8, l4);
+        }
+#pragma unroll
+        for (int jn = 0; jn < CI_TN; ++jn) {
+            const int oy = oy0 + wn * CI_TN + jn, ox = ox0 + l31;
+            float v[8];
+#pragma unroll
+            for (int j = 0; j < 8; ++j) {
+                const int k = kb + j, ci = k / 9, t = k - ci * 9, ky = t / 3, kx = t - ky * 3;
+                const int iy = oy + ky - 1, ix = ox + kx - 1;
+                const bool ok = k < K && iy >= 0 && iy < a.Hin && ix >= 0 && ix < a.Win;
+                const float x = inb[ok ? ci * plane + (long)iy * a.Win + ix : 0];
+                v[j] = ok ? x : 0.f;
+            }
+            uint4 h4, l4;
+            split8<PR_BF16X3>(v, h4, l4);
+            bh[jn] = __builtin_bit_cast(bf16x8, h4); bl[jn] = __builtin_bit_cast(bf16x8, l4);
+        }
+#pragma unroll
+        for (int i = 0; i < CI_TM; ++i)
+#pragma unroll
+            for (int jn = 0; jn < CI_TN; ++jn) {
+                acc[i][jn] = __builtin_amdgcn_mfma_f32_32x32x16_bf16(al[i], bh[jn], acc[i][jn], 0, 0, 0);
+                acc[i][jn] = __builtin_amdgcn_mfma_f32_32x32x16_bf16(ah[i], bl[jn], acc[i][jn], 0, 0, 0);
+                acc[i][jn] = __builtin_amdgcn_mfma_f32_32x32x16_bf16(ah[i], bh[jn], acc[i][jn], 0, 0, 0);
+            }
+    }
+    conv_lowp_epilogue<CI_WM, CI_WN, CI_TM, CI_TN, EPI_STATS>(a, acc, smem_b, co0, oy0, ox0, 32, tile_id, b, 0);
+}
+
+void launch_conv_fewcin(const ConvArgs& a, hipStream_t st) {
+    constexpr int MT = CI_WM * CI_TM * 32, NT = CI_WN * CI_TN * 32;
+    const dim3 grid((unsigned)(((a.Hout * a.Wout) / NT) * ((a.Cout + MT - 1) / MT) * a.B));
+    hipLaunchKernelGGL(conv_fewcin_bf16x3, grid, dim3(CI_WM * CI_WN * 64), (size_t)CI_WM * 32 * NT * 4, st, a);
+}
+
+__global__ __launch_bounds__(256) void mask_rowwin_kernel(const uint8_t* mask, const uint8_t* mask2, int C, int H, int W, int* win) {
+    __shared__ int lo, hi;
+    if (threadIdx.x == 0) { lo = H; hi = -1; }
+    __syncthreads();
+    int mylo = H, myhi = -1;
+    for (int r = threadIdx.x; r < C * H; r += 256) {
+        const int y = r % H;
+        if (y >= mylo && y <= myhi) continue;
+        const long base = (long)r * W;
+        unsigned any = 0;
+        for (int x = 0; x < W; ++x) any |= mask[base + x] | (mask2 ? mask2[base + x] : 0);
+        if (any) { mylo = y < mylo ? y : mylo; myhi = y > myhi ? y : myhi; }
+    }
+    if (myhi >= 0) { atomicMin(&lo, mylo); atomicMax(&hi, myhi); }
+    __syncthreads();
+    if (threadIdx.x == 0) { win[0] = lo; win[1] = hi; }
+}
+void launch_mask_rowwin(const uint8_t* mask, const uint8_t* mask2, int C, int H, int W, int* win, hipStream_t st) {
+    hipLaunchKernelGGL(mask_rowwin_kernel, dim3(1), dim3(256), 0, st, mask, mask2, C, H, W, win);
+}
+
+}
diff --git a/loco-edit_amd/csrc/conv_plan.hip b/loco-edit_amd/csrc/conv_plan.hip
--- a/loco-edit_amd/csrc/conv_plan.hip
+++ b/loco-edit_amd/csrc/conv_plan.hip
@@ -104,6 +104,21 @@
     return a.tile == 5;
 }
 
+bool conv_ends_enabled() {
+    static const bool on = env_int("LOCO_END_CONVS", 1) != 0;
+    return on;
+}
+static int conv_ends_ok(const ConvArgs& a, int prec) {
+    if (!conv_ends_enabled() || prec != 1 || a.taps != 9 || a.stride != 1 || a.pad != 1 || a.upsample || a.zins || a.Cin2 > 0 || a.nsplit != 1 ||
+        (a.Wout % 32) != 0 || (a.Hout % 8) != 0 || a.Hout * a.Wout < 4096 || a.gemm || a.dual || a.pers_groups || a.cot_d)
+        return 0;
+    if (a.Cout * 9 <= 32 && (a.Cin % BKC) == 0 && !a.st_part &&
+        (a.mode == CM_NONE || a.mode == CM_GN_SILU || (a.mode == CM_TAN_SILU && a.sx)))
+        return 1;
+    if (a.Cin * 9 <= 32 && a.mode == CM_NONE && a.tile == 5) return 2;
+    return 0;
+}
+
 static bool conv_dual_ok(const ConvArgs& a) {
     static const bool on = diag_switch("LOCO_CONV_DUAL") != 0;
     if (!on || a.taps != 9 || a.Cin2 > 0 || a.nsplit != 1 || a.stride != 1 || a.upsample || a.zins || a.pad != 1 || (a.Cin % BKC) != 0 ||
@@ -202,6 +217,8 @@
         ConvArgs& p = parts[i];
         p.tile = tile_for(p, prec, tile_override);
         p.pair = prec == 1 && conv_pair_ok(p);
+        p.ends = conv_ends_ok(p, prec);
+        if (!p.ends) p.rowwin = nullptr;
     }
     return n;
 }
@@ -326,6 +343,7 @@
     static const char* tiles[6] = {"2,2,2,2", "4,1,1,2", "1,4,1,1", "2,2,1,1", "2,2,2,4", "2,4,2,2"};
     static char names[3][2][6][6][56];
     static char others[5][3][6][40];
+    static char ends[2][6][6][64];
     const int mode = (a.mode < 0 || a.mode > 5) ? 2 : a.mode;
     const char* other = nullptr;
     int k = 0, v = mode;
@@ -341,6 +359,11 @@
     }
     int t = a.tile == 6 ? 0 : a.tile;
     if (t < 0 || t > 5) t = 0;
+    if (prec == 1 && taps == 9 && (a.ends == 1 || a.ends == 2)) {
+        char* n = ends[a.ends - 1][t][mode];
+        if (!n[0]) snprintf(n, 64, "conv_mfma_bf16x3<9,%s,%d>:%s", tiles[t], mode, a.ends == 1 ? "conv_fewcout_bf16x3" : "conv_fewcin_bf16x3");
+        return n;
+    }
     int m = mode;
     if (taps != 9 && m != CM_NONE) m = CM_GN;
     if (!prec && m == CM_GN_GELU) m = CM_GN_SILU;
diff --git a/loco-edit_amd/csrc/conv_plan_text.h b/loco-edit_amd/csrc/conv_plan_text.h
--- a/loco-edit_amd/csrc/conv_plan_text.h
+++ b/loco-edit_amd/csrc/conv_plan_text.h
@@ -12,9 +12,9 @@
         for (int pi = 0; pi < l.nparts; ++pi) {
             const ConvArgs& y = l.parts[pi];
             snprintf(line, sizeof(line),
-                     "launch=%d part=%d kernel=%s tile=%d nsplit=%d B=%d s0=%d gemm=%d gemm_tm=%d pair=%d Cin2=%d sc_first=%d cot=%d\n",
+                     "launch=%d part=%d kernel=%s tile=%d nsplit=%d B=%d s0=%d gemm=%d gemm_tm=%d pair=%d Cin2=%d sc_first=%d cot=%d ends=%d\n",
                      li, pi, conv_variant_name(y, taps, prec), y.tile, l.args.nsplit, y.B, l.s0 + (pi ? l.args.B - y.B : 0), y.gemm,
-                     y.gemm ? y.gemm_tm : 0, y.pair, y.Cin2, p.sc_first ? 1 : 0, p.cot ? 1 : 0);
+                     y.gemm ? y.gemm_tm : 0, y.pair, y.Cin2, p.sc_first ? 1 : 0, p.cot ? 1 : 0, y.ends);
             out += line;
         }
     }
diff --git a/loco-edit_amd/csrc/engine.hip b/loco-edit_amd/csrc/engine.hip
--- a/loco-edit_amd/csrc/engine.hip
+++ b/loco-edit_amd/csrc/engine.hip
@@ -141,6 +141,8 @@
     int mask2_from = 0;
     int* mask_idx = nullptr;
     int* mask_L_dev = nullptr;
+    int* mask_win = nullptr;
+    bool mask_win_ok = false;
     long mask_L = 0;
     hipStream_t mask_stream = nullptr;
     int primal_B = 0;
@@ -1202,7 +1204,7 @@
 
 constexpr size_t RED_BYTES = (size_t)4 << 20;
 
-int tangent_pass(loco_ctx* c, const float* V, int B, hipStream_t st) {
+int tangent_pass(loco_ctx* c, const float* V, int B, hipStream_t st, const int* rowwin = nullptr) {
     const loco_unet_cfg& cfg = c->cfg;
     const long PS = c->prog->per_sample;
     auto TP = [&](int id) { return c->arenaP + c->tens[id].off; };
@@ -1418,6 +1420,7 @@
                 setw(a, op.conv, false);
                 set_tan(c, a, op.n1, TP(op.in));
                 a.out = TT(op.out); a.out_bs = PS; a.Cout = to.C; a.Hout = to.H; a.Wout = to.W; a.B = B;
+                if (op.out == c->prog->eps_t) a.rowwin = rowwin;
                 run_conv(c, a, 9, st);
                 break;
             }
@@ -1434,7 +1437,7 @@
                      stt.tc, c->prog->stats_per_sample, c->red, st, c->cfg.act);
 }
 
-int cotangent_pass(loco_ctx* c, const float* ge, const float* gx0, float* Aout, int B, hipStream_t st) {
+int cotangent_pass(loco_ctx* c, const float* ge, const float* gx0, float* Aout, int B, hipStream_t st, const int* rowwin = nullptr) {
     const loco_unet_cfg& cfg = c->cfg;
     const long PS = c->prog->per_sample;
     const int G = cfg.gn_groups;
@@ -1454,6 +1457,8 @@
                 a.in = GO(op); a.in_bs = GOS(op); a.Cin = to.C; a.Hin = to.H; a.Win = to.W;
                 setw(a, op.conv, true);
                 a.out = TG(op.a1); a.out_bs = PS; a.Cout = ti.C; a.Hout = ti.H; a.Wout = ti.W; a.B = B;
+                const int* const win = (op.out == c->prog->eps_t && conv_ends_enabled() && (ti.W % 4) == 0) ? rowwin : nullptr;
+                a.rowwin = win;
                 {
                     const StatReq rq = req_lin(c, ST_COT, &op.n1, TP(op.in));
                     run_conv(c, a, 9, st, &rq);
@@ -1462,7 +1467,7 @@
                 NS sp = nstats(c, c->statsP, op.n1);
                 NS stt = nstats(c, c->statsT, op.n1);
                 launch_gn_apply(2, TG(op.a1), PS, TP(op.in), 0, nullptr, 0, TG(op.in), PS, 0, B, ti.C, ti.H * ti.W, G,
-                                sp.sc, sp.sh, sp.mr, 0, 0, stt.tst, c->prog->stats_per_sample, st, cfg.act);
+                                sp.sc, sp.sh, sp.mr, 0, 0, stt.tst, c->prog->stats_per_sample, st, cfg.act, 1.0f, win, ti.W);
                 break;
             }
             case OP_UP: {
@@ -1800,7 +1805,7 @@
     }
     if (dalloc(c, &c->mask2, (size_t)c->prog->n_out)) return -1;
     if (dalloc(c, &c->mask, (size_t)c->prog->n_out) || dalloc(c, &c->mask_idx, (size_t)c->prog->n_out) ||
-        dalloc(c, &c->mask_L_dev, 4)) return -1;
+        dalloc(c, &c->mask_L_dev, 4) || dalloc(c, &c->mask_win, 4)) return -1;
     HIPCHK(c, hipEventCreate(&c->ev0));
     HIPCHK(c, hipEventCreate(&c->ev1));
     {
@@ -2024,6 +2029,11 @@
     if (mask) {
         HIPCHK(c, hipMemcpyAsync(c->mask, mask, (size_t)c->prog->n_out, hipMemcpyDeviceToDevice, st));
         launch_mask_compact(c->mask, c->prog->n_out, c->mask_idx, c->mask_L_dev, st);
+        {
+            const Tens& te = c->tens[c->prog->eps_t];
+            c->mask_win_ok = (long)te.C * te.H * te.W == (long)c->prog->n_out;
+            if (c->mask_win_ok) launch_mask_rowwin(c->mask, nullptr, te.C, te.H, te.W, c->mask_win, st);
+        }
         c->mask_L = -1;
         c->mask_stream = st;
     }
@@ -2035,10 +2045,16 @@
 int loco_pmp_set_second_mask(loco_ctx* c, const uint8_t* mask2, int32_t from_row, void* stream) {
     if (!c) return -2;
     if (!c->primal_ok) { c->err = "loco_pmp_primal has not been called"; return -2; }
-    if (!mask2) { c->has_mask2 = false; return 0; }
+    const Tens& te = c->tens[c->prog->eps_t];
+    if (!mask2) {
+        if (c->has_mask2 && c->mask_win_ok) launch_mask_rowwin(c->mask, nullptr, te.C, te.H, te.W, c->mask_win, (hipStream_t)stream);
+        c->has_mask2 = false;
+        return 0;
+    }
     if (!c->has_mask) { c->err = "a second mask needs a first one (loco_pmp_primal with mask)"; return -2; }
     if (from_row < 0) { c->err = "from_row must be >= 0"; return -2; }
     HIPCHK(c, hipMemcpyAsync(c->mask2, mask2, (size_t)c->prog->n_out, hipMemcpyDeviceToDevice, (hipStream_t)stream));
+    if (c->mask_win_ok) launch_mask_rowwin(c->mask, c->mask2, te.C, te.H, te.W, c->mask_win, (hipStream_t)stream);
     c->has_mask2 = true;
     c->mask2_from = from_row;
     return 0;
@@ -2053,7 +2069,7 @@
         int B = (k - b0 < MB) ? k - b0 : MB;
         int rc = run_lanes(c, B, st, [&](int s0, int nb, hipStream_t ls) -> int {
             const float* Vc = V + (long)(b0 + s0) * c->prog->n_in;
-            if (tangent_pass(c, Vc, nb, ls)) return -1;
+            if (tangent_pass(c, Vc, nb, ls, c->has_mask && c->mask_win_ok ? c->mask_win : nullptr)) return -1;
             launch_copy(c->arenaT + c->tens[c->prog->eps_t].off, c->prog->per_sample, c->eps_buf, c->prog->n_out, 0, nb, c->prog->n_out, ls);
             launch_masked_axpby(c->prog->n_out == c->prog->n_in ? Vc : nullptr, c->eps_buf, c->has_mask ? c->mask : nullptr, c->p_cv,
                                 c->p_ce, U + (long)(b0 + s0) * c->prog->n_out, nb, c->prog->n_out, ls,
@@ -2078,7 +2094,8 @@
             launch_cot_seed(U + (long)(b0 + s0) * c->prog->n_out, c->has_mask ? c->mask : nullptr, c->p_cv, c->p_ce, c->ge,
                             same ? c->gx0 : nullptr, nb, c->prog->n_out, ls, c->has_mask2 ? c->mask2 : nullptr,
                             (long)c->mask2_from - (b0 + s0));
-            return cotangent_pass(c, c->ge, same ? c->gx0 : nullptr, A + (long)(b0 + s0) * c->prog->n_in, nb, ls);
+            return cotangent_pass(c, c->ge, same ? c->gx0 : nullptr, A + (long)(b0 + s0) * c->prog->n_in, nb, ls,
+                                  c->has_mask && c->mask_win_ok ? c->mask_win : nullptr);
         });
         if (rc) return rc;
     }
@@ -2396,10 +2413,12 @@
 }
 extern "C" {
 int loco_bench_conv(loco_ctx* c, int32_t cin, int32_t cout, int32_t H, int32_t W, int32_t B, int32_t mode,
-                    int32_t taps, int32_t tile, int32_t iters, float* ms_avg, void* stream) {
+                    int32_t taps, int32_t tile, int32_t iters, float* ms_avg, void* stream, int32_t win_y0, int32_t win_y1) {
     if (!c) return -2;
     if (finalize_params(c)) return -3;
     hipStream_t st = (hipStream_t)stream;
+    const int win[2] = {win_y0, win_y1};
+    if (win_y0 >= 0) HIPCHK(c, hipMemcpy(c->mask_win + 2, win, sizeof(win), hipMemcpyHostToDevice));
     const long HW = (long)H * W;
     const long in_e = (long)cin * HW, out_e = (long)cout * HW;
     if ((in_e + out_e) * B > (long)c->cfg.max_batch * c->prog->per_sample || 2 * in_e > (long)c->prog->per_sample ||
@@ -2442,6 +2461,7 @@
         a.cot_d = out + out_e * B; a.cot_d_bs = out_e; a.cot_sx = c->sxcache; a.cot_tc = c->statsT; a.cot_tc_bs = c->prog->stats_per_sample;
     }
     if (getenv("LOCO_BENCH_ACC") && atoi(getenv("LOCO_BENCH_ACC"))) a.accumulate = 1;
+    if (win_y0 >= 0) a.rowwin = c->mask_win + 2;
     conv_plan_family(a, c->prec);
     if (const char* e = getenv("LOCO_DUAL_WHATIF")) a.no_deep = atoi(e);
     ConvArgs parts[2];
@@ -2511,7 +2531,13 @@
     auto up64 = [](long v) { return (v + 63) & ~63L; };
     const long offT_in2 = d->in_arena ? up64(in_e * B) : 0, offT_cot = offT_in2 + up64(in2_e * B);
     const long needT = offT_cot + (d->cot_d ? out_e * B : 0);
-    const long sx_cot = lin ? up64(in_e) : 0, need_sx = sx_cot + (d->cot_d ? out_e : 0);
+    const bool st_cot = d->st_kind == ST_COT;
+    if (d->st_kind != ST_NONE && (!d->st_part || (d->st_kind != ST_FWD && !st_cot) || d->cot_d || (d->Cout % 128) != 0 ||
+                                  (st_cot && (!d->cot_prim || !d->cot_sc || !d->cot_sh || !d->cot_mr || d->cot_cpg < 1 || d->Cout % d->cot_cpg)))) {
+        c->err = "debug_conv: epilogue statistics need st_part, kind 1 or 3 (with cot_prim, cot_sc, cot_sh, cot_mr, cot_cpg), whole 128-cout tiles, no cot_d";
+        return -2;
+    }
+    const long sx_cot = lin ? up64(in_e) : 0, need_sx = sx_cot + ((d->cot_d || st_cot) ? out_e : 0);
     if (needT > (long)c->cfg.max_batch * c->prog->per_sample || (lin && in_e > (long)c->cfg.max_batch * c->prog->per_sample) ||
         need_sx > c->prog->sx_total) { c->err = "debug_conv: shape exceeds the arenas"; return -2; }
     const int G = lin ? d->Cin / d->cpg : 0;
@@ -2556,6 +2582,7 @@
     a.mode = d->mode; a.stride = d->stride; a.upsample = d->upsample; a.zins = d->zins; a.accumulate = d->accumulate;
     a.pad = d->pad >= 0 ? d->pad : taps == 1 ? 0 : d->zins ? 2 : d->stride == 2 ? 0 : 1;
     a.sc = d->sc; a.sh = d->sh; a.scsh_bs = 0; a.cpg = d->cpg;
+    a.rowwin = d->rowwin;
     if (lin) {
         if (he == hipSuccess) he = copy(c->arenaP, d->prim, in_e);
         a.prim = c->arenaP; a.prim_bs = 0;
@@ -2588,6 +2615,13 @@
                                d->cot_mr, d->Cout, d->cot_cpg, (long)d->Cout, 1, ctc + b * cbs);
         launch_gn_cache(d->cot_prim, d->Cout, Hout * Wout, d->cot_cpg, d->cot_sc, d->cot_sh, d->cot_mr, c->sxcache + sx_cot, st, ACT_SILU);
         a.cot_d = cd; a.cot_d_bs = out_e; a.cot_sx = c->sxcache + sx_cot; a.cot_tc = ctc; a.cot_tc_bs = cbs;
+    }
+    if (d->st_kind != ST_NONE) {
+        a.st_part = d->st_part; a.st_kind = d->st_kind;
+        if (st_cot) {
+            launch_gn_cache(d->cot_prim, d->Cout, Hout * Wout, d->cot_cpg, d->cot_sc, d->cot_sh, d->cot_mr, c->sxcache + sx_cot, st, ACT_SILU);
+            a.st_sx = c->sxcache + sx_cot;
+        }
     }
     if (he != hipSuccess) { c->err = std::string("debug_conv: ") + hipGetErrorString(he); release(); return -1; }
     std::string text;
diff --git a/loco-edit_amd/csrc/kernels.h b/loco-edit_amd/csrc/kernels.h
--- a/loco-edit_amd/csrc/kernels.h
+++ b/loco-edit_amd/csrc/kernels.h
@@ -77,12 +77,16 @@
     size_t partial_floats;
     int pers_groups;
     int tile, pair;
+    int ends;
+    const int* rowwin;
 };
 
 void launch_conv(const ConvArgs& a, int taps, hipStream_t st);
 void launch_conv_bf16x3(const ConvArgs& a, int taps, hipStream_t st);
 void launch_conv_f16(const ConvArgs& a, int taps, hipStream_t st);
 void launch_conv_splitk_reduce(const ConvArgs& a, hipStream_t st);
+void launch_conv_fewcout(const ConvArgs& a, hipStream_t st);
+void launch_conv_fewcin(const ConvArgs& a, hipStream_t st);
 
 struct ConvEnv {
     int prec = 1;
@@ -131,6 +135,7 @@
 void conv_plan_family(ConvArgs& a, int prec);
 int conv_plan_parts(ConvArgs& a, int prec, int tile_override, ConvArgs parts[2]);
 
+bool conv_ends_enabled();
 int conv_bf16_tile_couts(const ConvArgs& a);
 const char* conv_variant_name(const ConvArgs& a, int taps, int prec);
 
@@ -221,7 +226,8 @@
                      const float* base, long base_bs, float* out, long out_bs, int accumulate,
                      int B, int C, int HW, int G, const float* sc, const float* sh, const float* mr,
                      long pbs_c, long pbs_g, const float* tst, long tst_bs, hipStream_t st, int act = 0,
-                     float base_scale = 1.0f);
+                     float base_scale = 1.0f,
+                     const int* rowwin = nullptr, int W = 0);
 
 void launch_ctx_groupnorm(const float* tok, int L, int D, int G, float eps, const float* gamma, const float* beta,
                           float* out, hipStream_t st);
@@ -290,5 +296,6 @@
                       hipStream_t st);
 void launch_mask_gather(const float* U, const int* idx, long L, long n, int k, float* out, hipStream_t st);
 void launch_mask_compact(const uint8_t* mask, long n, int* idx, int* count, hipStream_t st);
+void launch_mask_rowwin(const uint8_t* mask, const uint8_t* mask2, int C, int H, int W, int* win, hipStream_t st);
 
 }
diff --git a/loco-edit_amd/csrc/misc.hip b/loco-edit_amd/csrc/misc.hip
--- a/loco-edit_amd/csrc/misc.hip
+++ b/loco-edit_amd/csrc/misc.hip
@@ -539,9 +539,13 @@
                                                        const float* base, long base_bs, float* out, long out_bs,
                                                        int accumulate, int C, int HW, int cpg, const float* sc,
                                                        const float* sh, const float* mr, long pbs_c, long pbs_g,
-                                                       const float* tst, long tbs, int act, float base_scale) {
+                                                       const float* tst, long tbs, int act, float base_scale,
+                                                       const int* rowwin, int W) {
     const int b = blockIdx.y;
     const long per = (long)C * HW;
+    int wy0 = 0, wy1 = -1;
+    const bool windowed = KIND == 2 && rowwin != nullptr;
+    if (windowed) { wy0 = rowwin[0] - 1; wy1 = rowwin[0] > rowwin[1] ? wy0 - 1 : rowwin[1] + 1; }
     for (long i = ((long)blockIdx.x * 256 + threadIdx.x) * 4; i < per; i += (long)gridDim.x * 1024) {
         int c = (int)(i / HW);
         int g = c / cpg;
@@ -558,7 +562,10 @@
         } else {
             float mean = mr[(long)b * pbs_g + 2 * g], rstd = mr[(long)b * pbs_g + 2 * g + 1];
             float m1 = tst[(long)b * tbs + g * 2], m2 = tst[(long)b * tbs + g * 2 + 1];
-            float4 dv = *reinterpret_cast<const float4*>(d + (long)b * d_bs + i);
+            float4 dv = make_float4(0.f, 0.f, 0.f, 0.f);
+            bool live = true;
+            if (windowed) { const int y = (int)((i - (long)c * HW) / W); live = y >= wy0 && y <= wy1; }
+            if (live) dv = *reinterpret_cast<const float4*>(d + (long)b * d_bs + i);
             float dd[4] = {dv.x, dv.y, dv.z, dv.w};
             float bb[4] = {0.f, 0.f, 0.f, 0.f};
             if (KIND >= 2 && base) {
@@ -587,14 +594,15 @@
 void launch_gn_apply(int kind, const float* d, long d_bs, const float* x, long x_bs, const float* base,
                      long base_bs, float* out, long out_bs, int accumulate, int B, int C, int HW, int G,
                      const float* sc, const float* sh, const float* mr, long pbs_c, long pbs_g, const float* tst,
-                     long tst_bs, hipStream_t st, int act, float base_scale) {
+                     long tst_bs, hipStream_t st, int act, float base_scale, const int* rowwin, int W) {
     long per = (long)C * HW;
+    if (kind != 2 || W <= 0 || (W % 4) != 0) rowwin = nullptr;
     int blocks = (int)((per / 4 + 255) / 256);
     if (blocks > 1024) blocks = 1024;
     dim3 grid(blocks, B);
     int cpg = C / G;
 #define GA(K) hipLaunchKernelGGL(gn_apply_kernel<K>, grid, dim3(256), 0, st, d, d_bs, x, x_bs, base, base_bs, out, \
-                                 out_bs, accumulate, C, HW, cpg, sc, sh, mr, pbs_c, pbs_g, tst, tst_bs, act, base_scale)
+                                 out_bs, accumulate, C, HW, cpg, sc, sh, mr, pbs_c, pbs_g, tst, tst_bs, act, base_scale, rowwin, W)
     switch (kind) {
         case 0: GA(0); break;
         case 1: GA(1); break;
diff --git a/loco-edit_amd/hip.py b/loco-edit_amd/hip.py
--- a/loco-edit_amd/hip.py
+++ b/loco-edit_amd/hip.py
@@ -54,7 +54,8 @@
     _fields_ = ([("struct_size", C.c_int32)] +
                 [(k, C.c_int32) for k in ("Cin", "Cout", "Hin", "Win", "B", "taps", "stride", "upsample", "zins", "mode", "cpg",
                                           "transposed", "accumulate", "in_arena", "pad", "Cin2", "cot_cpg")] +
-                [("res_scale", C.c_float), ("reserved", C.c_int32)] + [(k, C.c_void_p) for k in _PTRS])
+                [("res_scale", C.c_float), ("st_kind", C.c_int32)] + [(k, C.c_void_p) for k in _PTRS] +
+                [("rowwin", C.c_void_p), ("st_part", C.c_void_p)])
 
 
 class LocoTextCfg(C.Structure):
@@ -165,7 +166,7 @@
         lib.loco_sam_destroy.argtypes = [vp]
         lib.loco_sam_destroy.restype = None
     if hasattr(lib, "loco_bench_conv"):
-        lib.loco_bench_conv.argtypes = [vp, i32, i32, i32, i32, i32, i32, i32, i32, i32, C.POINTER(f32), vp]
+        lib.loco_bench_conv.argtypes = [vp, i32, i32, i32, i32, i32, i32, i32, i32, i32, C.POINTER(f32), vp, i32, i32]
         lib.loco_debug_tensor.argtypes = [vp, C.c_char_p, vp, i64, vp]
         lib.loco_debug_tensor.restype = i64
     if hasattr(lib, "loco_debug_conv"):
@@ -608,11 +609,12 @@
             raise RuntimeError(f"{sym} is a diagnostic of include/loco_hip_diag.h: build `make -C loco-edit_amd/csrc diag` "
                                "and set LOCO_HIP_LIB=<repo>/loco-edit_amd/libloco_hip_diag.so")
 
-    def bench_conv(self, cin, cout, H, W, B, mode, taps=9, tile=-1, iters=20) -> float:
+    def bench_conv(self, cin, cout, H, W, B, mode, taps=9, tile=-1, iters=20, window=None) -> float:
         self._need_diag("loco_bench_conv")
         ms = C.c_float()
+        y0, y1 = (-1, -1) if window is None else window
         self._check(self.lib.loco_bench_conv(self._ctx, cin, cout, H, W, B, mode, taps, tile, iters, C.byref(ms),
-                                             _stream()), "loco_bench_conv")
+                                             _stream(), y0, y1), "loco_bench_conv")
         return float(ms.value)
 
     def debug_conv(self, out: torch.Tensor, **desc):
@@ -624,8 +626,13 @@
         _chk_dev(out)
         d.out = out.data_ptr()
         for k, v in desc.items():
-            if k not in LocoConvDesc._PTRS:
-                if not hasattr(d, k) or k in ("struct_size", "reserved"):
+            if k in ("rowwin", "st_part"):
+                if v is not None:
+                    _chk_dev(v, torch.int32 if k == "rowwin" else torch.float32)
+                    keep.append(v)
+                    setattr(d, k, v.data_ptr())
+            elif k not in LocoConvDesc._PTRS:
+                if not hasattr(d, k) or k == "struct_size":
                     raise TypeError(f"debug_conv: no descriptor field {k!r}")
                 setattr(d, k, v)
             elif v is not None:
```

Measured after the change: 20.08 edit-directions/s, median of 6. About the same (+1.0%).
